# meffmadd/intro-tc-vae

Measured on AMD Instinct MI355X. Metric: images/sec (64x64x3, z=128, bs=64) intro-TC step, higher is better.
Workload: dtype f32 in/out/accumulate, conv products on split-fp16 MFMA (two scaled fp16 planes, 3 products, fp32-class); 1 GPU; c2: IntroTCSovler.train_step, conv arch, 64x64x3, z_dim=128, channels (64, 128, 256, 512), batch 64/GPU, Adam lr 2e-4, clip 100, N=10000; global_batch=64, parallelism=single, sync_bn=False

## Files before the change

### include/itcv_hip.h

```cpp
#ifndef ITCV_HIP_H
#define ITCV_HIP_H

#include <stddef.h>
#include <stdint.h>

#ifdef __cplusplus
extern "C" {
#endif

#define ITCV_ABI_VERSION 4

int itcv_abi_version(void);
const char* itcv_last_error(void);
int itcv_set_option(const char* name, int value);
int itcv_get_option(const char* name);

int itcv_profile_begin(void);
int itcv_profile_end(void);
int itcv_profile_get(int i, int* code, double* flop, float* ms);
int itcv_profile_clear(void);

size_t itcv_conv2d_packed_weight_elems(int Co, int Ci, int KS, int for_dgrad);
int itcv_conv2d_pack_weight(const float* w, float* wp, int Co, int Ci, int KS, int for_dgrad,
                            void* stream);
size_t itcv_conv2d_fwd_workspace(int B, int Ci, int H, int W, int Co, int KS);
int itcv_conv2d_fwd(const float* x, const float* wp, const float* bias, float* y, int B, int Ci,
                    int H, int W, int Co, int KS, int up2, void* ws, size_t ws_bytes, void* stream);
int itcv_conv2d_bf16s_supported(int Ci, int Co, int KS);
size_t itcv_conv2d_packed_weight_bytes_bf16s(int Co, int Ci, int KS, int for_dgrad, int ns);
int itcv_conv2d_pack_weight_bf16s(const float* w, void* wp, int Co, int Ci, int KS, int for_dgrad, int ns,
                                  void* stream);
size_t itcv_pack_desc_bytes(void);
int itcv_conv2d_pack_desc_bf16s(void* host_desc, const float* w, void* wp, int Co, int Ci, int KS, int for_dgrad,
                                int ns, int block0);
int itcv_conv2d_pack_weights_bf16s(const void* dev_table, int n, int total_blocks, int ns, void* stream);
size_t itcv_conv2d_fwd_bf16s_workspace(int B, int Ci, int H, int W, int Co, int KS);
int itcv_conv2d_fwd_bf16s(const float* x, const void* wp, const float* bias, float* y, int B, int Ci, int H,
                          int W, int Co, int KS, int up2, int ns, void* ws, size_t ws_bytes, void* stream);
#define ITCV_PLANES_F16X2 4
size_t itcv_planes_bytes(int B, int C, int HW, int ns);
int itcv_split_planes(const float* x, void* planes, int B, int C, int HW, int ns, void* stream);
int itcv_absmax(const float* x, size_t n, float* parts, void* stream);
int itcv_split_planes_scaled(const float* x, void* planes, int B, int C, int HW, int ns, const float* amax, void* stream);
size_t itcv_conv2d_fwd_bf16p_workspace(int B, int Ci, int H, int W, int Co, int KS, int ns);
int itcv_conv2d_fwd_bf16p(const void* xplanes, const void* wp, const float* bias, float* y, int B, int Ci, int H,
                          int W, int Co, int KS, int up2, int ns, void* ws, size_t ws_bytes, void* stream);
int itcv_conv2d_fwd_bf16p_stat_tiles(int B, int Ci, int H, int W, int Co, int KS, int ns);
int itcv_conv2d_fwd_bf16p_st(const void* xplanes, const void* wp, const float* bias, float* y, int B, int Ci, int H,
                             int W, int Co, int KS, int up2, int ns, float* tile_stats, void* ws, size_t ws_bytes,
                             void* stream);
int itcv_conv2d_wgrad_bf16p_supported(int B, int Ci, int H, int W, int Co, int KS);
size_t itcv_conv2d_wgrad_bf16p_workspace(int B, int Ci, int H, int W, int Co, int KS);
int itcv_conv2d_wgrad_bf16p(const void* xplanes, const void* dyplanes, float* dw, int B, int Ci, int H, int W,
                            int Co, int KS, int up2, int ns , int accumulate, void* ws, size_t ws_bytes,
                            void* stream);
int itcv_conv2d_wgrad_bf16p_slabs(int B, int Ci, int H, int W, int Co, int KS);
size_t itcv_wgrad_reduce_desc_bytes(void);
int itcv_wgrad_reduce_desc(void* host_desc, const float* const* slabs, const int* splits, int nsrc, float* dw, int Co,
                           int Ci, int accumulate, int block0);
int itcv_wgrad_reduce_many(const void* dev_table, int n, int total_blocks, void* stream);
int itcv_wgrad_reduce_max_descs(void);
size_t itcv_linear_workspace(int B, int K, int N);
int itcv_linear_fwd(const float* x, const float* w, const float* bias, float* y, int B, int K, int N, void* ws,
                    size_t ws_bytes, void* stream);
int itcv_linear_dgrad(const float* dy, const float* w, float* dx, int B, int K, int N, void* ws, size_t ws_bytes,
                      void* stream);
int itcv_linear_wgrad(const float* dy, const float* x, float* dw, int B, int K, int N, int accumulate, void* ws,
                      size_t ws_bytes, void* stream);
int itcv_conv2d_wgrad5_bf16p_supported(int Cs, int Cb, int H, int W);
size_t itcv_conv2d_wgrad5_bf16p_workspace(int B, int H);
int itcv_conv2d_wgrad5_bf16p(const float* small, const void* big_planes, float* dw, int B, int Cs, int H, int W,
                             int stem, int ns , const float* small_amax ,
                             int accumulate, void* ws, size_t ws_bytes, void* stream);
int itcv_conv2d_small_cout_supported(int Co, int KS);
int itcv_conv2d_small_cout_bf16p_supported(int C, int Co, int KS);
int itcv_conv2d_small_cout_fwd_bf16p(const void* xplanes, const float* w, const float* bias, float* y, int B, int C,
                                     int H, int W, int Co, int KS, int for_dgrad, int ns , void* stream);
int itcv_conv2d_small_cout_fwd(const float* x, const float* w, const float* bias, float* y, int B, int C,
                               int H, int W, int Co, int KS, int for_dgrad, void* stream);
int itcv_conv2d_small_cin_supported(int C, int KS);
int itcv_conv2d_small_cin_fwd(const float* x, const float* w, const float* bias, float* y, int B, int C, int H,
                              int W, int Co, int KS, int for_dgrad, void* stream);

int itcv_conv2d_small_cin_bf16x3_supported(int C, int Co, int KS, int W);
int itcv_conv2d_small_cin_fwd_bf16x3(const float* x, const float* w, const float* bias, float* y, int B, int C, int H,
                                     int W, int Co, int KS, int for_dgrad, int ns ,
                                     const float* x_amax , void* stream);
int itcv_conv2d_wgrad_bf16s_supported(int Ci, int H, int W, int Co, int KS);
int itcv_conv2d_wgrad_bf16s(const float* x, const float* dy, float* dw, int B, int Ci, int H, int W, int Co,
                            int KS, int ns, int accumulate, void* ws, size_t ws_bytes, void* stream);
size_t itcv_conv2d_wgrad_workspace(int B, int Ci, int H, int W, int Co, int KS);
int itcv_conv2d_wgrad(const float* x, const float* dy, float* dw, int B, int Ci, int H, int W,
                      int Co, int KS, int up2, int accumulate, void* ws, size_t ws_bytes, void* stream);
int itcv_conv2d_fwd_variant(int B, int Ci, int H, int W, int Co, int KS, int up2);
int itcv_conv2d_wgrad_variant(int B, int Ci, int H, int W, int Co, int KS, int up2);
size_t itcv_bias_grad_workspace(int B, int C, int HW);
int itcv_bias_grad(const float* dy, float* db, int B, int C, int HW, int accumulate, void* ws,
                   size_t ws_bytes, void* stream);

size_t itcv_bn_workspace(int B, int C, int HW);
int itcv_bn_moments(const float* x, double* sums, int B, int C, int HW, void* ws, size_t ws_bytes,
                    void* stream);
int itcv_bn_train_stats(const float* x, int B, int C, int HW, float eps, float momentum, float* running_mean,
                        float* running_var, int64_t* num_batches_tracked, float* mean, float* rstd, void* ws,
                        size_t ws_bytes, void* stream);
int itcv_bn_finalize(const double* sums, double count, float eps, float momentum, float* running_mean,
                     float* running_var, int64_t* num_batches_tracked, float* mean, float* rstd, int C,
                     void* stream);
int itcv_bn_eval_stats(const float* running_mean, const float* running_var, float eps, float* mean,
                       float* rstd, int C, void* stream);
int itcv_bn_act_fwd(const float* x, const float* mean, const float* rstd, const float* gamma,
                    const float* beta, const float* skip, float* y, int B, int C, int H, int W,
                    float slope, int pool, void* planes, int ns, size_t plane_stride, void* stream);
int itcv_bn_act_planes_supported(int C, int H, int W, int pool);
int itcv_bn_act_bwd_reduce(const float* x, const float* dy, const float* mean, const float* rstd,
                           const float* gamma, const float* beta, const float* skip, double* dsums,
                           float* dgamma, float* dbeta, int accumulate, int B, int C, int H, int W,
                           float slope, int pool, int up2, void* ws, size_t ws_bytes, void* stream);
int itcv_bn_act_bwd_apply(const float* x, const float* dy, const float* mean, const float* rstd,
                          const float* gamma, const float* beta, const float* skip, const double* dsums,
                          const double* local_dsums, double count, float* dx, float* dskip,
                          float* dgamma, float* dbeta, int accumulate, int B, int C, int H, int W,
                          float slope, int pool, int up2, void* dx_planes, int ns, size_t plane_stride, void* stream);

int itcv_bn_train_fwd(const float* x, const float* gamma, const float* beta, const float* skip, float* y, void* planes,
                      int ns, int B, int C, int H, int W, float slope, int pool, float eps, float momentum,
                      float* running_mean, float* running_var, int64_t* num_batches_tracked, float* mean, float* rstd,
                      void* ws, size_t ws_bytes, size_t plane_stride, const float* tile_stats, int tiles, int tile_pitch,
                      int groups, void* stream);
int itcv_bn_train_bwd(const float* x, const float* dy, const float* mean, const float* rstd, const float* gamma,
                      const float* beta, const float* skip, double* dsums, float* dx, float* dskip, void* dx_planes,
                      int ns, float* dgamma, float* dbeta, int accumulate, int B, int C, int H, int W, float slope,
                      int pool, int up2, void* ws, size_t ws_bytes, size_t plane_stride, int groups, void* stream);

#define ITCV_BN_PATH_ONE_BLOCK 0
#define ITCV_BN_PATH_SLICED_FOLD 1
#define ITCV_BN_PATH_SLICED_COMBINE 2
#define ITCV_BN_PATH_FALLBACK 3
#define ITCV_BN_PATH_PER_GROUP 4
#define ITCV_BN_PATH_TILE_STATS 5
int itcv_bn_plan_query(int bwd, int B, int C, int H, int W, int pool, int up2, int groups, int planes, int ns,
                       size_t ws_bytes, int tile_stats, int* path, int* splits);

int itcv_lrelu_fwd(const float* x, float* y, size_t n, float slope, void* stream);
int itcv_lrelu_bwd(const float* x, const float* dy, float* dx, size_t n, float slope, void* stream);
int itcv_sigmoid_fwd(const float* x, float* y, size_t n, void* stream);
int itcv_sigmoid_bwd(const float* y, const float* dy, float* dx, size_t n, void* stream);
int itcv_avgpool2_fwd(const float* x, float* y, int BC, int H, int W, void* stream);
int itcv_avgpool2_bwd(const float* dy, float* dx, int BC, int H, int W, void* stream);
int itcv_upsample2_fwd(const float* x, float* y, int BC, int H, int W, void* stream);
int itcv_upsample2_bwd(const float* dy, float* dx, int BC, int H, int W, void* stream);
int itcv_add(const float* a, const float* b, float* out, size_t n, void* stream);

int itcv_reparam_fwd(const float* mu, const float* logvar, const float* eps, float* z, size_t n,
                     void* stream);
int itcv_reparam_bwd(const float* dz, const float* logvar, const float* eps, float* dmu, float* dlogvar,
                     size_t n, void* stream);
int itcv_kl_rows_fwd(const float* logvar, const float* mu, float* kl, int B, int D, void* stream);
int itcv_kl_rows_bwd(const float* g, const float* logvar, const float* mu, float* dlogvar, float* dmu,
                     int B, int D, void* stream);

#define ITCV_TC_VAR_FROM_ROW 0x1
#define ITCV_TC_EPS_DENSITY 0x2
#define ITCV_TC_WEIGHTED 0x4
#define ITCV_TC_LIVE (ITCV_TC_VAR_FROM_ROW | ITCV_TC_EPS_DENSITY)
size_t itcv_tc_fwd_workspace(int Bl, int Bt, int D);
int itcv_tc_fwd(const float* z, const float* mu_all, const float* logvar, float* prodm, float* logqz,
                float* lse, float* sjoint, int Bl, int Bt, int row_offset, int D, int64_t dataset_size, int flags,
                void* ws, size_t ws_bytes, void* stream);
size_t itcv_tc_bwd_workspace(int Bl, int Bt);
int itcv_tc_bwd(const float* g, const float* z, const float* mu_all, const float* logvar,
                const float* logqz, const float* lse, const float* sjoint, float* dz, float* dmu_all,
                float* dlogvar, int Bl, int Bt, int row_offset, int D, int64_t dataset_size, int flags, void* ws,
                size_t ws_bytes, void* stream);
int itcv_tc_kl_fwd(const float* z, const float* mu_all, const float* logvar, float* out, float* rows, float* prodm,
                   float* logqz, float* lse, float* sjoint, int Bl, int Bt, int row_offset, int D, int64_t dataset_size,
                   float coef_tc, float coef_kl, int reduction, void* ws, size_t ws_bytes, void* stream);
int itcv_tc_kl_bwd(const float* g, const float* z, const float* mu_all, const float* logvar, const float* logqz,
                   const float* lse, const float* sjoint, float* dz, float* dmu_all, float* dlogvar, int Bl, int Bt,
                   int row_offset, int D, int64_t dataset_size, float coef_tc, float coef_kl, int reduction, void* ws,
                   size_t ws_bytes, void* stream);
size_t itcv_tc_full_fwd_workspace(int Bl, int Bt, int D);
int itcv_tc_full_fwd(const float* z, const float* mu_all, const float* logvar_all, int ld, float* out, float* rows,
                     float* comps, float* prodm, float* logqz, float* lse, float* sjoint, float* ivar, int Bl, int Bt,
                     int row_offset, int D, int64_t dataset_size, float alpha, float beta, float gamma, int reduction,
                     void* ws, size_t ws_bytes, void* stream);
size_t itcv_tc_full_bwd_workspace(int Bl, int Bt);
int itcv_tc_full_bwd(const float* g, const float* z, const float* mu_all, const float* logvar_all, int ld,
                     const float* logqz, const float* lse, const float* sjoint, const float* ivar, float* dz, float* dmu_all,
                     float* dlogvar_all, int Bl, int Bt, int row_offset, int D, int64_t dataset_size, float alpha,
                     float beta, float gamma, int reduction, void* ws, size_t ws_bytes, void* stream);
int itcv_kl_loss_fwd(const float* logvar, const float* mu, float* out, int B, int D, int reduction, float scale, void* stream);
int itcv_kl_loss_bwd(const float* g, const float* logvar, const float* mu, float* dlogvar, float* dmu, int B, int D,
                     int reduction, float scale, void* stream);
int itcv_diag_logdensity_rows(const float* z, const float* mu, const float* logvar, float* logq_cx,
                              float* logpz, int B, int D, void* stream);
int itcv_gauss_logdensity_fwd(const float* x, const float* mu, const float* logvar, float* out, const int64_t* dims,
                              const int64_t* sx, const int64_t* sm, const int64_t* sl, int eps_density, void* stream);
int itcv_gauss_logdensity_bwd(const float* g, const float* x, const float* mu, const float* logvar, float* dx,
                              float* dlogvar, const int64_t* dims, const int64_t* sx, const int64_t* sm,
                              const int64_t* sl, int eps_density, void* stream);
int itcv_sampling_fwd(const float* lp, float* prodm, float* logqz, float* lse, float* sjoint, int B, int D,
                      int64_t dataset_size, int weighted, void* stream);
int itcv_sampling_bwd(const float* g_prodm, const float* g_logqz, const float* lp, const float* lse,
                      const float* sjoint, const float* logqz, float* dlp, int B, int D, int64_t dataset_size,
                      int weighted, void* stream);
int itcv_on_off_diag(const float* x, float* diag, float* off, int m, int n, void* stream);

#define ITCV_LOSS_MSE 0
#define ITCV_LOSS_L1 1
#define ITCV_LOSS_BCE 2
int itcv_recon_rows_fwd(const float* x, const float* recon, float* rows, int B, size_t P, int loss_type,
                        void* ws, size_t ws_bytes, void* stream);
size_t itcv_recon_workspace(int B, size_t P);
int itcv_recon_rows_bwd(const float* x, const float* recon, const float* g, float* drecon, int B, size_t P,
                        int loss_type, void* stream);

int itcv_recon_loss_fwd(const float* x, const float* recon, float* out, int B, size_t P, int loss_type, int reduction,
                        float scale, void* ws, size_t ws_bytes, void* stream);
int itcv_recon_loss_bwd(const float* x, const float* recon, const float* g, float* drecon, int B, size_t P,
                        int loss_type, int reduction, float scale, void* stream);
int itcv_exp_elbo_fwd(const float* a, const float* b, float* out, float* w, int B, float c, void* stream);
int itcv_exp_elbo_bwd(const float* g, const float* w, float* da, float* db, int B, void* stream);
int itcv_lincomb_fwd(const float* const* terms, const float* weights, int n, float* out, void* stream);
int itcv_lincomb_bwd(const float* g, const float* weights, int n, float* grads, void* stream);

size_t itcv_sumsq_workspace(size_t n);
int itcv_sumsq(const float* x, size_t n, double* out, void* ws, size_t ws_bytes, void* stream);
int itcv_clip_coef(const double* sumsq, int nparts, double clip, float* norm_out, float* coef_out,
                   void* stream);
int itcv_scale_by_dev(float* x, size_t n, const float* coef_dev, void* stream);
int itcv_adam_step(float* p, const float* g, float* m, float* v, size_t n, float lr, float beta1,
                   float beta2, float eps, int step, void* stream);
int itcv_adam_step_dev(float* p, const float* g, float* m, float* v, size_t n, float lr, float beta1,
                       float beta2, float eps, int* step_dev, void* stream);
#define ITCV_OPT_MAXIMIZE 0x1
#define ITCV_OPT_NESTEROV 0x2
#define ITCV_OPT_AMSGRAD 0x4
#define ITCV_OPT_DECOUPLED_WD 0x8
#define ITCV_OPT_CENTERED 0x10
int itcv_adamx_step_dev(float* p, const float* g, float* exp_avg, float* exp_avg_sq, float* max_exp_avg_sq,
                        const unsigned char* live, size_t n, double lr, double beta1, double beta2, double eps,
                        double weight_decay, int flags, int* step_dev, void* stream);
int itcv_sgd_step_dev(float* p, const float* g, float* momentum_buffer, const unsigned char* live, size_t n, double lr,
                      double momentum, double dampening, double weight_decay, int flags, int* step_dev, void* stream);
int itcv_adagrad_step_dev(float* p, const float* g, float* sum, const unsigned char* live, size_t n, double lr,
                          double lr_decay, double weight_decay, double eps, int flags, int* step_dev, void* stream);
int itcv_rmsprop_step_dev(float* p, const float* g, float* square_avg, float* momentum_buffer, float* grad_avg,
                          const unsigned char* live, size_t n, double lr, double alpha, double eps,
                          double weight_decay, double momentum, int flags, int* step_dev, void* stream);
int itcv_fill(float* x, size_t n, float value, void* stream);
int itcv_hflip(const float* x, float* y, const unsigned char* flip, int B, int rows_per_image, int W, void* stream);

#ifdef __cplusplus
}
#endif
#endif
```

### intro-tc-vae_amd/csrc/norm_act.hip

```cpp
#include <stdlib.h>

#include <type_traits>

#include "common.h"

namespace itcv {

constexpr int kRedThreads = 256;

__device__ __forceinline__ uint32_t fdiv(uint32_t a, uint32_t d, int sh) { return sh >= 0 ? (a >> sh) : (a / d); }

struct BnGrp {
  size_t xs;
  size_t os;
  size_t dys;
  size_t ps;
  int cs;
  int G;
};

struct BnFinal {
  double count;
  float eps, momentum;
  float* running_mean;
  float* running_var;
  int64_t* nbt;
  float* mean;
  float* rstd;
};

__device__ __forceinline__ void bn_finalize(double s1, double s2, double count, float eps, float momentum,
                                            float* running_mean, float* running_var, int c, float& mean_c, float& rstd_c) {
  const double m = s1 / count;
  double var = s2 / count - m * m;
  if (var < 0.0) var = 0.0;
  mean_c = (float)m;
  rstd_c = (float)(1.0 / sqrt(var + (double)eps));
  if (running_mean) running_mean[c] = (1.f - momentum) * running_mean[c] + momentum * (float)m;
  if (running_var) {
    const double unbiased = count > 1.0 ? var * count / (count - 1.0) : var;
    running_var[c] = (1.f - momentum) * running_var[c] + momentum * (float)unbiased;
  }
}

template <bool FUSED>
__global__ __launch_bounds__(kRedThreads) void bn_moments_partial(const float* __restrict__ x,
                                                                  double* __restrict__ part, int B, int C, int HW,
                                                                  int splits, int hw_shift, BnFinal f, BnGrp grp) {
  __shared__ double scratch[kRedThreads / 64];
  const uint32_t c = blockIdx.x, s = blockIdx.y, hw_n = HW, total = (uint32_t)B * hw_n;
  const uint32_t chunk = ((total + splits - 1) / splits + 3) & ~3u;
  const uint32_t beg = s * chunk, end = min(beg + chunk, total);
  const int ngroups = (FUSED && grp.G > 1) ? grp.G : 1;
  if (!FUSED) {
    x += (size_t)blockIdx.z * grp.xs;
    part += (size_t)blockIdx.z * splits * 2 * C;
  }
 for (int gi = 0; gi < ngroups; ++gi, x += grp.xs, f.mean += grp.cs, f.rstd += grp.cs) {
  double s1 = 0.0, s2 = 0.0;
  if ((HW & 3) == 0) {
#pragma unroll 4
    for (uint32_t i = beg + threadIdx.x * 4; i < end; i += kRedThreads * 4) {
      const uint32_t b = fdiv(i, hw_n, hw_shift), hw = i - b * hw_n;
      const float4 v = *reinterpret_cast<const float4*>(x + ((size_t)b * C + c) * hw_n + hw);
      s1 += ((double)v.x + (double)v.y) + ((double)v.z + (double)v.w);
      s2 += ((double)v.x * v.x + (double)v.y * v.y) + ((double)v.z * v.z + (double)v.w * v.w);
    }
  } else {
    for (uint32_t i = beg + threadIdx.x; i < end; i += kRedThreads) {
      const uint32_t b = fdiv(i, hw_n, hw_shift), hw = i - b * hw_n;
      const float v = x[((size_t)b * C + c) * hw_n + hw];
      s1 += (double)v;
      s2 += (double)v * v;
    }
  }
  s1 = block_sum(s1, scratch);
  s2 = block_sum(s2, scratch);
  if (threadIdx.x == 0) {
    if (FUSED) {
      bn_finalize(s1, s2, f.count, f.eps, f.momentum, f.running_mean, f.running_var, c, f.mean[c], f.rstd[c]);
      if (c == 0 && f.nbt) f.nbt[0] += 1;
    } else {
      part[((size_t)s * 2 + 0) * C + c] = s1;
      part[((size_t)s * 2 + 1) * C + c] = s2;
    }
  }
 }
}

__global__ void combine_partials(const double* __restrict__ part, double* __restrict__ sums, int C2, int splits) {
  const int i = blockIdx.x * blockDim.x + threadIdx.x;
  if (i >= C2) return;
  sums[i] = fold_strided(0.0, part + i, (size_t)C2, splits);
}

__global__ void bn_finalize_kernel(const double* __restrict__ sums, double count, float eps, float momentum,
                                   float* running_mean, float* running_var, int64_t* nbt, float* mean, float* rstd,
                                   int C) {
  const int c = blockIdx.x * blockDim.x + threadIdx.x;
  if (c == 0 && nbt) nbt[0] += 1;
  if (c >= C) return;
  bn_finalize(sums[c], sums[C + c], count, eps, momentum, running_mean, running_var, c, mean[c], rstd[c]);
}

__global__ __launch_bounds__(256) void bn_tile_stats_finalize_kernel(const float* __restrict__ ts, int tiles, int pitch,
                                                                    double count, float eps, float momentum,
                                                                    float* running_mean, float* running_var, int64_t* nbt,
                                                                    float* mean, float* rstd, int C) {
  __shared__ double scratch[4];
  const int c = blockIdx.x;
  const float* p1 = ts + (size_t)c * pitch;
  const float* p2 = ts + ((size_t)C + c) * pitch;
  double s1 = 0.0, s2 = 0.0;
  for (int t = threadIdx.x; t < tiles; t += 256) s1 += (double)p1[t], s2 += (double)p2[t];
  s1 = block_sum(s1, scratch);
  s2 = block_sum(s2, scratch);
  if (threadIdx.x == 0) {
    bn_finalize(s1, s2, count, eps, momentum, running_mean, running_var, c, mean[c], rstd[c]);
    if (c == 0 && nbt) nbt[0] += 1;
  }
}

__global__ void bn_combine_finalize_groups_kernel(const double* __restrict__ part, int splits, int G, double count, float eps,
                                                  float momentum, float* running_mean, float* running_var, int64_t* nbt,
                                                  float* mean, float* rstd, int C) {
  const int c = blockIdx.x * blockDim.x + threadIdx.x;
  if (c == 0 && nbt) nbt[0] += G;
  if (c >= C) return;
  for (int g = 0; g < G; ++g) {
    const double* pg = part + (size_t)g * splits * 2 * C;
    const double s1 = fold_strided(0.0, pg + c, (size_t)2 * C, splits);
    const double s2 = fold_strided(0.0, pg + C + c, (size_t)2 * C, splits);
    bn_finalize(s1, s2, count, eps, momentum, running_mean, running_var, c, mean[(size_t)g * C + c], rstd[(size_t)g * C + c]);
  }
}
__global__ void bn_combine_param_groups_kernel(const double* __restrict__ part, double* __restrict__ dsums, int C, int splits,
                                               int G, float* dgamma, float* dbeta, int accumulate) {
  const int c = blockIdx.x * blockDim.x + threadIdx.x;
  if (c >= C) return;
  float db = (accumulate && dbeta) ? dbeta[c] : 0.f, dg = (accumulate && dgamma) ? dgamma[c] : 0.f;
  for (int g = 0; g < G; ++g) {
    const double* pg = part + (size_t)g * splits * 2 * C;
    const double s1 = fold_strided(0.0, pg + c, (size_t)2 * C, splits);
    const double s2 = fold_strided(0.0, pg + C + c, (size_t)2 * C, splits);
    dsums[(size_t)g * 2 * C + c] = s1;
    dsums[(size_t)g * 2 * C + C + c] = s2;
    db += (float)s1, dg += (float)s2;
  }
  if (dbeta) dbeta[c] = db;
  if (dgamma) dgamma[c] = dg;
}

__global__ void bn_eval_stats_kernel(const float* rm, const float* rv, float eps, float* mean, float* rstd, int C) {
  const int c = blockIdx.x * blockDim.x + threadIdx.x;
  if (c >= C) return;
  mean[c] = rm[c];
  rstd[c] = 1.f / sqrtf(rv[c] + eps);
}

__device__ __forceinline__ float lrelu(float v, float slope) { return v > 0.f ? v : v * slope; }

template <int POOL>
__global__ void bn_act_fwd_kernel(const float* __restrict__ x, const float* __restrict__ mean,
                                  const float* __restrict__ rstd, const float* __restrict__ gamma,
                                  const float* __restrict__ beta, const float* __restrict__ skip,
                                  float* __restrict__ y, int C, int H, int W, size_t nout, float slope,
                                  int hw_shift, int c_mask) {
  const int HW = H * W;
  if (POOL == 0) {
    for (size_t i = ((size_t)blockIdx.x * blockDim.x + threadIdx.x) * 4; i < nout;
         i += (size_t)gridDim.x * blockDim.x * 4) {
      const uint32_t pl = fdiv((uint32_t)i, HW, hw_shift);
      const int c = c_mask >= 0 ? (int)(pl & (uint32_t)c_mask) : (int)(pl % (uint32_t)C);
      const float sc = gamma[c] * rstd[c], sh = beta[c] - mean[c] * sc;
      float4 v = *reinterpret_cast<const float4*>(x + i);
      v.x = v.x * sc + sh, v.y = v.y * sc + sh, v.z = v.z * sc + sh, v.w = v.w * sc + sh;
      if (skip) {
        const float4 k = *reinterpret_cast<const float4*>(skip + i);
        v.x += k.x, v.y += k.y, v.z += k.z, v.w += k.w;
      }
      v.x = lrelu(v.x, slope), v.y = lrelu(v.y, slope), v.z = lrelu(v.z, slope), v.w = lrelu(v.w, slope);
      *reinterpret_cast<float4*>(y + i) = v;
    }
  } else {
    const int Ho = H / 2, Wo = W / 2, HWo = Ho * Wo;
    for (size_t i = (size_t)blockIdx.x * blockDim.x + threadIdx.x; i < nout; i += (size_t)gridDim.x * blockDim.x) {
      const uint32_t bc = hw_shift >= 2 ? ((uint32_t)i >> (hw_shift - 2)) : (uint32_t)i / (uint32_t)HWo;
      const int r = (int)((uint32_t)i - bc * HWo), ho = r / Wo, wo = r - ho * Wo;
      const int c = c_mask >= 0 ? (int)(bc & (uint32_t)c_mask) : (int)(bc % (uint32_t)C);
      const float sc = gamma[c] * rstd[c], sh = beta[c] - mean[c] * sc;
      const size_t src = (size_t)bc * HW + (size_t)(2 * ho) * W + 2 * wo;
      const float2 a = *reinterpret_cast<const float2*>(x + src);
      const float2 b = *reinterpret_cast<const float2*>(x + src + W);
      float v0 = a.x * sc + sh, v1 = a.y * sc + sh, v2 = b.x * sc + sh, v3 = b.y * sc + sh;
      if (skip) {
        const float2 ka = *reinterpret_cast<const float2*>(skip + src);
        const float2 kb = *reinterpret_cast<const float2*>(skip + src + W);
        v0 += ka.x, v1 += ka.y, v2 += kb.x, v3 += kb.y;
      }
      y[i] = 0.25f * (lrelu(v0, slope) + lrelu(v1, slope) + lrelu(v2, slope) + lrelu(v3, slope));
    }
  }
}

constexpr int kStatCh = 64;
struct BnStatsIn {
  const double* part;
  int splits;
  double count;
  float eps, momentum;
  float* running_mean;
  float* running_var;
  int64_t* nbt;
  float* mean_out;
  float* rstd_out;
};

template <int PX, int NS>
__device__ __forceinline__ void store_planes_wave(u32x4* __restrict__ planes, size_t plane_stride, uint32_t per_plane,
                                                  uint32_t HWo, uint32_t cidx0, const u32x4 (&ch)[PX][NS],
                                                  u32x4* __restrict__ strip) {
  const uint32_t lane = threadIdx.x & 63;
#pragma unroll
  for (int p = 0; p < NS; ++p) {
#pragma unroll
    for (int s = 0; s < PX; ++s) strip[lane * PX + s] = ch[s][p];
#pragma unroll
    for (int k = 0; k < PX; ++k) {
      const uint32_t n = k * 64 + lane, idx2 = cidx0 + n / PX, s2 = n % PX;
      const uint32_t bc8 = idx2 / per_plane, pp = idx2 - bc8 * per_plane;
      planes[(size_t)p * plane_stride + (size_t)bc8 * HWo + (size_t)pp * PX + s2] = strip[n];
    }
  }
}

template <int POOL, int NS, bool STATS, bool F16 = false>
__global__ __launch_bounds__(256) void bn_act_fwd_planes_kernel(
    const float* __restrict__ x, const float* __restrict__ mean, const float* __restrict__ rstd,
    const float* __restrict__ gamma, const float* __restrict__ beta, const float* __restrict__ skip,
    float* __restrict__ y, u32x4* __restrict__ planes, int B, int C, int H, int W, float slope, BnStatsIn st,
    size_t plane_stride, BnGrp grp) {
  if constexpr (F16) {
    if (blockIdx.x == 0 && blockIdx.z == 0 && threadIdx.x == 0) {
      ScaleRec* rec = reinterpret_cast<ScaleRec*>(planes + (size_t)NS * plane_stride);
      rec->scale = 1.f, rec->inv = 1.f, rec->pad[0] = rec->pad[1] = 0.f;
    }
  }
  {
    const size_t g = blockIdx.z;
    x += g * grp.xs, planes += g * grp.ps, mean += g * grp.cs, rstd += g * grp.cs;
    if (skip) skip += g * grp.xs;
    if (y) y += g * grp.os;
  }
  __shared__ float s_mean[STATS ? kStatCh : 1], s_rstd[STATS ? kStatCh : 1];
  constexpr int PX = POOL ? 2 : 4;
  __shared__ u32x4 strips[4][64 * PX];
  const int HW = H * W, C8 = C >> 3;
  const int Ho = POOL ? H / 2 : H, Wo = POOL ? W / 2 : W, HWo = Ho * Wo;
  const uint32_t per_plane = (uint32_t)HWo / PX, total = (uint32_t)B * C8 * per_plane;
  for (uint32_t base = blockIdx.x * blockDim.x; base < total; base += gridDim.x * blockDim.x) {
    const uint32_t idx = base + threadIdx.x;
    const uint32_t g0 = base / per_plane;
    if (STATS) {
      __syncthreads();
      const uint32_t last = min(base + blockDim.x, total) - 1, ng = last / per_plane - g0 + 1;
      if (threadIdx.x < ng * 8) {
        const uint32_t gz = blockIdx.z, G = grp.G > 1 ? grp.G : 1;
        const uint32_t g = g0 + threadIdx.x / 8, c = (g % C8) * 8 + (threadIdx.x & 7);
        const double* part = st.part + (size_t)gz * st.splits * 2 * C;
        const double s1 = fold_strided(0.0, part + c, (size_t)2 * C, st.splits);
        const double s2 = fold_strided(0.0, part + C + c, (size_t)2 * C, st.splits);
        float mf, rf;
        bn_finalize(s1, s2, st.count, st.eps, 0.f, nullptr, nullptr, 0, mf, rf);
        s_mean[threadIdx.x] = mf, s_rstd[threadIdx.x] = rf;
        if (g < (uint32_t)C8 && g * per_plane >= base) {
          st.mean_out[(size_t)gz * C + c] = mf, st.rstd_out[(size_t)gz * C + c] = rf;
          if (gz == 0) {
            double t1 = s1, t2 = s2;
            for (uint32_t gg = 0; gg < G; ++gg) {
              if (gg) {
                const double* pg = st.part + (size_t)gg * st.splits * 2 * C;
                t1 = fold_strided(0.0, pg + c, (size_t)2 * C, st.splits);
                t2 = fold_strided(0.0, pg + C + c, (size_t)2 * C, st.splits);
              }
              float um, ur;
              bn_finalize(t1, t2, st.count, st.eps, st.momentum, st.running_mean, st.running_var, c, um, ur);
            }
            if (c == 0 && st.nbt) st.nbt[0] += G;
          }
        }
      }
      __syncthreads();
    }
    if (idx >= total) continue;
    const uint32_t bc8 = idx / per_plane, pp = idx - bc8 * per_plane;
    const uint32_t b = bc8 / C8, c8 = bc8 - b * C8;
    float o[8][PX];
    float4 xin[POOL ? 1 : 8];
    float p_ga[8], p_be[8], p_mu[8], p_rs[8];
#pragma unroll
    for (int j = 0; j < 8; ++j) {
      const int c = c8 * 8 + j;
      if (POOL == 0) xin[POOL ? 0 : j] = *reinterpret_cast<const float4*>(x + ((size_t)b * C + c) * HW + (size_t)pp * 4);
      p_ga[j] = gamma[c], p_be[j] = beta[c];
      p_mu[j] = STATS ? s_mean[(bc8 - g0) * 8 + j] : mean[c], p_rs[j] = STATS ? s_rstd[(bc8 - g0) * 8 + j] : rstd[c];
    }
#pragma unroll
    for (int j = 0; j < 8; ++j) {
      const int c = c8 * 8 + j;
      const float mu = p_mu[j], rs = p_rs[j];
      const float sc = p_ga[j] * rs, sh = p_be[j] - mu * sc;
      const size_t bc = (size_t)b * C + c;
      if (POOL == 0) {
        const size_t i = bc * HW + (size_t)pp * 4;
        float4 v = xin[POOL ? 0 : j];
        v.x = v.x * sc + sh, v.y = v.y * sc + sh, v.z = v.z * sc + sh, v.w = v.w * sc + sh;
        if (skip) {
          const float4 k = *reinterpret_cast<const float4*>(skip + i);
          v.x += k.x, v.y += k.y, v.z += k.z, v.w += k.w;
        }
        v.x = lrelu(v.x, slope), v.y = lrelu(v.y, slope), v.z = lrelu(v.z, slope), v.w = lrelu(v.w, slope);
        if (y) *reinterpret_cast<float4*>(y + i) = v;
        o[j][0] = v.x, o[j][1] = v.y, o[j][POOL ? 0 : 2] = v.z, o[j][POOL ? 1 : 3] = v.w;
      } else {
        const uint32_t ho = (pp * 2) / Wo, wo = pp * 2 - ho * Wo;
        const size_t src = bc * HW + (size_t)(2 * ho) * W + 2 * wo;
        const float4 a = *reinterpret_cast<const float4*>(x + src);
        const float4 bb = *reinterpret_cast<const float4*>(x + src + W);
        float v0 = a.x * sc + sh, v1 = a.y * sc + sh, v2 = bb.x * sc + sh, v3 = bb.y * sc + sh;
        float w0 = a.z * sc + sh, w1 = a.w * sc + sh, w2 = bb.z * sc + sh, w3 = bb.w * sc + sh;
        if (skip) {
          const float4 ka = *reinterpret_cast<const float4*>(skip + src);
          const float4 kb = *reinterpret_cast<const float4*>(skip + src + W);
          v0 += ka.x, v1 += ka.y, v2 += kb.x, v3 += kb.y;
          w0 += ka.z, w1 += ka.w, w2 += kb.z, w3 += kb.w;
        }
        const float r0 = 0.25f * (lrelu(v0, slope) + lrelu(v1, slope) + lrelu(v2, slope) + lrelu(v3, slope));
        const float r1 = 0.25f * (lrelu(w0, slope) + lrelu(w1, slope) + lrelu(w2, slope) + lrelu(w3, slope));
        if (y) *reinterpret_cast<float2*>(y + bc * HWo + (size_t)pp * 2) = make_float2(r0, r1);
        o[j][0] = r0, o[j][1] = r1;
      }
    }
    u32x4 chk[PX][NS];
#pragma unroll
    for (int px = 0; px < PX; ++px) {
      float v8[8];
#pragma unroll
      for (int j = 0; j < 8; ++j) v8[j] = o[j][px];
      split8<NS, F16>(v8, chk[px]);
    }
    const uint32_t cidx0 = base + (threadIdx.x & ~63u);
    if (cidx0 + 64 <= total) {
      store_planes_wave<PX, NS>(planes, plane_stride, per_plane, (uint32_t)HWo, cidx0, chk, strips[threadIdx.x >> 6]);
    } else {
#pragma unroll
      for (int px = 0; px < PX; ++px)
#pragma unroll
        for (int p = 0; p < NS; ++p) planes[(size_t)p * plane_stride + (size_t)bc8 * HWo + (size_t)pp * PX + px] = chk[px][p];
    }
  }
}

template <int MODE>
__device__ __forceinline__ float upstream(const float* __restrict__ dy, size_t bc, int h, int w, int H, int W) {
  if (MODE == 0) return dy[bc * H * W + (size_t)h * W + w];
  if (MODE == 1) return 0.25f * dy[bc * (H / 2) * (W / 2) + (size_t)(h >> 1) * (W / 2) + (w >> 1)];
  const size_t base = bc * (size_t)(4 * H * W) + (size_t)(2 * h) * (2 * W) + 2 * w;
  const float2 a = *reinterpret_cast<const float2*>(dy + base);
  const float2 b = *reinterpret_cast<const float2*>(dy + base + 2 * W);
  return (a.x + a.y) + (b.x + b.y);
}

template <int MODE>
__global__ __launch_bounds__(kRedThreads) void bn_bwd_partial(const float* __restrict__ x,
                                                              const float* __restrict__ dy,
                                                              const float* __restrict__ mean,
                                                              const float* __restrict__ rstd,
                                                              const float* __restrict__ gamma,
                                                              const float* __restrict__ beta,
                                                              const float* __restrict__ skip,
                                                              double* __restrict__ part, int B, int C, int H, int W,
                                                              float slope, int splits) {
  __shared__ double scratch[kRedThreads / 64];
  const int c = blockIdx.x, s = blockIdx.y, HW = H * W;
  const size_t total = (size_t)B * HW;
  const size_t chunk = (total + splits - 1) / splits;
  const size_t beg = (size_t)s * chunk, end = beg + chunk < total ? beg + chunk : total;
  const float mu = mean[c], rs = rstd[c], ga = gamma[c], be = beta[c];
  double s1 = 0.0, s2 = 0.0;
  for (size_t i = beg + threadIdx.x; i < end; i += kRedThreads) {
    const size_t b = i / HW;
    const int hw = (int)(i - b * HW), h = hw / W, w = hw - h * W;
    const size_t bc = b * C + c;
    const float xh = (x[bc * HW + hw] - mu) * rs;
    float u = xh * ga + be;
    if (skip) u += skip[bc * HW + hw];
    float g = upstream<MODE>(dy, bc, h, w, H, W);
    if (!(u > 0.f)) g *= slope;
    s1 += (double)g;
    s2 += (double)g * (double)xh;
  }
  s1 = block_sum(s1, scratch);
  s2 = block_sum(s2, scratch);
  if (threadIdx.x == 0) {
    part[((size_t)s * 2 + 0) * C + c] = s1;
    part[((size_t)s * 2 + 1) * C + c] = s2;
  }
}

template <int MODE>
__global__ void bn_bwd_apply_kernel(const float* __restrict__ x, const float* __restrict__ dy,
                                    const float* __restrict__ mean, const float* __restrict__ rstd,
                                    const float* __restrict__ gamma, const float* __restrict__ beta,
                                    const float* __restrict__ skip, const double* __restrict__ dsums, double count,
                                    float* __restrict__ dx, float* __restrict__ dskip, int C, int H, int W,
                                    size_t n, float slope) {
  const int HW = H * W;
  for (size_t i = (size_t)blockIdx.x * blockDim.x + threadIdx.x; i < n; i += (size_t)gridDim.x * blockDim.x) {
    const size_t bc = i / HW;
    const int hw = (int)(i - bc * HW), h = hw / W, w = hw - h * W;
    const int c = (int)(bc % C);
    const float mu = mean[c], rs = rstd[c], ga = gamma[c];
    const float xh = (x[i] - mu) * rs;
    float u = xh * ga + beta[c];
    if (skip) u += skip[i];
    float g = upstream<MODE>(dy, bc, h, w, H, W);
    if (!(u > 0.f)) g *= slope;
    const float m1 = (float)(dsums[c] / count), m2 = (float)(dsums[C + c] / count);
    dx[i] = ga * rs * (g - m1 - xh * m2);
    if (dskip) dskip[i] = g;
  }
}



template <int MODE>
__device__ __forceinline__ float4 upstream4(const float* __restrict__ dy, uint32_t bc, uint32_t h, uint32_t w,
                                            uint32_t H, uint32_t W) {
  if (MODE == 0) return *reinterpret_cast<const float4*>(dy + (size_t)bc * H * W + h * W + w);
  if (MODE == 1) {
    const float2 d = *reinterpret_cast<const float2*>(dy + (size_t)bc * (H / 2) * (W / 2) + (h >> 1) * (W / 2) + (w >> 1));
    return make_float4(0.25f * d.x, 0.25f * d.x, 0.25f * d.y, 0.25f * d.y);
  }
  const float* p = dy + (size_t)bc * (4 * H * W) + (size_t)(2 * h) * (2 * W) + 2 * w;
  const float4 a0 = *reinterpret_cast<const float4*>(p), a1 = *reinterpret_cast<const float4*>(p + 4);
  const float4 b0 = *reinterpret_cast<const float4*>(p + 2 * W), b1 = *reinterpret_cast<const float4*>(p + 2 * W + 4);
  return make_float4((a0.x + a0.y) + (b0.x + b0.y), (a0.z + a0.w) + (b0.z + b0.w), (a1.x + a1.y) + (b1.x + b1.y),
                     (a1.z + a1.w) + (b1.z + b1.w));
}

struct BnBwdFinal {
  double* dsums;
  float* dgamma;
  float* dbeta;
  int accumulate;
};

template <int MODE, bool FUSED, bool MX = false>
__global__ __launch_bounds__(kRedThreads) void bn_bwd_partial_v4(
    const float* __restrict__ x, const float* __restrict__ dy, const float* __restrict__ mean,
    const float* __restrict__ rstd, const float* __restrict__ gamma, const float* __restrict__ beta,
    const float* __restrict__ skip, double* __restrict__ part, int B, int C, int H, int W, float slope, int splits,
    int w_shift, int hw_shift, BnBwdFinal f, BnGrp grp, float* __restrict__ mx = nullptr, int nmx = 0) {
  __shared__ double scratch[kRedThreads / 64];
  __shared__ float mscratch[MX ? 2 * (kRedThreads / 64) : 1];
  const uint32_t gz = FUSED ? 0u : blockIdx.z;
  const uint32_t c = blockIdx.x, s = blockIdx.y, HW = H * W, total = (uint32_t)B * HW;
  const uint32_t chunk = ((total + splits - 1) / splits + 3) & ~3u;
  const uint32_t beg = s * chunk, end = min(beg + chunk, total);
  const float ga = gamma[c], be = beta[c];
  const int ngroups = (FUSED && grp.G > 1) ? grp.G : 1;
  if (!FUSED) {
    const size_t g = blockIdx.z;
    x += g * grp.xs, dy += g * grp.dys, mean += g * grp.cs, rstd += g * grp.cs, part += g * splits * 2 * C;
    if (skip) skip += g * grp.xs;
  }
  float acc_db = 0.f, acc_dg = 0.f;
  if (FUSED && threadIdx.x == 0 && f.accumulate) {
    if (f.dbeta) acc_db = f.dbeta[c];
    if (f.dgamma) acc_dg = f.dgamma[c];
  }
 for (int gi = 0; gi < ngroups; ++gi, x += grp.xs, dy += grp.dys, mean += grp.cs, rstd += grp.cs, f.dsums += 2 * grp.cs) {
  if (skip && gi) skip += grp.xs;
  const float mu = mean[c], rs = rstd[c];
  double s1 = 0.0, s2 = 0.0;
  float gmax = 0.f, xmax = 0.f;
  constexpr int U = 4;
  for (uint32_t i0 = beg + threadIdx.x * 4; i0 < end; i0 += kRedThreads * 4 * U) {
    float4 xv4[U], g4[U], k4[U];
    bool ok[U];
#pragma unroll
    for (int u = 0; u < U; ++u) {
      const uint32_t iu = i0 + (uint32_t)u * kRedThreads * 4;
      ok[u] = iu < end;
      const uint32_t i = ok[u] ? iu : i0;
      const uint32_t b = fdiv(i, HW, hw_shift), hw = i - b * HW;
      const uint32_t h = fdiv(hw, W, w_shift), w = hw - h * W;
      const uint32_t bc = b * C + c;
      xv4[u] = *reinterpret_cast<const float4*>(x + (size_t)bc * HW + hw);
      g4[u] = upstream4<MODE>(dy, bc, h, w, H, W);
    }
    if (skip) {
#pragma unroll
      for (int u = 0; u < U; ++u) {
        const uint32_t iu = i0 + (uint32_t)u * kRedThreads * 4, i = iu < end ? iu : i0;
        const uint32_t b = fdiv(i, HW, hw_shift), hw = i - b * HW;
        k4[u] = *reinterpret_cast<const float4*>(skip + (size_t)(b * C + c) * HW + hw);
      }
    } else {
#pragma unroll
      for (int u = 0; u < U; ++u) k4[u] = make_float4(0.f, 0.f, 0.f, 0.f);
    }
#pragma unroll
    for (int u = 0; u < U; ++u) {
      const float4 xv = xv4[u];
      float4 g = g4[u];
      const float xh0 = (xv.x - mu) * rs, xh1 = (xv.y - mu) * rs, xh2 = (xv.z - mu) * rs, xh3 = (xv.w - mu) * rs;
      float u0 = xh0 * ga + be, u1 = xh1 * ga + be, u2 = xh2 * ga + be, u3 = xh3 * ga + be;
      if (skip) u0 += k4[u].x, u1 += k4[u].y, u2 += k4[u].z, u3 += k4[u].w;
      if (!(u0 > 0.f)) g.x *= slope;
      if (!(u1 > 0.f)) g.y *= slope;
      if (!(u2 > 0.f)) g.z *= slope;
      if (!(u3 > 0.f)) g.w *= slope;
      const double a1 = ((double)g.x + (double)g.y) + ((double)g.z + (double)g.w);
      const double a2 = ((double)g.x * xh0 + (double)g.y * xh1) + ((double)g.z * xh2 + (double)g.w * xh3);
      s1 += ok[u] ? a1 : 0.0;
      s2 += ok[u] ? a2 : 0.0;
      if constexpr (MX) {
        const float gm = fmaxf(fmaxf(fabsf(g.x), fabsf(g.y)), fmaxf(fabsf(g.z), fabsf(g.w)));
        const float xm = fmaxf(fmaxf(fabsf(xh0), fabsf(xh1)), fmaxf(fabsf(xh2), fabsf(xh3)));
        gmax = fmaxf(gmax, ok[u] ? gm : 0.f);
        xmax = fmaxf(xmax, ok[u] ? xm : 0.f);
      }
    }
  }
  s1 = block_sum(s1, scratch);
  s2 = block_sum(s2, scratch);
  if constexpr (MX) {
    gmax = wave_max(gmax), xmax = wave_max(xmax);
    if ((threadIdx.x & 63) == 0) mscratch[threadIdx.x >> 6] = gmax, mscratch[kRedThreads / 64 + (threadIdx.x >> 6)] = xmax;
    __syncthreads();
    if (threadIdx.x == 0) {
      float gm = 0.f, xm = 0.f;
      for (int k = 0; k < kRedThreads / 64; ++k) gm = fmaxf(gm, mscratch[k]), xm = fmaxf(xm, mscratch[kRedThreads / 64 + k]);
      const size_t idx = ((size_t)(FUSED ? (uint32_t)gi : gz) * splits + s) * C + c;
      mx[idx] = fabsf(ga * rs) * gm, mx[(size_t)nmx + idx] = xm;
    }
    __syncthreads();
  }
  if (threadIdx.x == 0) {
    if (FUSED) {
      f.dsums[c] = s1;
      f.dsums[C + c] = s2;
      acc_db += (float)s1, acc_dg += (float)s2;
    } else {
      part[((size_t)s * 2 + 0) * C + c] = s1;
      part[((size_t)s * 2 + 1) * C + c] = s2;
    }
  }
 }
  if (FUSED && threadIdx.x == 0) {
    if (f.dbeta) f.dbeta[c] = acc_db;
    if (f.dgamma) f.dgamma[c] = acc_dg;
  }
}

template <int MODE>
__global__ void bn_bwd_apply_v4(const float* __restrict__ x, const float* __restrict__ dy,
                                const float* __restrict__ mean, const float* __restrict__ rstd,
                                const float* __restrict__ gamma, const float* __restrict__ beta,
                                const float* __restrict__ skip, const double* __restrict__ dsums, double count,
                                float* __restrict__ dx, float* __restrict__ dskip, int C, int H, int W, uint32_t n4,
                                float slope, int w_shift, int hw_shift, int c_mask) {
  const uint32_t HW = H * W;
  for (uint32_t j = blockIdx.x * blockDim.x + threadIdx.x; j < n4; j += gridDim.x * blockDim.x) {
    const uint32_t i = j * 4;
    const uint32_t bc = fdiv(i, HW, hw_shift), hw = i - bc * HW;
    const uint32_t h = fdiv(hw, W, w_shift), w = hw - h * W;
    const uint32_t c = c_mask >= 0 ? (bc & (uint32_t)c_mask) : (bc % (uint32_t)C);
    const float mu = mean[c], rs = rstd[c], ga = gamma[c], be = beta[c];
    const float m1 = (float)(dsums[c] / count), m2 = (float)(dsums[C + c] / count), gr = ga * rs;
    const float4 xv = *reinterpret_cast<const float4*>(x + i);
    float4 g = upstream4<MODE>(dy, bc, h, w, H, W);
    const float xh0 = (xv.x - mu) * rs, xh1 = (xv.y - mu) * rs, xh2 = (xv.z - mu) * rs, xh3 = (xv.w - mu) * rs;
    float u0 = xh0 * ga + be, u1 = xh1 * ga + be, u2 = xh2 * ga + be, u3 = xh3 * ga + be;
    if (skip) {
      const float4 k = *reinterpret_cast<const float4*>(skip + i);
      u0 += k.x, u1 += k.y, u2 += k.z, u3 += k.w;
    }
// ... 42 lines not shown
      for (int k = 0; k < 4; ++k) {
        u = fmaxf(fmaxf(u, fmaxf(tu[k].x, tu[k].y)), fmaxf(tu[k].z, tu[k].w));
        v = fmaxf(fmaxf(v, fmaxf(tv[k].x, tv[k].y)), fmaxf(tv[k].z, tv[k].w));
      }
    }
    u = wave_max(u), v = wave_max(v);
    if ((threadIdx.x & 63) == 0) s_uv[threadIdx.x >> 6] = u, s_uv[4 + (threadIdx.x >> 6)] = v;
    __syncthreads();
    u = fmaxf(fmaxf(s_uv[0], s_uv[1]), fmaxf(s_uv[2], s_uv[3]));
    v = fmaxf(fmaxf(s_uv[4], s_uv[5]), fmaxf(s_uv[6], s_uv[7]));
    pscale = scale_for_bound(u * (2.f + v));
    if (blockIdx.x == 0 && blockIdx.z == 0 && threadIdx.x == 0) {
      ScaleRec* rec = reinterpret_cast<ScaleRec*>(planes + (size_t)NS * plane_stride);
      rec->scale = pscale, rec->inv = 1.f / pscale, rec->pad[0] = rec->pad[1] = 0.f;
    }
  }
  const uint32_t zg = gridDim.z - 1 - blockIdx.z;
  {
    const size_t g = zg;
    x += g * grp.xs, dy += g * grp.dys, planes += g * grp.ps, mean += g * grp.cs, rstd += g * grp.cs;
    if (dsums) dsums += g * 2 * grp.cs;
    if (skip) skip += g * grp.xs;
    if (dx) dx += g * grp.xs;
    if (dskip) dskip += g * grp.xs;
  }
  __shared__ float s_m1[SUMS ? kStatCh : 1], s_m2[SUMS ? kStatCh : 1];
  __shared__ u32x4 strips[4][64 * 4];
  const uint32_t HW = H * W, C8 = C >> 3, per_plane = HW / 4, total = (uint32_t)B * C8 * per_plane;
  const uint32_t sweep = gridDim.x * blockDim.x, rbase = (gridDim.x - 1 - blockIdx.x) * blockDim.x;
  for (int it = (int)((total + sweep - 1) / sweep) - 1; it >= 0; --it) {
    const uint32_t base = (uint32_t)it * sweep + rbase;
    if (base >= total) continue;
    const uint32_t idx = base + threadIdx.x;
    const uint32_t g0 = base / per_plane;
    if (SUMS) {
      __syncthreads();
      const uint32_t last = min(base + blockDim.x, total) - 1, ng = last / per_plane - g0 + 1;
      if (threadIdx.x < ng * 8) {
        const uint32_t gz = zg, G = grp.G > 1 ? grp.G : 1;
        const uint32_t g = g0 + threadIdx.x / 8, c = (g % C8) * 8 + (threadIdx.x & 7);
        const double* part = sm.part + (size_t)gz * sm.splits * 2 * C;
        const double s1 = fold_strided(0.0, part + c, (size_t)2 * C, sm.splits);
        const double s2 = fold_strided(0.0, part + C + c, (size_t)2 * C, sm.splits);
        s_m1[threadIdx.x] = (float)(s1 / count), s_m2[threadIdx.x] = (float)(s2 / count);
        if (g < C8 && g * per_plane >= base) {
          sm.dsums_out[(size_t)gz * 2 * C + c] = s1, sm.dsums_out[(size_t)gz * 2 * C + C + c] = s2;
          if (gz == 0) {
            float db = (sm.accumulate && sm.dbeta) ? sm.dbeta[c] : 0.f, dg = (sm.accumulate && sm.dgamma) ? sm.dgamma[c] : 0.f;
            db += (float)s1, dg += (float)s2;
            for (uint32_t gg = 1; gg < G; ++gg) {
              const double* pg = sm.part + (size_t)gg * sm.splits * 2 * C;
              db += (float)fold_strided(0.0, pg + c, (size_t)2 * C, sm.splits);
              dg += (float)fold_strided(0.0, pg + C + c, (size_t)2 * C, sm.splits);
            }
            if (sm.dbeta) sm.dbeta[c] = db;
            if (sm.dgamma) sm.dgamma[c] = dg;
          }
        }
      }
      __syncthreads();
    }
    if (idx >= total) continue;
    const uint32_t bc8 = idx / per_plane, p4 = idx - bc8 * per_plane;
    const uint32_t b = bc8 / C8, c8 = bc8 - b * C8;
    const uint32_t hw = p4 * 4, h = fdiv(hw, W, w_shift), w = hw - h * W;
    float o[8][4];
#pragma unroll
    for (int j0 = 0; j0 < 8; j0 += 4) {
      float4 xv4[4], g4[4], k4[4];
      float pm[4][4];
      double ds4[4][2];
#pragma unroll
      for (int jj = 0; jj < 4; ++jj) {
        const uint32_t c = c8 * 8 + j0 + jj, bc = b * C + c;
        xv4[jj] = *reinterpret_cast<const float4*>(x + bc * HW + hw);
        g4[jj] = upstream4<MODE>(dy, bc, h, w, H, W);
        pm[jj][0] = mean[c], pm[jj][1] = rstd[c], pm[jj][2] = gamma[c], pm[jj][3] = beta[c];
        if (!SUMS) ds4[jj][0] = dsums[c], ds4[jj][1] = dsums[C + c];
      }
      if (skip) {
#pragma unroll
        for (int jj = 0; jj < 4; ++jj) k4[jj] = *reinterpret_cast<const float4*>(skip + (b * C + c8 * 8 + j0 + jj) * HW + hw);
      } else {
#pragma unroll
        for (int jj = 0; jj < 4; ++jj) k4[jj] = make_float4(0.f, 0.f, 0.f, 0.f);
      }
#pragma unroll
      for (int jj = 0; jj < 4; ++jj) {
        const int j = j0 + jj;
        const uint32_t c = c8 * 8 + j, bc = b * C + c;
        const uint32_t i = bc * HW + hw;
        const float mu = pm[jj][0], rs = pm[jj][1], ga = pm[jj][2], be = pm[jj][3];
        const float m1 = SUMS ? s_m1[(bc8 - g0) * 8 + j] : (float)(ds4[jj][0] / count);
        const float m2 = SUMS ? s_m2[(bc8 - g0) * 8 + j] : (float)(ds4[jj][1] / count), gr = ga * rs;
        const float4 xv = xv4[jj];
        float4 g = g4[jj];
        const float xh0 = (xv.x - mu) * rs, xh1 = (xv.y - mu) * rs, xh2 = (xv.z - mu) * rs, xh3 = (xv.w - mu) * rs;
        float u0 = xh0 * ga + be, u1 = xh1 * ga + be, u2 = xh2 * ga + be, u3 = xh3 * ga + be;
        if (skip) {
          const float4 k = k4[jj];
          u0 += k.x, u1 += k.y, u2 += k.z, u3 += k.w;
        }
        if (!(u0 > 0.f)) g.x *= slope;
        if (!(u1 > 0.f)) g.y *= slope;
        if (!(u2 > 0.f)) g.z *= slope;
        if (!(u3 > 0.f)) g.w *= slope;
        const float4 d = make_float4(gr * (g.x - m1 - xh0 * m2), gr * (g.y - m1 - xh1 * m2), gr * (g.z - m1 - xh2 * m2),
                                     gr * (g.w - m1 - xh3 * m2));
        if (dx) *reinterpret_cast<float4*>(dx + i) = d;
        if (dskip) *reinterpret_cast<float4*>(dskip + i) = g;
        o[j][0] = d.x, o[j][1] = d.y, o[j][2] = d.z, o[j][3] = d.w;
      }
    }
    u32x4 chk[4][NS];
#pragma unroll
    for (int px = 0; px < 4; ++px) {
      float v8[8];
#pragma unroll
      for (int j = 0; j < 8; ++j) v8[j] = o[j][px];
      split8<NS, F16>(v8, chk[px], pscale);
    }
    const uint32_t cidx0 = base + (threadIdx.x & ~63u);
    if (cidx0 + 64 <= total) {
      store_planes_wave<4, NS>(planes, plane_stride, per_plane, HW, cidx0, chk, strips[threadIdx.x >> 6]);
    } else {
#pragma unroll
      for (int px = 0; px < 4; ++px)
#pragma unroll
        for (int p = 0; p < NS; ++p) planes[(size_t)p * plane_stride + (size_t)bc8 * HW + hw + px] = chk[px][p];
    }
  }
}

__global__ void bn_param_grad_kernel(const double* __restrict__ local, float* dgamma, float* dbeta, int C,
                                     int accumulate) {
  const int c = blockIdx.x * blockDim.x + threadIdx.x;
  if (c >= C) return;
  if (dbeta) dbeta[c] = (accumulate ? dbeta[c] : 0.f) + (float)local[c];
  if (dgamma) dgamma[c] = (accumulate ? dgamma[c] : 0.f) + (float)local[C + c];
}

__global__ void lrelu_fwd_kernel(const float* __restrict__ x, float* __restrict__ y, size_t n, float slope) {
  for (size_t i = (size_t)blockIdx.x * blockDim.x + threadIdx.x; i < n; i += (size_t)gridDim.x * blockDim.x)
    y[i] = lrelu(x[i], slope);
}
__global__ void lrelu_bwd_kernel(const float* __restrict__ x, const float* __restrict__ dy, float* __restrict__ dx,
                                 size_t n, float slope) {
  for (size_t i = (size_t)blockIdx.x * blockDim.x + threadIdx.x; i < n; i += (size_t)gridDim.x * blockDim.x)
    dx[i] = x[i] > 0.f ? dy[i] : dy[i] * slope;
}
__global__ void sigmoid_fwd_kernel(const float* __restrict__ x, float* __restrict__ y, size_t n) {
  for (size_t i = (size_t)blockIdx.x * blockDim.x + threadIdx.x; i < n; i += (size_t)gridDim.x * blockDim.x)
    y[i] = 1.f / (1.f + expf(-x[i]));
}
__global__ void sigmoid_bwd_kernel(const float* __restrict__ y, const float* __restrict__ dy,
                                   float* __restrict__ dx, size_t n) {
  for (size_t i = (size_t)blockIdx.x * blockDim.x + threadIdx.x; i < n; i += (size_t)gridDim.x * blockDim.x) {
    const float s = y[i];
    dx[i] = dy[i] * (1.f - s) * s;
  }
}
__global__ void add_kernel(const float* __restrict__ a, const float* __restrict__ b, float* __restrict__ o,
                           size_t n) {
  for (size_t i = (size_t)blockIdx.x * blockDim.x + threadIdx.x; i < n; i += (size_t)gridDim.x * blockDim.x)
    o[i] = a[i] + b[i];
}
__global__ void avgpool2_fwd_kernel(const float* __restrict__ x, float* __restrict__ y, int H, int W, size_t nout) {
  const int Ho = H / 2, Wo = W / 2;
  for (size_t i = (size_t)blockIdx.x * blockDim.x + threadIdx.x; i < nout; i += (size_t)gridDim.x * blockDim.x) {
    const size_t bc = i / ((size_t)Ho * Wo);
    const int r = (int)(i - bc * Ho * Wo), ho = r / Wo, wo = r - ho * Wo;
    const size_t src = bc * H * W + (size_t)(2 * ho) * W + 2 * wo;
    const float2 a = *reinterpret_cast<const float2*>(x + src);
    const float2 b = *reinterpret_cast<const float2*>(x + src + W);
    y[i] = 0.25f * ((a.x + a.y) + (b.x + b.y));
  }
}
__global__ void avgpool2_bwd_kernel(const float* __restrict__ dy, float* __restrict__ dx, int H, int W, size_t n) {
  for (size_t i = (size_t)blockIdx.x * blockDim.x + threadIdx.x; i < n; i += (size_t)gridDim.x * blockDim.x) {
    const size_t bc = i / ((size_t)H * W);
    const int r = (int)(i - bc * H * W), h = r / W, w = r - h * W;
    dx[i] = 0.25f * dy[bc * (H / 2) * (W / 2) + (size_t)(h >> 1) * (W / 2) + (w >> 1)];
  }
}
__global__ void upsample2_fwd_kernel(const float* __restrict__ x, float* __restrict__ y, int H, int W, size_t n) {
  const int Ho = 2 * H, Wo = 2 * W;
  for (size_t i = (size_t)blockIdx.x * blockDim.x + threadIdx.x; i < n; i += (size_t)gridDim.x * blockDim.x) {
    const size_t bc = i / ((size_t)Ho * Wo);
    const int r = (int)(i - bc * Ho * Wo), h = r / Wo, w = r - h * Wo;
    y[i] = x[bc * H * W + (size_t)(h >> 1) * W + (w >> 1)];
  }
}
__global__ void upsample2_bwd_kernel(const float* __restrict__ dy, float* __restrict__ dx, int H, int W, size_t n) {
  for (size_t i = (size_t)blockIdx.x * blockDim.x + threadIdx.x; i < n; i += (size_t)gridDim.x * blockDim.x) {
    const size_t bc = i / ((size_t)H * W);
    const int r = (int)(i - bc * H * W), h = r / W, w = r - h * W;
    dx[i] = upstream<2>(dy, bc, h, w, H, W);
  }
}

static inline int ilog2_exact(int v) {
  if (v <= 0 || (v & (v - 1))) return -1;
  int sh = 0;
  while ((1 << sh) < v) ++sh;
  return sh;
}

static inline int grid_for(size_t n, int per_thread = 1) {
  size_t b = cdivz(cdivz(n, per_thread), 256);
  if (b > 256 * 8) b = 256 * 8;
  return b < 1 ? 1 : (int)b;
}

static inline bool bn_fmt_ok(int ns) { return ns == 2 || ns == 3 || ns == ITCV_PLANES_F16X2; }
static inline int bn_splits(int B, int C, int HW) {
  const size_t total = (size_t)B * HW;
  constexpr int target = 1024;
  int s = cdiv(target, C);
  const size_t maxs = cdivz(total, 1024);
  if ((size_t)s > maxs) s = (int)maxs;
  if (s < 1) s = 1;
  if (C >= 256 && total <= 65536) s = 1;
  return s;
}

enum class BnPath {
  OneBlock,
  SlicedFold,
  SlicedCombine,
  Fallback,
  PerGroup,
  TileStats,
};
struct BnPlan {
  BnPath path;
  int G, splits, mode;
  bool vec, f16;
  int per_plane, nmx;
  BnGrp grp;
  size_t pstride;
  size_t part_doubles;
  size_t ws_need;
  dim3 rgrid, agrid;
};

static inline size_t bn_ws_bytes(int G, int splits, int C, bool maxima) {
  return (size_t)G * splits * 2 * C * (sizeof(double) + (maxima ? sizeof(float) : 0));
}

static BnPlan bn_plan(bool bwd, int B, int C, int H, int W, int pool, int up2, int groups, bool planes, int ns,
                      size_t plane_stride, size_t ws_bytes, bool tile_stats) {
  BnPlan p{};
  const bool opool = !bwd && pool;
  const int HW = H * W, HWo = opool ? HW / 4 : HW;
  const size_t n = (size_t)B * C * HW;
  p.G = groups > 1 ? groups : 1;
  p.splits = bn_splits(B, C, HW);
  p.mode = pool ? 1 : (up2 ? 2 : 0);
  p.vec = W % 4 == 0 && n < (1ull << 31);
  p.f16 = ns == ITCV_PLANES_F16X2 && (planes || (bwd && groups > 1));
  p.per_plane = HWo / (opool ? 2 : 4);
  p.nmx = p.G * p.splits * C;
  p.grp = BnGrp{n, (size_t)B * C * HWo, pool ? n / 4 : (up2 ? n * 4 : n), (size_t)B * (C / 8) * HWo, C, p.G};
  p.pstride = plane_stride ? plane_stride : p.grp.ps;
  p.part_doubles = (size_t)p.G * p.splits * 2 * C;
  p.ws_need = bn_ws_bytes(p.G, p.splits, C, bwd && p.f16);
  const bool planes_ok = planes && bn_fmt_ok(ns) && itcv_bn_act_planes_supported(C, H, W, opool) && n < (1ull << 31);
  if (tile_stats) p.path = groups > 1 ? BnPath::PerGroup : BnPath::TileStats;
  else if (!planes_ok) p.path = groups > 1 ? BnPath::PerGroup : BnPath::Fallback;
  else if (p.splits == 1) p.path = BnPath::OneBlock;
  else if (groups > 1 && ws_bytes < p.ws_need) p.path = BnPath::PerGroup;
  else p.path = p.per_plane >= 64 ? BnPath::SlicedFold : BnPath::SlicedCombine;
  if (groups > 1 && p.path == BnPath::OneBlock && !(bwd && p.f16)) p.ws_need = 0;
  p.rgrid = dim3(C, p.splits, p.splits == 1 ? 1 : p.G);
  if (planes_ok) p.agrid = dim3(grid_for((size_t)B * (C / 8) * p.per_plane), 1, p.G);
  else p.agrid = dim3(bwd ? grid_for(n, p.vec ? 4 : 1) : grid_for((size_t)B * C * HWo, pool ? 1 : 4));
  return p;
}

template <int N, typename F>
static inline void bn_pick(int v, F&& f) {
  if constexpr (N > 1) {
    if (v == N - 1) return f(std::integral_constant<int, N - 1>{});
    return bn_pick<N - 1>(v, f);
  } else {
    f(std::integral_constant<int, 0>{});
  }
}
static inline int bn_fmt(int ns) { return ns == ITCV_PLANES_F16X2 ? 2 : (ns == 2 ? 0 : 1); }

static int bn_stats_launch(const BnPlan& p, const float* x, int B, int C, int HW, const BnFinal& f, void* ws, size_t ws_bytes,
                           hipStream_t st, const char* who) {
  ITCV_REQUIRE(!p.ws_need || (ws && ws_bytes >= p.ws_need), who);
  double* part = static_cast<double*>(ws);
  if (p.splits == 1)
    hipLaunchKernelGGL(bn_moments_partial<true>, p.rgrid, dim3(kRedThreads), 0, st, x, part, B, C, HW, 1, ilog2_exact(HW), f,
                       p.grp);
  else
    hipLaunchKernelGGL(bn_moments_partial<false>, p.rgrid, dim3(kRedThreads), 0, st, x, part, B, C, HW, p.splits,
                       ilog2_exact(HW), BnFinal{}, p.grp);
  ITCV_CHECK_LAUNCH(who);
  if (p.splits > 1 && p.path != BnPath::SlicedFold) {
    hipLaunchKernelGGL(bn_combine_finalize_groups_kernel, dim3(cdiv(C, 256)), dim3(256), 0, st, part, p.splits, p.G, f.count,
                       f.eps, f.momentum, f.running_mean, f.running_var, f.nbt, f.mean, f.rstd, C);
    ITCV_CHECK_LAUNCH(who);
  }
  return 0;
}

static int bn_fwd_apply_launch(const BnPlan& p, const float* x, const float* mean, const float* rstd, const float* gamma,
                               const float* beta, const float* skip, float* y, void* planes, int ns, int B, int C, int H, int W,
                               float slope, int pool, const BnStatsIn& fold, hipStream_t st) {
  ITCV_REQUIRE((size_t)B * C * H * W < (1ull << 31), "itcv_bn_act_fwd(tensor < 2^31 elements)");
  if (planes) {
    ITCV_REQUIRE(bn_fmt_ok(ns) && itcv_bn_act_planes_supported(C, H, W, pool), "itcv_bn_act_fwd(planes)");
    bn_pick<2>(pool ? 1 : 0, [&](auto pool_c) {
      bn_pick<3>(bn_fmt(ns), [&](auto fmt_c) {
        bn_pick<2>(fold.part ? 1 : 0, [&](auto stats_c) {
          constexpr int POOL = decltype(pool_c)::value, FMT = decltype(fmt_c)::value;
          constexpr bool STATS = decltype(stats_c)::value != 0;
          launch_timed((bn_act_fwd_planes_kernel<POOL, FMT == 1 ? 3 : 2, STATS, FMT == 2>), p.agrid, dim3(256), 0, st, x, mean,
                       rstd, gamma, beta, skip, y, static_cast<u32x4*>(planes), B, C, H, W, slope, fold, p.pstride, p.grp);
        });
      });
    });
    ITCV_CHECK_LAUNCH("itcv_bn_act_fwd(planes)");
    return 0;
  }
  if (pool) ITCV_REQUIRE(H % 2 == 0 && W % 2 == 0, "itcv_bn_act_fwd(pool)");
  else ITCV_REQUIRE((H * W) % 4 == 0, "itcv_bn_act_fwd(H*W % 4)");
  const size_t nout = pool ? (size_t)B * C * (H / 2) * (W / 2) : (size_t)B * C * H * W;
  bn_pick<2>(pool ? 1 : 0, [&](auto pool_c) {
    hipLaunchKernelGGL(bn_act_fwd_kernel<decltype(pool_c)::value>, p.agrid, dim3(256), 0, st, x, mean, rstd, gamma, beta, skip,
                       y, C, H, W, nout, slope, ilog2_exact(H * W), ilog2_exact(C) >= 0 ? C - 1 : -1);
  });
  ITCV_CHECK_LAUNCH("itcv_bn_act_fwd");
  return 0;
}

static int bn_bwd_reduce_launch(const BnPlan& p, const float* x, const float* dy, const float* mean, const float* rstd,
                                const float* gamma, const float* beta, const float* skip, double* dsums, float* dgamma,
                                float* dbeta, int accumulate, int B, int C, int H, int W, float slope, void* ws, size_t ws_bytes,
                                hipStream_t st, const char* who) {
  if (p.mode == 1) ITCV_REQUIRE(H % 2 == 0 && W % 2 == 0, who);
  ITCV_REQUIRE(!p.ws_need || (ws && ws_bytes >= p.ws_need), who);
  ITCV_REQUIRE(!p.f16 || p.vec, "itcv_bn_train_bwd(fp16 planes need W % 4 == 0)");
  double* part = static_cast<double*>(ws);
  float* mx = p.f16 ? reinterpret_cast<float*>(part + p.part_doubles) : nullptr;
  const bool fused = p.vec && p.splits == 1;
  const BnBwdFinal bf = fused ? BnBwdFinal{dsums, dgamma, dbeta, accumulate} : BnBwdFinal{};
  bn_pick<3>(p.mode, [&](auto mode_c) {
    constexpr int MODE = decltype(mode_c)::value;
    if (!p.vec) {
      hipLaunchKernelGGL(bn_bwd_partial<MODE>, p.rgrid, dim3(kRedThreads), 0, st, x, dy, mean, rstd, gamma, beta, skip, part,
                         B, C, H, W, slope, p.splits);
      return;
    }
    bn_pick<2>(fused ? 1 : 0, [&](auto fused_c) {
      bn_pick<2>(p.f16 ? 1 : 0, [&](auto mx_c) {
        hipLaunchKernelGGL((bn_bwd_partial_v4<MODE, decltype(fused_c)::value != 0, decltype(mx_c)::value != 0>), p.rgrid,
                           dim3(kRedThreads), 0, st, x, dy, mean, rstd, gamma, beta, skip, part, B, C, H, W, slope, p.splits,
                           ilog2_exact(W), ilog2_exact(H * W), bf, p.grp, mx, p.nmx);
      });
    });
  });
  ITCV_CHECK_LAUNCH(who);
  if (!fused && p.path != BnPath::SlicedFold) {
    hipLaunchKernelGGL(bn_combine_param_groups_kernel, dim3(cdiv(C, 256)), dim3(256), 0, st, part, dsums, C, p.splits, p.G,
                       dgamma, dbeta, accumulate);
    ITCV_CHECK_LAUNCH(who);
  }
  return 0;
}

static int bn_bwd_apply_launch(const BnPlan& p, const float* x, const float* dy, const float* mean, const float* rstd,
                               const float* gamma, const float* beta, const float* skip, const double* dsums, double count,
                               float* dx, float* dskip, void* dx_planes, int ns, int B, int C, int H, int W, float slope,
                               const BnBwdSumsIn& fold, const float* mx, hipStream_t st) {
  ITCV_REQUIRE(x && dy && mean && rstd && gamma && beta && dsums && (dx || dx_planes) && B > 0 && C > 0 && count > 0,
               "itcv_bn_act_bwd_apply");
  const int wsh = ilog2_exact(W);
  if (dx_planes) {
    ITCV_REQUIRE(bn_fmt_ok(ns) && p.vec && itcv_bn_act_planes_supported(C, H, W, 0), "itcv_bn_act_bwd_apply(planes)");
    if (ns == ITCV_PLANES_F16X2 && !mx)
      return fail("%s: fp16 gradient planes take their scale from the maxima of the reduce pass: use itcv_bn_train_bwd",
                  "itcv_bn_act_bwd_apply");
    bn_pick<3>(p.mode, [&](auto mode_c) {
      bn_pick<3>(bn_fmt(ns), [&](auto fmt_c) {
        bn_pick<2>(fold.part ? 1 : 0, [&](auto sums_c) {
          constexpr int MODE = decltype(mode_c)::value, FMT = decltype(fmt_c)::value;
          constexpr bool SUMS = decltype(sums_c)::value != 0;
          launch_timed((bn_bwd_apply_planes<MODE, FMT == 1 ? 3 : 2, SUMS, FMT == 2>), p.agrid, dim3(256), 0, st, x, dy, mean,
                       rstd, gamma, beta, skip, SUMS ? static_cast<const double*>(nullptr) : dsums, count, dx, dskip,
                       static_cast<u32x4*>(dx_planes), B, C, H, W, slope, wsh, fold, p.pstride, p.grp, mx, p.nmx);
        });
      });
    });
    ITCV_CHECK_LAUNCH("itcv_bn_act_bwd_apply(planes)");
    return 0;
  }
  const size_t n = (size_t)B * C * H * W;
  bn_pick<3>(p.mode, [&](auto mode_c) {
    constexpr int MODE = decltype(mode_c)::value;
    if (p.vec)
      hipLaunchKernelGGL(bn_bwd_apply_v4<MODE>, p.agrid, dim3(256), 0, st, x, dy, mean, rstd, gamma, beta, skip, dsums, count,
                         dx, dskip, C, H, W, (uint32_t)(n / 4), slope, wsh, ilog2_exact(H * W),
                         ilog2_exact(C) >= 0 ? C - 1 : -1);
    else
      hipLaunchKernelGGL(bn_bwd_apply_kernel<MODE>, p.agrid, dim3(256), 0, st, x, dy, mean, rstd, gamma, beta, skip, dsums,
                         count, dx, dskip, C, H, W, n, slope);
  });
  ITCV_CHECK_LAUNCH("itcv_bn_act_bwd_apply");
  return 0;
}

}

using namespace itcv;

extern "C" {

size_t itcv_bn_workspace(int B, int C, int HW) {
  if (B <= 0 || C <= 0 || HW <= 0) return 0;
  return bn_ws_bytes(1, bn_splits(B, C, HW), C, true);
}

int itcv_bn_moments(const float* x, double* sums, int B, int C, int HW, void* ws, size_t ws_bytes, void* stream) {
  ITCV_REQUIRE(x && sums && B > 0 && C > 0 && HW > 0, "itcv_bn_moments");
  const int splits = bn_splits(B, C, HW);
  ITCV_REQUIRE(ws && ws_bytes >= bn_ws_bytes(1, splits, C, false), "itcv_bn_moments(workspace)");
  double* part = static_cast<double*>(ws);
  hipLaunchKernelGGL(bn_moments_partial<false>, dim3(C, splits), dim3(kRedThreads), 0, S(stream), x, part, B, C, HW,
                     splits, ilog2_exact(HW), BnFinal{}, BnGrp{});
  ITCV_CHECK_LAUNCH("itcv_bn_moments");
  hipLaunchKernelGGL(combine_partials, dim3(cdiv(2 * C, 256)), dim3(256), 0, S(stream), part, sums, 2 * C, splits);
  ITCV_CHECK_LAUNCH("itcv_bn_moments(combine)");
  return 0;
}

int itcv_bn_train_stats(const float* x, int B, int C, int HW, float eps, float momentum, float* running_mean,
                        float* running_var, int64_t* num_batches_tracked, float* mean, float* rstd, void* ws,
                        size_t ws_bytes, void* stream) {
  ITCV_REQUIRE(x && mean && rstd && B > 0 && C > 0 && HW > 0, "itcv_bn_train_stats");
  const BnPlan p = bn_plan(false, B, C, HW, 1, 0, 0, 1, false, 0, 0, ws ? ws_bytes : 0, false);
  const BnFinal f{(double)B * HW, eps, momentum, running_mean, running_var, num_batches_tracked, mean, rstd};
  return bn_stats_launch(p, x, B, C, HW, f, ws, ws_bytes, S(stream), "itcv_bn_train_stats");
}

int itcv_bn_finalize(const double* sums, double count, float eps, float momentum, float* running_mean,
                     float* running_var, int64_t* num_batches_tracked, float* mean, float* rstd, int C,
                     void* stream) {
  ITCV_REQUIRE(sums && mean && rstd && C > 0 && count > 0, "itcv_bn_finalize");
  hipLaunchKernelGGL(bn_finalize_kernel, dim3(cdiv(C, 256)), dim3(256), 0, S(stream), sums, count, eps, momentum,
                     running_mean, running_var, num_batches_tracked, mean, rstd, C);
  ITCV_CHECK_LAUNCH("itcv_bn_finalize");
  return 0;
}

int itcv_bn_eval_stats(const float* running_mean, const float* running_var, float eps, float* mean, float* rstd,
                       int C, void* stream) {
  ITCV_REQUIRE(running_mean && running_var && mean && rstd && C > 0, "itcv_bn_eval_stats");
  hipLaunchKernelGGL(bn_eval_stats_kernel, dim3(cdiv(C, 256)), dim3(256), 0, S(stream), running_mean, running_var,
                     eps, mean, rstd, C);
  ITCV_CHECK_LAUNCH("itcv_bn_eval_stats");
  return 0;
}

int itcv_bn_act_planes_supported(int C, int H, int W, int pool) {
  return C > 0 && (C & 7) == 0 && H > 0 && W > 0 && W % 4 == 0 && (!pool || H % 2 == 0);
}

int itcv_bn_act_fwd(const float* x, const float* mean, const float* rstd, const float* gamma, const float* beta,
                    const float* skip, float* y, int B, int C, int H, int W, float slope, int pool, void* planes,
                    int ns, size_t plane_stride, void* stream) {
  ITCV_REQUIRE(x && mean && rstd && gamma && beta && (y || planes) && B > 0 && C > 0 && H > 0 && W > 0, "itcv_bn_act_fwd");
  const BnPlan p = bn_plan(false, B, C, H, W, pool, 0, 1, planes != nullptr, ns, plane_stride, 0, false);
  return bn_fwd_apply_launch(p, x, mean, rstd, gamma, beta, skip, y, planes, ns, B, C, H, W, slope, pool, BnStatsIn{},
                             S(stream));
}

int itcv_bn_act_bwd_reduce(const float* x, const float* dy, const float* mean, const float* rstd, const float* gamma,
                           const float* beta, const float* skip, double* dsums, float* dgamma, float* dbeta,
                           int accumulate, int B, int C, int H, int W, float slope, int pool, int up2, void* ws,
                           size_t ws_bytes, void* stream) {
  ITCV_REQUIRE(x && dy && mean && rstd && gamma && beta && dsums && B > 0 && C > 0, "itcv_bn_act_bwd_reduce");
  ITCV_REQUIRE(!(pool && up2), "itcv_bn_act_bwd_reduce(pool and up2 are exclusive)");
  const BnPlan p = bn_plan(true, B, C, H, W, pool, up2, 1, false, 0, 0, ws ? ws_bytes : 0, false);
  return bn_bwd_reduce_launch(p, x, dy, mean, rstd, gamma, beta, skip, dsums, dgamma, dbeta, accumulate, B, C, H, W, slope, ws,
                              ws_bytes, S(stream), "itcv_bn_act_bwd_reduce");
}

int itcv_bn_act_bwd_apply(const float* x, const float* dy, const float* mean, const float* rstd, const float* gamma,
                          const float* beta, const float* skip, const double* dsums, const double* local_dsums,
                          double count, float* dx, float* dskip, float* dgamma, float* dbeta, int accumulate, int B,
                          int C, int H, int W, float slope, int pool, int up2, void* dx_planes, int ns,
                          size_t plane_stride, void* stream) {
  ITCV_REQUIRE(!(pool && up2), "itcv_bn_act_bwd_apply(pool and up2 are exclusive)");
  const BnPlan p = bn_plan(true, B, C, H, W, pool, up2, 1, dx_planes != nullptr, ns, plane_stride, 0, false);
  if (int e = bn_bwd_apply_launch(p, x, dy, mean, rstd, gamma, beta, skip, dsums, count, dx, dskip, dx_planes, ns, B, C, H, W,
                                  slope, BnBwdSumsIn{}, nullptr, S(stream)))
    return e;
  if (dgamma || dbeta) {
    hipLaunchKernelGGL(bn_param_grad_kernel, dim3(cdiv(C, 256)), dim3(256), 0, S(stream), local_dsums ? local_dsums : dsums,
                       dgamma, dbeta, C, accumulate);
    ITCV_CHECK_LAUNCH("itcv_bn_act_bwd_apply(param grads)");
  }
  return 0;
}

int itcv_bn_train_fwd(const float* x, const float* gamma, const float* beta, const float* skip, float* y, void* planes,
                      int ns, int B, int C, int H, int W, float slope, int pool, float eps, float momentum,
                      float* running_mean, float* running_var, int64_t* num_batches_tracked, float* mean, float* rstd,
                      void* ws, size_t ws_bytes, size_t plane_stride, const float* tile_stats, int tiles, int tile_pitch,
                      int groups, void* stream) {
  ITCV_REQUIRE(x && gamma && beta && mean && rstd && (y || planes) && B > 0 && C > 0 && H > 0 && W > 0, "itcv_bn_train_fwd");
  const double px_out = (double)(groups > 1 ? groups : 1) * B * C * (pool ? H * W / 4 : H * W);
  ProfScope bn_prof(S(stream), 13, ilog2_exact(W) >= 0 ? ilog2_exact(W) : 0, C / 8, pool ? 1 : 0, planes ? ns : 0,
                    (double)(groups > 1 ? groups : 1) * B * C * H * W * 4.0 * (skip ? 2 : 1) + px_out * ((planes ? 4.0 : 0.0) + (y ? 4.0 : 0.0)));
  if (groups > 1) ITCV_REQUIRE(!planes || plane_stride, "itcv_bn_train_fwd(groups need the plane stride of the whole tensor)");
  const BnPlan p = bn_plan(false, B, C, H, W, pool, 0, groups, planes != nullptr, ns, plane_stride, ws ? ws_bytes : 0,
                           tile_stats != nullptr);
  if (p.path == BnPath::PerGroup && planes && ns == ITCV_PLANES_F16X2)
    return fail("%s: fp16 planes need the merged group path (no tile statistics, a workspace of itcv_bn_workspace * groups)",
                "itcv_bn_train_fwd");
  if (p.path == BnPath::PerGroup) {
    const BnGrp& s = p.grp;
    for (int g = 0; g < groups; ++g)
      if (int e = itcv_bn_train_fwd(x + g * s.xs, gamma, beta, skip ? skip + g * s.xs : nullptr, y ? y + g * s.os : nullptr,
                                    planes ? static_cast<u32x4*>(planes) + g * s.ps : nullptr, ns, B, C, H, W, slope, pool,
                                    eps, momentum, running_mean, running_var, num_batches_tracked, mean + (size_t)g * C,
                                    rstd + (size_t)g * C, ws, ws_bytes, plane_stride,
                                    tile_stats ? tile_stats + (size_t)g * tiles : nullptr, tiles, tile_pitch, 1, stream))
        return e;
    return 0;
  }
  const BnFinal f{(double)B * H * W, eps, momentum, running_mean, running_var, num_batches_tracked, mean, rstd};
  if (p.path == BnPath::TileStats) {
    ITCV_REQUIRE(tiles > 0 && tile_pitch >= tiles, "itcv_bn_train_fwd(tile statistics)");
    hipLaunchKernelGGL(bn_tile_stats_finalize_kernel, dim3(C), dim3(256), 0, S(stream), tile_stats, tiles, tile_pitch, f.count,
                       eps, momentum, running_mean, running_var, num_batches_tracked, mean, rstd, C);
    ITCV_CHECK_LAUNCH("itcv_bn_train_fwd(tile statistics)");
  } else if (int e = bn_stats_launch(p, x, B, C, H * W, f, ws, ws_bytes, S(stream), "itcv_bn_train_fwd(statistics)")) {
    return e;
  }
  const BnStatsIn fold = p.path == BnPath::SlicedFold
                             ? BnStatsIn{static_cast<const double*>(ws), p.splits, f.count, eps, momentum, running_mean,
                                         running_var, num_batches_tracked, mean, rstd}
                             : BnStatsIn{};
  return bn_fwd_apply_launch(p, x, mean, rstd, gamma, beta, skip, y, planes, ns, B, C, H, W, slope, pool, fold, S(stream));
}

int itcv_bn_train_bwd(const float* x, const float* dy, const float* mean, const float* rstd, const float* gamma,
                      const float* beta, const float* skip, double* dsums, float* dx, float* dskip, void* dx_planes,
                      int ns, float* dgamma, float* dbeta, int accumulate, int B, int C, int H, int W, float slope,
                      int pool, int up2, void* ws, size_t ws_bytes, size_t plane_stride, int groups, void* stream) {
  ITCV_REQUIRE(x && dy && mean && rstd && gamma && beta && dsums && (dx || dx_planes) && B > 0 && C > 0,
               "itcv_bn_train_bwd");
  ITCV_REQUIRE(!(pool && up2), "itcv_bn_train_bwd(pool and up2 are exclusive)");
  const double bn_el = (double)(groups > 1 ? groups : 1) * B * C * H * W;
  ProfScope bn_prof(S(stream), 14, ilog2_exact(W) >= 0 ? ilog2_exact(W) : 0, C / 8, pool ? 1 : (up2 ? 2 : 0), dx_planes ? ns : 0,
                    bn_el * 4.0 * (1.0 + (pool ? 0.25 : (up2 ? 4.0 : 1.0)) + (skip ? 1.0 : 0.0)) +
                        bn_el * ((dx_planes ? 4.0 : 0.0) + (dx ? 4.0 : 0.0) + (dskip ? 4.0 : 0.0)));
  if (groups > 1) ITCV_REQUIRE(!dx_planes || plane_stride, "itcv_bn_train_bwd(groups need the plane stride of the whole tensor)");
  const BnPlan p = bn_plan(true, B, C, H, W, pool, up2, groups, dx_planes != nullptr, ns, plane_stride, ws ? ws_bytes : 0,
                           false);
  const size_t ws_need = p.ws_need;
  if (p.f16 && groups > 1 && (p.path == BnPath::PerGroup || !(ws && ws_bytes >= ws_need)))
    return fail("%s: fp16 gradient planes need the merged group path (W %% 4 == 0, planes, a workspace of itcv_bn_workspace * groups)",
                "itcv_bn_train_bwd");
  if (p.path == BnPath::PerGroup) {
    const BnGrp& s = p.grp;
    for (int g = 0; g < groups; ++g)
      if (int e = itcv_bn_train_bwd(x + g * s.xs, dy + g * s.dys, mean + (size_t)g * C, rstd + (size_t)g * C, gamma, beta,
                                    skip ? skip + g * s.xs : nullptr, dsums + (size_t)g * 2 * C, dx ? dx + g * s.xs : nullptr,
                                    dskip ? dskip + g * s.xs : nullptr,
                                    dx_planes ? static_cast<u32x4*>(dx_planes) + g * s.ps : nullptr, ns, dgamma, dbeta,
                                    (accumulate || g > 0) ? 1 : 0, B, C, H, W, slope, pool, up2, ws, ws_bytes, plane_stride,
                                    1, stream))
        return e;
    return 0;
  }
  if (p.f16) ITCV_REQUIRE(ws && ws_bytes >= ws_need, "itcv_bn_train_bwd(workspace, fp16 planes)");
  if (int e = bn_bwd_reduce_launch(p, x, dy, mean, rstd, gamma, beta, skip, dsums, dgamma, dbeta, accumulate, B, C, H, W, slope,
                                   ws, ws_bytes, S(stream), "itcv_bn_train_bwd(sums)"))
    return e;
  const BnBwdSumsIn fold = p.path == BnPath::SlicedFold
                               ? BnBwdSumsIn{static_cast<const double*>(ws), p.splits, dsums, dgamma, dbeta, accumulate}
                               : BnBwdSumsIn{};
  const float* mx = p.f16 ? reinterpret_cast<const float*>(static_cast<const double*>(ws) + p.part_doubles) : nullptr;
  return bn_bwd_apply_launch(p, x, dy, mean, rstd, gamma, beta, skip, dsums, (double)B * H * W, dx, dskip, dx_planes, ns, B, C,
                             H, W, slope, fold, mx, S(stream));
}

static_assert((int)BnPath::OneBlock == ITCV_BN_PATH_ONE_BLOCK && (int)BnPath::SlicedFold == ITCV_BN_PATH_SLICED_FOLD &&
                  (int)BnPath::SlicedCombine == ITCV_BN_PATH_SLICED_COMBINE && (int)BnPath::Fallback == ITCV_BN_PATH_FALLBACK &&
                  (int)BnPath::PerGroup == ITCV_BN_PATH_PER_GROUP && (int)BnPath::TileStats == ITCV_BN_PATH_TILE_STATS,
              "ITCV_BN_PATH_* follow BnPath");

int itcv_bn_plan_query(int bwd, int B, int C, int H, int W, int pool, int up2, int groups, int planes, int ns,
                       size_t ws_bytes, int tile_stats, int* path, int* splits) {
  ITCV_REQUIRE(B > 0 && C > 0 && H > 0 && W > 0, "itcv_bn_plan_query");
  const BnPlan p = bn_plan(bwd != 0, B, C, H, W, pool, up2, groups, planes != 0, ns, 0, ws_bytes, tile_stats != 0);
  if (path) *path = (int)p.path;
  if (splits) *splits = p.splits;
  return 0;
}

#define ITCV_POINTWISE(NAME, KERNEL, N, ...)                                                        \
  do {                                                                                              \
    if ((N) == 0) return 0;                                                                         \
    hipLaunchKernelGGL(KERNEL, dim3(grid_for(N)), dim3(256), 0, S(stream), __VA_ARGS__);            \
    ITCV_CHECK_LAUNCH(NAME);                                                                        \
    return 0;                                                                                       \
  } while (0)

int itcv_lrelu_fwd(const float* x, float* y, size_t n, float slope, void* stream) {
  ITCV_REQUIRE(x && y, "itcv_lrelu_fwd");
  ITCV_POINTWISE("itcv_lrelu_fwd", lrelu_fwd_kernel, n, x, y, n, slope);
}
int itcv_lrelu_bwd(const float* x, const float* dy, float* dx, size_t n, float slope, void* stream) {
  ITCV_REQUIRE(x && dy && dx, "itcv_lrelu_bwd");
  ITCV_POINTWISE("itcv_lrelu_bwd", lrelu_bwd_kernel, n, x, dy, dx, n, slope);
}
int itcv_sigmoid_fwd(const float* x, float* y, size_t n, void* stream) {
  ITCV_REQUIRE(x && y, "itcv_sigmoid_fwd");
  ITCV_POINTWISE("itcv_sigmoid_fwd", sigmoid_fwd_kernel, n, x, y, n);
}
int itcv_sigmoid_bwd(const float* y, const float* dy, float* dx, size_t n, void* stream) {
  ITCV_REQUIRE(y && dy && dx, "itcv_sigmoid_bwd");
  ITCV_POINTWISE("itcv_sigmoid_bwd", sigmoid_bwd_kernel, n, y, dy, dx, n);
}
int itcv_add(const float* a, const float* b, float* out, size_t n, void* stream) {
  ITCV_REQUIRE(a && b && out, "itcv_add");
  ITCV_POINTWISE("itcv_add", add_kernel, n, a, b, out, n);
}
int itcv_avgpool2_fwd(const float* x, float* y, int BC, int H, int W, void* stream) {
  ITCV_REQUIRE(x && y && BC > 0 && H > 0 && W > 0 && H % 2 == 0 && W % 2 == 0, "itcv_avgpool2_fwd");
  const size_t n = (size_t)BC * (H / 2) * (W / 2);
  ITCV_POINTWISE("itcv_avgpool2_fwd", avgpool2_fwd_kernel, n, x, y, H, W, n);
}
int itcv_avgpool2_bwd(const float* dy, float* dx, int BC, int H, int W, void* stream) {
  ITCV_REQUIRE(dy && dx && BC > 0 && H > 0 && W > 0 && H % 2 == 0 && W % 2 == 0, "itcv_avgpool2_bwd");
  const size_t n = (size_t)BC * H * W;
  ITCV_POINTWISE("itcv_avgpool2_bwd", avgpool2_bwd_kernel, n, dy, dx, H, W, n);
}
int itcv_upsample2_fwd(const float* x, float* y, int BC, int H, int W, void* stream) {
  ITCV_REQUIRE(x && y && BC > 0 && H > 0 && W > 0, "itcv_upsample2_fwd");
  const size_t n = (size_t)BC * H * W * 4;
  ITCV_POINTWISE("itcv_upsample2_fwd", upsample2_fwd_kernel, n, x, y, H, W, n);
}
int itcv_upsample2_bwd(const float* dy, float* dx, int BC, int H, int W, void* stream) {
  ITCV_REQUIRE(dy && dx && BC > 0 && H > 0 && W > 0, "itcv_upsample2_bwd");
  const size_t n = (size_t)BC * H * W;
  ITCV_POINTWISE("itcv_upsample2_bwd", upsample2_bwd_kernel, n, dy, dx, H, W, n);
}

}
```

### intro-tc-vae_amd/hipvae/abi.py

```python
import ctypes
import os
import subprocess

import torch

_HERE = os.path.dirname(os.path.abspath(__file__))
PKG_ROOT = os.path.dirname(_HERE)
LIB_PATH = os.environ.get("ITCV_LIB") or os.path.join(PKG_ROOT, "lib", "libitcv_hip.so")
CSRC = os.path.join(PKG_ROOT, "csrc")
ABI_VERSION = 4

p, i32, i64, sz, f32, f64 = (ctypes.c_void_p, ctypes.c_int, ctypes.c_int64, ctypes.c_size_t,
                             ctypes.c_float, ctypes.c_double)

SIGNATURES = {
    "itcv_abi_version": (i32, []),
    "itcv_last_error": (ctypes.c_char_p, []),
    "itcv_set_option": (i32, [ctypes.c_char_p, i32]),
    "itcv_get_option": (i32, [ctypes.c_char_p]),
    "itcv_profile_begin": (i32, []),
    "itcv_profile_end": (i32, []),
    "itcv_profile_get": (i32, [i32, p, p, p]),
    "itcv_profile_clear": (i32, []),
    "itcv_conv2d_packed_weight_elems": (sz, [i32, i32, i32, i32]),
    "itcv_conv2d_pack_weight": (i32, [p, p, i32, i32, i32, i32, p]),
    "itcv_conv2d_fwd_workspace": (sz, [i32] * 6),
    "itcv_conv2d_fwd": (i32, [p, p, p, p, i32, i32, i32, i32, i32, i32, i32, p, sz, p]),
    "itcv_conv2d_bf16s_supported": (i32, [i32, i32, i32]),
    "itcv_conv2d_packed_weight_bytes_bf16s": (sz, [i32] * 5),
    "itcv_conv2d_pack_weight_bf16s": (i32, [p, p, i32, i32, i32, i32, i32, p]),
    "itcv_pack_desc_bytes": (sz, []),
    "itcv_conv2d_pack_desc_bf16s": (i32, [p, p, p, i32, i32, i32, i32, i32, i32]),
    "itcv_conv2d_pack_weights_bf16s": (i32, [p, i32, i32, i32, p]),
    "itcv_conv2d_fwd_bf16s_workspace": (sz, [i32] * 6),
    "itcv_conv2d_fwd_bf16s": (i32, [p, p, p, p] + [i32] * 8 + [p, sz, p]),
    "itcv_planes_bytes": (sz, [i32] * 4),
    "itcv_split_planes": (i32, [p, p, i32, i32, i32, i32, p]),
    "itcv_absmax": (i32, [p, sz, p, p]),
    "itcv_split_planes_scaled": (i32, [p, p, i32, i32, i32, i32, p, p]),
    "itcv_conv2d_fwd_bf16p_workspace": (sz, [i32] * 7),
    "itcv_conv2d_fwd_bf16p": (i32, [p, p, p, p] + [i32] * 8 + [p, sz, p]),
    "itcv_conv2d_fwd_bf16p_stat_tiles": (i32, [i32] * 7),
    "itcv_conv2d_fwd_bf16p_st": (i32, [p, p, p, p] + [i32] * 8 + [p, p, sz, p]),
    "itcv_conv2d_wgrad_bf16p_supported": (i32, [i32] * 6),
    "itcv_conv2d_wgrad_bf16p_workspace": (sz, [i32] * 6),
    "itcv_conv2d_wgrad_bf16p": (i32, [p, p, p] + [i32] * 9 + [p, sz, p]),
    "itcv_conv2d_wgrad_bf16p_slabs": (i32, [i32] * 6),
    "itcv_wgrad_reduce_desc_bytes": (sz, []),
    "itcv_wgrad_reduce_desc": (i32, [p, p, p, i32, p, i32, i32, i32, i32]),
    "itcv_wgrad_reduce_many": (i32, [p, i32, i32, p]),
    "itcv_wgrad_reduce_max_descs": (i32, []),
    "itcv_linear_workspace": (sz, [i32] * 3),
    "itcv_linear_fwd": (i32, [p, p, p, p, i32, i32, i32, p, sz, p]),
    "itcv_linear_dgrad": (i32, [p, p, p, i32, i32, i32, p, sz, p]),
    "itcv_linear_wgrad": (i32, [p, p, p, i32, i32, i32, i32, p, sz, p]),
    "itcv_conv2d_wgrad5_bf16p_supported": (i32, [i32] * 4),
    "itcv_conv2d_wgrad5_bf16p_workspace": (sz, [i32, i32]),
    "itcv_conv2d_wgrad5_bf16p": (i32, [p, p, p] + [i32] * 6 + [p, i32, p, sz, p]),
    "itcv_conv2d_small_cout_supported": (i32, [i32, i32]),
    "itcv_conv2d_small_cout_bf16p_supported": (i32, [i32, i32, i32]),
    "itcv_conv2d_small_cout_fwd_bf16p": (i32, [p, p, p, p] + [i32] * 8 + [p]),
    "itcv_conv2d_small_cout_fwd": (i32, [p, p, p, p] + [i32] * 7 + [p]),
    "itcv_conv2d_small_cin_supported": (i32, [i32, i32]),
    "itcv_conv2d_small_cin_fwd": (i32, [p, p, p, p] + [i32] * 7 + [p]),
    "itcv_conv2d_small_cin_bf16x3_supported": (i32, [i32, i32, i32, i32]),
    "itcv_conv2d_small_cin_fwd_bf16x3": (i32, [p, p, p, p] + [i32] * 8 + [p, p]),
    "itcv_conv2d_wgrad_bf16s_supported": (i32, [i32] * 5),
    "itcv_conv2d_wgrad_bf16s": (i32, [p, p, p] + [i32] * 8 + [p, sz, p]),
    "itcv_conv2d_wgrad_workspace": (sz, [i32] * 6),
    "itcv_conv2d_wgrad": (i32, [p, p, p, i32, i32, i32, i32, i32, i32, i32, i32, p, sz, p]),
    "itcv_conv2d_fwd_variant": (i32, [i32] * 7),
    "itcv_conv2d_wgrad_variant": (i32, [i32] * 7),
    "itcv_bias_grad_workspace": (sz, [i32, i32, i32]),
    "itcv_bias_grad": (i32, [p, p, i32, i32, i32, i32, p, sz, p]),
    "itcv_bn_workspace": (sz, [i32, i32, i32]),
    "itcv_bn_moments": (i32, [p, p, i32, i32, i32, p, sz, p]),
    "itcv_bn_train_stats": (i32, [p, i32, i32, i32, f32, f32, p, p, p, p, p, p, sz, p]),
    "itcv_bn_finalize": (i32, [p, f64, f32, f32, p, p, p, p, p, i32, p]),
    "itcv_bn_eval_stats": (i32, [p, p, f32, p, p, i32, p]),
    "itcv_bn_act_planes_supported": (i32, [i32] * 4),
    "itcv_bn_act_fwd": (i32, [p, p, p, p, p, p, p, i32, i32, i32, i32, f32, i32, p, i32, sz, p]),
    "itcv_bn_act_bwd_reduce": (i32, [p, p, p, p, p, p, p, p, p, p, i32, i32, i32, i32, i32, f32, i32, i32, p, sz,
                                     p]),
    "itcv_bn_act_bwd_apply": (i32, [p, p, p, p, p, p, p, p, p, f64, p, p, p, p, i32, i32, i32, i32, i32, f32,
                                    i32, i32, p, i32, sz, p]),
    "itcv_bn_train_fwd": (i32, [p, p, p, p, p, p, i32, i32, i32, i32, i32, f32, i32, f32, f32, p, p, p, p, p, p, sz, sz, p, i32, i32,
                                i32, p]),
    "itcv_bn_train_bwd": (i32, [p, p, p, p, p, p, p, p, p, p, p, i32, p, p, i32, i32, i32, i32, i32, f32, i32, i32, p,
                                sz, sz, i32, p]),
    "itcv_bn_plan_query": (i32, [i32] * 10 + [sz, i32, p, p]),
    "itcv_lrelu_fwd": (i32, [p, p, sz, f32, p]),
    "itcv_lrelu_bwd": (i32, [p, p, p, sz, f32, p]),
    "itcv_sigmoid_fwd": (i32, [p, p, sz, p]),
    "itcv_sigmoid_bwd": (i32, [p, p, p, sz, p]),
    "itcv_avgpool2_fwd": (i32, [p, p, i32, i32, i32, p]),
    "itcv_avgpool2_bwd": (i32, [p, p, i32, i32, i32, p]),
    "itcv_upsample2_fwd": (i32, [p, p, i32, i32, i32, p]),
    "itcv_upsample2_bwd": (i32, [p, p, i32, i32, i32, p]),
    "itcv_add": (i32, [p, p, p, sz, p]),
    "itcv_reparam_fwd": (i32, [p, p, p, p, sz, p]),
    "itcv_reparam_bwd": (i32, [p, p, p, p, p, sz, p]),
    "itcv_kl_rows_fwd": (i32, [p, p, p, i32, i32, p]),
    "itcv_kl_rows_bwd": (i32, [p, p, p, p, p, i32, i32, p]),
    "itcv_tc_fwd_workspace": (sz, [i32, i32, i32]),
    "itcv_tc_fwd": (i32, [p, p, p, p, p, p, p, i32, i32, i32, i32, i64, i32, p, sz, p]),
    "itcv_tc_bwd_workspace": (sz, [i32, i32]),
    "itcv_tc_bwd": (i32, [p, p, p, p, p, p, p, p, p, p, i32, i32, i32, i32, i64, i32, p, sz, p]),
    "itcv_tc_kl_fwd": (i32, [p] * 9 + [i32, i32, i32, i32, i64, f32, f32, i32, p, sz, p]),
    "itcv_tc_kl_bwd": (i32, [p] * 10 + [i32, i32, i32, i32, i64, f32, f32, i32, p, sz, p]),
    "itcv_tc_full_fwd_workspace": (sz, [i32, i32, i32]),
    "itcv_tc_full_fwd": (i32, [p, p, p, i32] + [p] * 8 + [i32, i32, i32, i32, i64, f32, f32, f32, i32, p, sz, p]),
    "itcv_tc_full_bwd_workspace": (sz, [i32, i32]),
    "itcv_tc_full_bwd": (i32, [p, p, p, p, i32] + [p] * 7 + [i32, i32, i32, i32, i64, f32, f32, f32, i32, p, sz, p]),
    "itcv_kl_loss_fwd": (i32, [p, p, p, i32, i32, i32, f32, p]),
    "itcv_kl_loss_bwd": (i32, [p, p, p, p, p, i32, i32, i32, f32, p]),
    "itcv_diag_logdensity_rows": (i32, [p, p, p, p, p, i32, i32, p]),
    "itcv_gauss_logdensity_fwd": (i32, [p, p, p, p, p, p, p, p, i32, p]),
    "itcv_gauss_logdensity_bwd": (i32, [p, p, p, p, p, p, p, p, p, p, i32, p]),
    "itcv_sampling_fwd": (i32, [p, p, p, p, p, i32, i32, i64, i32, p]),
    "itcv_sampling_bwd": (i32, [p, p, p, p, p, p, p, i32, i32, i64, i32, p]),
    "itcv_on_off_diag": (i32, [p, p, p, i32, i32, p]),
    "itcv_recon_workspace": (sz, [i32, sz]),
    "itcv_recon_rows_fwd": (i32, [p, p, p, i32, sz, i32, p, sz, p]),
    "itcv_recon_rows_bwd": (i32, [p, p, p, p, i32, sz, i32, p]),
    "itcv_recon_loss_fwd": (i32, [p, p, p, i32, sz, i32, i32, f32, p, sz, p]),
    "itcv_recon_loss_bwd": (i32, [p, p, p, p, i32, sz, i32, i32, f32, p]),
    "itcv_exp_elbo_fwd": (i32, [p, p, p, p, i32, f32, p]),
    "itcv_exp_elbo_bwd": (i32, [p, p, p, p, i32, p]),
    "itcv_lincomb_fwd": (i32, [p, p, i32, p, p]),
    "itcv_lincomb_bwd": (i32, [p, p, i32, p, p]),
    "itcv_sumsq_workspace": (sz, [sz]),
    "itcv_sumsq": (i32, [p, sz, p, p, sz, p]),
    "itcv_clip_coef": (i32, [p, i32, f64, p, p, p]),
    "itcv_scale_by_dev": (i32, [p, sz, p, p]),
    "itcv_adam_step": (i32, [p, p, p, p, sz, f32, f32, f32, f32, i32, p]),
    "itcv_adam_step_dev": (i32, [p, p, p, p, sz, f32, f32, f32, f32, p, p]),
    "itcv_adamx_step_dev": (i32, [p] * 6 + [sz] + [f64] * 5 + [i32, p, p]),
    "itcv_sgd_step_dev": (i32, [p] * 4 + [sz] + [f64] * 4 + [i32, p, p]),
    "itcv_adagrad_step_dev": (i32, [p] * 4 + [sz] + [f64] * 4 + [i32, p, p]),
    "itcv_rmsprop_step_dev": (i32, [p] * 6 + [sz] + [f64] * 5 + [i32, p, p]),
    "itcv_fill": (i32, [p, sz, f32, p]),
    "itcv_hflip": (i32, [p, p, p, i32, i32, i32, p]),
}

TC_VAR_FROM_ROW, TC_EPS_DENSITY, TC_WEIGHTED = 1, 2, 4
TC_LIVE = TC_VAR_FROM_ROW | TC_EPS_DENSITY
BN_PATHS = ("OneBlock", "SlicedFold", "SlicedCombine", "Fallback", "PerGroup", "TileStats")
LOSS_TYPES = {"mse": 0, "l1": 1, "bce": 2}
OPT_MAXIMIZE, OPT_NESTEROV, OPT_AMSGRAD, OPT_DECOUPLED_WD, OPT_CENTERED = 0x1, 0x2, 0x4, 0x8, 0x10


class HipExtensionError(RuntimeError):
    pass


def build(verbose=False):
    out = subprocess.run(["make", "-C", CSRC, "-j4"], capture_output=True, text=True)
    if verbose or out.returncode:
        print(out.stdout[-4000:], out.stderr[-4000:])
    if out.returncode:
        raise HipExtensionError("building libitcv_hip.so failed (see output above)")
    return LIB_PATH


def _load():
    if not os.path.exists(LIB_PATH):
        raise HipExtensionError(
            f"{LIB_PATH} is missing: build it with `make -C {CSRC}` (or __graft_entry__.build()). "
            "There is no CPU fallback for the HIP hot path.")
    lib = ctypes.CDLL(LIB_PATH)
    for name, (res, args) in SIGNATURES.items():
        try:
            fn = getattr(lib, name)
        except AttributeError as e:
            raise HipExtensionError(f"{LIB_PATH} does not export {name}") from e
        fn.restype, fn.argtypes = res, args
    if lib.itcv_abi_version() != ABI_VERSION:
        raise HipExtensionError(f"ABI version mismatch: library {lib.itcv_abi_version()} != binding {ABI_VERSION}")
    return lib


class _Lib:

    _PURE = ("_supported", "_workspace", "_bytes", "_elems", "_variant", "_stat_tiles", "_slabs", "_max_descs")

    def __init__(self, cdll):
        object.__setattr__(self, "_cdll", cdll)

    def __getattr__(self, name):
        fn = getattr(self._cdll, name)
        if name.endswith(self._PURE):
            memo = {}

            def cached(*args, _fn=fn, _memo=memo):
                r = _memo.get(args)
                if r is None:
                    r = _memo[args] = _fn(*args)
                return r

            fn = cached
        object.__setattr__(self, name, fn)
        return fn


lib = _Lib(_load())


def last_error():
    return lib.itcv_last_error().decode()


def check(rc, exc=RuntimeError):
    if rc:
        raise exc(last_error())


def stream():
    return torch._C._cuda_getCurrentRawStream(torch.cuda.current_device())


def ptr(t):
    if t is None:
        return None
    if not t.is_cuda:
        raise HipExtensionError("HIP kernels need device tensors (got a CPU tensor); there is no CPU path")
    if not t.is_contiguous():
        raise HipExtensionError("HIP kernels need contiguous tensors")
    return t.data_ptr()


def call(name, *args):
    check(getattr(lib, name)(*args))


def bn_plan_query(bwd, B, C, H, W, pool=0, up2=0, groups=1, planes=True, ns=2, ws_bytes=None, tile_stats=False):
    if ws_bytes is None:
        ws_bytes = lib.itcv_bn_workspace(B, C, H * W) * max(int(groups), 1)
    path, splits = ctypes.c_int(-1), ctypes.c_int(-1)
    call("itcv_bn_plan_query", int(bool(bwd)), B, C, H, W, int(pool), int(up2), int(groups), int(bool(planes)), int(ns),
         ws_bytes, int(bool(tile_stats)), ctypes.byref(path), ctypes.byref(splits))
    return BN_PATHS[path.value], splits.value
```

### intro-tc-vae_amd/hipvae/functional.py

```python
import contextlib
import weakref

import torch
import torch.distributed as dist
from torch.autograd import Function
from torch.autograd.function import once_differentiable

from . import abi
from .abi import call, lib, ptr, stream

F32 = torch.float32


def set_option(name, value):
    call("itcv_set_option", name.encode(), int(value))


def get_option(name):
    return lib.itcv_get_option(name.encode())


@contextlib.contextmanager
def option_scope(name, value):
    prev = get_option(name)
    set_option(name, value)
    try:
        yield
    finally:
        set_option(name, prev)


def _ws(nbytes, device):
    return torch.empty(max(int(nbytes), 16), dtype=torch.uint8, device=device)


def _f32c(t):
    if t.dtype != F32:
        raise abi.HipExtensionError(f"HIP path is fp32 only (got {t.dtype})")
    return t if t.is_contiguous() else t.contiguous()


_DIRECT = [False]


@contextlib.contextmanager
def direct_grad_accumulation():
    prev, _DIRECT[0] = _DIRECT[0], True
    try:
        yield
    finally:
        _DIRECT[0] = prev


def _grad_target(param):
    g = param.grad if _DIRECT[0] else None
    return g if (g is not None and g.is_contiguous() and g.dtype == F32) else None



_WEIGHT_EPOCH = [0]
_PACK_CACHE = {}


_PARAM_EPOCH = {}


def bump_weight_epoch(params=None):
    if params is None:
        _WEIGHT_EPOCH[0] += 1
        return
    for p in params:
        _PARAM_EPOCH[id(p)] = _PARAM_EPOCH.get(id(p), 0) + 1


_NS = {"fp32": 0, "bf16x3": 2, "bf16x6": 3, "f16x3": 4}
F16X2 = 4
import os as _os

_CONV_MATH = [_os.environ.get("ITCV_CONV_MATH", "fp32")]
assert _CONV_MATH[0] in _NS, "ITCV_CONV_MATH must be one of fp32 / bf16x3 / bf16x6 / f16x3"


def _two(ns):
    return ns in (2, F16X2)


_SMALL_PLANES = [True]
_POISON = [False]
_PLANES = [True]


def set_conv_math(mode):
    assert mode in _NS, mode
    _CONV_MATH[0] = mode


def conv_math():
    return _CONV_MATH[0]


@contextlib.contextmanager
def conv_math_scope(mode):
    if mode is None:
        yield
        return
    assert mode in _NS, mode
    prev, _CONV_MATH[0] = _CONV_MATH[0], mode
    try:
        yield
    finally:
        _CONV_MATH[0] = prev


def _pack_key(weight):
    return (weight.data_ptr(), weight._version, _WEIGHT_EPOCH[0], _PARAM_EPOCH.get(id(weight), 0))


def _pack_entry(weight, key):
    ent = _PACK_CACHE.get(id(weight))
    if ent is None:
        ent = _PACK_CACHE[id(weight)] = [key, {}]
        weakref.finalize(weight, _PACK_CACHE.pop, id(weight), None)
        weakref.finalize(weight, _PARAM_EPOCH.pop, id(weight), None)
    elif ent[0] != key:
        ent[0], ent[1] = key, {}
    return ent


def packed_weight(weight, w4, for_dgrad, ns=0):
    ent = _pack_entry(weight, _pack_key(weight))
    wp = ent[1].get((for_dgrad, ns))
    if wp is None:
        grp = _PACK_GROUPS.get(id(weight)) if ns and _PACK_BATCH[0] else None
        if grp is not None:
            wp = grp.pack(weight, w4, for_dgrad, ns)
        else:
            wp = ent[1][(for_dgrad, ns)] = pack_weight(w4, for_dgrad) if ns == 0 else pack_weight_bf16s(w4, for_dgrad, ns)
    return wp


_PACK_BATCH = [True]
_PACK_GROUPS = {}


class _PackGroup:

    def __init__(self):
        self.members = {}
        self.tables = {}

    def pack(self, weight, w4, for_dgrad, ns):
        k = (for_dgrad, ns)
        mem = self.members.setdefault(k, {})
        rec = mem.get(id(weight))
        if rec is None or rec[2] != w4.data_ptr() or rec[1] != tuple(w4.shape[:3]):
            wp = pack_weight_bf16s(w4, for_dgrad, ns)
            mem[id(weight)] = [weakref.ref(weight), tuple(w4.shape[:3]), w4.data_ptr(), wp]
            self.tables.pop(k, None)
            _pack_entry(weight, _pack_key(weight))[1][k] = wp
            return wp
        stale = [i for i, r in mem.items()
                 if r[0]() is None or r[0]().data_ptr() != r[2] or tuple(r[0]().shape[:3]) != r[1]]
        if stale:
            for i in stale:
                del mem[i]
            self.tables.pop(k, None)
        tab = self.tables.get(k)
        if tab is None:
            tab = self.tables[k] = self._build(mem, for_dgrad, ns, weight.device)
        call("itcv_conv2d_pack_weights_bf16s", ptr(tab[0]), tab[1], tab[2], ns, stream())
        for r in mem.values():
            m = r[0]()
            _pack_entry(m, _pack_key(m))[1][k] = r[3]
        return rec[3]

    @staticmethod
    def _build(mem, for_dgrad, ns, device):
        import ctypes

        nb = lib.itcv_pack_desc_bytes()
        host = (ctypes.c_uint8 * (nb * len(mem)))()
        blocks = 0
        for i, r in enumerate(mem.values()):
            co, ci, ks = r[1]
            got = lib.itcv_conv2d_pack_desc_bf16s(ctypes.byref(host, i * nb), r[2], ptr(r[3]), co, ci, ks, int(for_dgrad), ns,
                                                  blocks)
            if got <= 0:
                raise abi.HipExtensionError("itcv_conv2d_pack_desc_bf16s: " + abi.last_error())
            blocks += got
        dev_table = torch.frombuffer(bytearray(host), dtype=torch.uint8).to(device)
        return dev_table, len(mem), blocks


def register_pack_group(params):
    grp = _PackGroup()
    for p in params:
        if p.dim() == 4:
            _PACK_GROUPS[id(p)] = grp
            weakref.finalize(p, _PACK_GROUPS.pop, id(p), None)
    return grp


def pack_weight_bf16s(w4, for_dgrad, ns):
    co, ci, ks = w4.shape[0], w4.shape[1], w4.shape[2]
    nbytes = lib.itcv_conv2d_packed_weight_bytes_bf16s(co, ci, ks, int(for_dgrad), ns)
    wp = torch.empty(nbytes // 4, dtype=torch.int32, device=w4.device)
    call("itcv_conv2d_pack_weight_bf16s", ptr(w4), ptr(wp), co, ci, ks, int(for_dgrad), ns, stream())
    return wp


_SCIN_MFMA = [True]


def conv_apply(x, weight, w4, for_dgrad, bias, B, Ci, H, W, Co, KS, up2):
    if not up2 and lib.itcv_conv2d_small_cout_supported(Co, KS):
        y = torch.empty((B, Co, H, W), dtype=F32, device=x.device)

        call("itcv_conv2d_small_cout_fwd", ptr(x), ptr(w4), ptr(bias), ptr(y), B, Ci, H, W, Co, KS, int(for_dgrad),
             stream())
        return y
    if not up2 and lib.itcv_conv2d_small_cin_supported(Ci, KS):
        y = torch.empty((B, Co, H, W), dtype=F32, device=x.device)
        fmt = _NS[_CONV_MATH[0]]
        if _SCIN_MFMA[0] and _two(fmt) and lib.itcv_conv2d_small_cin_bf16x3_supported(Ci, Co, KS, W):
            amax = absmax_parts(x) if (fmt == F16X2 and for_dgrad) else None
            call("itcv_conv2d_small_cin_fwd_bf16x3", ptr(x), ptr(w4), ptr(bias), ptr(y), B, Ci, H, W, Co, KS,
                 int(for_dgrad), fmt, ptr(amax), stream())
            return y

        call("itcv_conv2d_small_cin_fwd", ptr(x), ptr(w4), ptr(bias), ptr(y), B, Ci, H, W, Co, KS, int(for_dgrad),
             stream())
        return y
    ns = _NS[_CONV_MATH[0]]
    if ns in (2, 3) and lib.itcv_conv2d_bf16s_supported(Ci, Co, KS):
        wp = packed_weight(weight, w4, for_dgrad, ns)
        y = torch.empty((B, Co, H, W), dtype=F32, device=x.device)
        nws = lib.itcv_conv2d_fwd_bf16s_workspace(B, Ci, H, W, Co, KS)
        ws = _ws(nws, x.device) if nws else None

        call("itcv_conv2d_fwd_bf16s", ptr(x), ptr(wp), ptr(bias), ptr(y), B, Ci, H, W, Co, KS, int(up2), ns, ptr(ws), nws,
             stream())
        return y
    return conv_fwd_raw(x, packed_weight(weight, w4, for_dgrad), bias, B, Ci, H, W, Co, KS, up2)


def absmax_parts(x):
    parts = torch.empty(256, dtype=F32, device=x.device)
    call("itcv_absmax", ptr(x), x.numel(), ptr(parts), stream())
    return parts


def split_planes(x, ns, gradient=False):
    B, C, H, W = x.shape
    nbytes = lib.itcv_planes_bytes(B, C, H * W, ns)
    if not nbytes:
        raise abi.HipExtensionError(f"split_planes: unsupported shape {tuple(x.shape)} / ns={ns}")
    xp = torch.empty(nbytes // 4, dtype=torch.int32, device=x.device)
    if ns == F16X2 and gradient:
        call("itcv_split_planes_scaled", ptr(x), ptr(xp), B, C, H * W, ns, ptr(absmax_parts(x)), stream())
    else:
        call("itcv_split_planes", ptr(x), ptr(xp), B, C, H * W, ns, stream())
    return xp


_FUSE_STATS = [False]


def conv_apply_planes(xp, weight, w4, for_dgrad, bias, B, Ci, H, W, Co, KS, up2, ns, want_stats=False):
    if not up2 and _two(ns) and lib.itcv_conv2d_small_cout_bf16p_supported(Ci, Co, KS):
        y = torch.empty((B, Co, H, W), dtype=F32, device=xp.device)
        call("itcv_conv2d_small_cout_fwd_bf16p", ptr(xp), ptr(w4), ptr(bias), ptr(y), B, Ci, H, W, Co, KS, int(for_dgrad),
             ns, stream())
        return y
    wp = packed_weight(weight, w4, for_dgrad, ns)
    y = torch.empty((B, Co, H, W), dtype=F32, device=xp.device)
    nws = lib.itcv_conv2d_fwd_bf16p_workspace(B, Ci, H, W, Co, KS, ns)
    ws = _ws(nws, xp.device) if nws else None
    T = lib.itcv_conv2d_fwd_bf16p_stat_tiles(B, Ci, H, W, Co, KS, ns) if (want_stats and _FUSE_STATS[0]) else 0
    stats = torch.empty((2, Co, T), dtype=F32, device=xp.device) if T else None
    call("itcv_conv2d_fwd_bf16p_st", ptr(xp), ptr(wp), ptr(bias), ptr(y), B, Ci, H, W, Co, KS, int(up2), ns, ptr(stats),
         ptr(ws), nws, stream())
    if stats is not None:
        y._itcv_tile_stats = (stats, T, 256, y._version, y.data_ptr())
    return y


def _tile_stats_of(x, B, G, HW):
    tag = getattr(x, "_itcv_tile_stats", None)
    if tag is None or tag[3] != x._version or tag[4] != x.data_ptr():
        return None
    stats, T, px = tag[0], tag[1], tag[2]
    if T * px != B * HW or (B // G * HW) % px:
        return None
    return stats, T // G, T


_DEFER = {"on": False, "pending": [], "pool": {}, "tables": {}}


@contextlib.contextmanager
def deferred_wgrad_reduces():
    prev, _DEFER["on"] = _DEFER["on"], True
    try:
        yield
    finally:
        _DEFER["on"] = prev
        if not prev:
            flush_wgrad_reduces()


def flush_wgrad_reduces():
    pend = _DEFER["pending"]
    if not pend:
        return
    import ctypes
    groups = {}
    for ws, dw, co, ci, slabs in pend:
        groups.setdefault(dw.data_ptr(), [dw, co, ci, []])[3].append((ws, slabs))
    key = tuple((k, tuple((w.data_ptr(), n) for w, n in g[3])) for k, g in groups.items())
    tab = _DEFER["tables"].get(key)
    if tab is None:
        nb = lib.itcv_wgrad_reduce_desc_bytes()
        descs, blocks = [], 0
        for dw, co, ci, srcs in groups.values():
            for c0 in range(0, len(srcs), 4):
                part = srcs[c0:c0 + 4]
                descs.append((dw, co, ci, part, 1))
        host = (ctypes.c_uint8 * (nb * len(descs)))()
        for i, (dw, co, ci, part, acc) in enumerate(descs):
            sl = (ctypes.c_void_p * len(part))(*[w.data_ptr() for w, _ in part])
            sp = (ctypes.c_int * len(part))(*[n for _, n in part])
            got = lib.itcv_wgrad_reduce_desc(ctypes.byref(host, i * nb), sl, sp, len(part), dw.data_ptr(), co, ci, acc, blocks)
            if got <= 0:
                raise abi.HipExtensionError("itcv_wgrad_reduce_desc: " + abi.last_error())
            blocks += got
        if len(descs) != len(groups):
            raise abi.HipExtensionError("deferred weight-gradient reduce: more than four passes over one weight")
        if len(_DEFER["tables"]) > 64:
            _DEFER["tables"].clear()
        tab = _DEFER["tables"][key] = (torch.frombuffer(bytearray(host), dtype=torch.uint8).to(pend[0][1].device), len(descs), blocks)
    call("itcv_wgrad_reduce_many", ptr(tab[0]), tab[1], tab[2], stream())
    pend.clear()


def _defer_slab_buffer(nbytes, device):
    k = (len(_DEFER["pending"]), int(nbytes), str(device))
    buf = _DEFER["pool"].get(k)
    if buf is None:
        buf = _DEFER["pool"][k] = torch.empty(max(int(nbytes), 16), dtype=torch.uint8, device=device)
    return buf


def conv_wgrad_planes(xp, dyp, B, Ci, H, W, Co, KS, up2, out=None, accumulate=False, ns=2):
    dw = out if out is not None else torch.empty((Co, Ci, KS, KS), dtype=F32, device=xp.device)
    nws = lib.itcv_conv2d_wgrad_bf16p_workspace(B, Ci, H, W, Co, KS)
    if _DEFER["on"] and out is not None and accumulate:
        same = sum(1 for p in _DEFER["pending"] if p[1].data_ptr() == dw.data_ptr())
        if same >= 4 or (same == 0 and len({p[1].data_ptr() for p in _DEFER["pending"]}) >= lib.itcv_wgrad_reduce_max_descs()):
            flush_wgrad_reduces()
        ws = _defer_slab_buffer(nws, xp.device)
        call("itcv_conv2d_wgrad_bf16p", ptr(xp), ptr(dyp), ptr(dw), B, Ci, H, W, Co, KS, int(up2), int(ns), 2, ptr(ws), nws,
             stream())
        _DEFER["pending"].append((ws, dw, Co, Ci, lib.itcv_conv2d_wgrad_bf16p_slabs(B, Ci, H, W, Co, KS)))
        return dw
    ws = _ws(nws, xp.device)

    call("itcv_conv2d_wgrad_bf16p", ptr(xp), ptr(dyp), ptr(dw), B, Ci, H, W, Co, KS, int(up2), int(ns), int(accumulate),
         ptr(ws), nws, stream())
    return dw


def pack_weight(w4, for_dgrad):
    co, ci, ks = w4.shape[0], w4.shape[1], w4.shape[2]
    wp = torch.empty(lib.itcv_conv2d_packed_weight_elems(co, ci, ks, for_dgrad), dtype=F32, device=w4.device)
    call("itcv_conv2d_pack_weight", ptr(w4), ptr(wp), co, ci, ks, int(for_dgrad), stream())
    return wp


class LaunchProfile:
    KINDS = {0: "conv_fwd_kernel", 1: "conv_fwd_bf16s_kernel", 2: "conv_wgrad_kernel", 3: "conv_wgrad_bf16s_kernel",
             4: "conv_small_cout_kernel", 5: "conv_small_cin_kernel", 6: "conv_fwd_bf16p_kernel",
             7: "conv_wgrad_bf16p_kernel", 8: "conv_fwd_bf16p2_kernel", 9: "conv_fwd_bf16p3_kernel",
             10: "conv_small_cout_planes_kernel", 11: "conv_small_cin_mfma_kernel", 12: "conv_wgrad5_planes_kernel",
             13: "bn_act_fwd_planes_kernel", 14: "bn_bwd_apply_planes"}
    HBM_KINDS = (13, 14)

    @classmethod
    def begin(cls):
        call("itcv_profile_begin")

    @classmethod
    def end(cls):
        import ctypes
        n = lib.itcv_profile_end()
        code, flop, ms = ctypes.c_int(), ctypes.c_double(), ctypes.c_float()
        out = []
        for i in range(n):
            call("itcv_profile_get", i, ctypes.byref(code), ctypes.byref(flop), ctypes.byref(ms))
            c = code.value
            kind, ks, bm, up2, ns = c & 15, (c >> 4) & 15, (c >> 8) & 255, (c >> 16) & 1, (c >> 20) & 15
            if kind in (0, 2):
                label = f"{cls.KINDS[kind]}<KS={ks},BM={bm},up2={up2}>"
            elif kind in (7, 8, 9):
                label = f"{cls.KINDS[kind]}<LOG2W={ks},BM={bm},up2={up2},NS={ns}>"
            elif kind in (1, 3, 6):
                label = f"{cls.KINDS[kind]}<KS={ks},BM={bm},up2={up2},NS={ns}>"
            elif kind in cls.HBM_KINDS:
                label = f"{cls.KINDS[kind]}<C={8 * bm},W={1 << ks},mode={(c >> 16) & 15},NS={ns}>"
            elif kind in (10, 11, 12):
                label = f"{cls.KINDS[kind]}<KS={ks},C={bm},stem={up2},NS={ns}>"
            else:
                label = f"{cls.KINDS[kind]}<KS={ks},C={bm}>"
            out.append((label, flop.value, ms.value * 1e-3))
        call("itcv_profile_clear")
        return out


def conv_fwd_raw(x, wp, bias, B, Ci, H, W, Co, KS, up2):
    y = torch.empty((B, Co, H, W), dtype=F32, device=x.device)
    nws = lib.itcv_conv2d_fwd_workspace(B, Ci, H, W, Co, KS)
    ws = _ws(nws, x.device) if nws else None

    call("itcv_conv2d_fwd", ptr(x), ptr(wp), ptr(bias), ptr(y), B, Ci, H, W, Co, KS, int(up2), ptr(ws), nws, stream())
    return y


def conv_wgrad_raw(x, dy, B, Ci, H, W, Co, KS, up2, out=None, accumulate=False):
    dw = out if out is not None else torch.empty((Co, Ci, KS, KS), dtype=F32, device=x.device)
    nws = lib.itcv_conv2d_wgrad_workspace(B, Ci, H, W, Co, KS)
    ws = _ws(nws, x.device)
    ns = _NS[_CONV_MATH[0]]
    if ns in (2, 3) and lib.itcv_conv2d_wgrad_bf16s_supported(Ci, H, W, Co, KS):
        if up2:
            xu = torch.empty((B, Ci, H, W), dtype=F32, device=x.device)
            call("itcv_upsample2_fwd", ptr(x), ptr(xu), B * Ci, H // 2, W // 2, stream())
            x = xu

        call("itcv_conv2d_wgrad_bf16s", ptr(x), ptr(dy), ptr(dw), B, Ci, H, W, Co, KS, ns, int(accumulate), ptr(ws), nws,
             stream())
        return dw

    call("itcv_conv2d_wgrad", ptr(x), ptr(dy), ptr(dw), B, Ci, H, W, Co, KS, int(up2), int(accumulate), ptr(ws), nws,
         stream())
    return dw


def bias_grad_raw(dy, B, C, HW, target=None):
    db = target if target is not None else torch.empty((C,), dtype=F32, device=dy.device)
    nws = lib.itcv_bias_grad_workspace(B, C, HW)
    ws = _ws(nws, dy.device)
    call("itcv_bias_grad", ptr(dy), ptr(db), B, C, HW, int(target is not None), ptr(ws), nws, stream())
    return None if target is not None else db


PLANES_STATS = [0, 0]


def _tag_planes(t, planes, ns, fp32_valid=True):
    t._itcv_planes = (planes, ns, t._version, t.data_ptr(), fp32_valid)


def _require_fp32(t, what):
    tag = getattr(t, "_itcv_planes", None)
    if tag is not None and not tag[4]:
        raise abi.HipExtensionError(f"{what}: this tensor was produced as planes only (fp32 values not written)")
    return t


def _tagged_planes(t, ns):
    tag = getattr(t, "_itcv_planes", None)
    if tag is None or tag[1] != ns or tag[2] != t._version or tag[3] != t.data_ptr():
        return None
    return tag[0]


def planes_of(t, ns, gradient=False):
    p = _tagged_planes(t, ns)
    PLANES_STATS[0 if p is not None else 1] += 1
    return p if p is not None else split_planes(t, ns, gradient)


def conv_input_planes_ns(conv, up2=False):
    if conv is None:
        return 0
    return _planes_ns(conv.in_channels, conv.out_channels, conv.kernel_size[0], up2)


def conv_grad_planes_ns(conv, needs_input_grad=True):
    if conv is None:
        return 0
    ks = conv.kernel_size[0]
    ns = _planes_ns(conv.out_channels, conv.in_channels, ks, False) if needs_input_grad else 0
    if not ns and _two(_NS[_CONV_MATH[0]]) and _PLANES[0] and (ks == 3 or (ks == 5 and _SMALL_PLANES[0]
                                                                           and conv.in_channels <= 3
                                                                           and conv.out_channels == 64)):
        ns = _NS[_CONV_MATH[0]]
    return ns


def conv_input_mode(conv, B, H, W, up2=False):
    ns = conv_input_planes_ns(conv, up2)
    if not ns:
        return 0, True
    ks = conv.kernel_size[0]
    wg_ok = (_wgrad_planes_ok(B, conv.in_channels, H, W, conv.out_channels, ks)
             or _wgrad5_mode(conv.in_channels, H, W, conv.out_channels, ks, up2) == "predict")
    return ns, not (_two(ns) and wg_ok)


def conv_grad_mode(conv, B, H, W, needs_input_grad=True):
    ns = conv_grad_planes_ns(conv, needs_input_grad)
    if not ns:
        return 0, True
    ks = conv.kernel_size[0]
    dgrad_ok = (not needs_input_grad) or _planes_ns(conv.out_channels, conv.in_channels, ks, False) == ns
    wgrad_ok = _two(ns) and _wgrad_planes_ok(B, conv.in_channels, H, W, conv.out_channels, ks)
    return ns, not (dgrad_ok and wgrad_ok and conv.bias is None)


def _planes_ns(Ci, Co, KS, up2):
    ns = _NS[_CONV_MATH[0]]
    if not ns or not _PLANES[0]:
        return 0
    if not up2 and _two(ns) and _SMALL_PLANES[0] and lib.itcv_conv2d_small_cout_bf16p_supported(Ci, Co, KS):
        return ns
    if not up2 and (lib.itcv_conv2d_small_cout_supported(Co, KS) or lib.itcv_conv2d_small_cin_supported(Ci, KS)):
        return 0
    return ns if lib.itcv_conv2d_bf16s_supported(Ci, Co, KS) else 0


def _wgrad5_mode(Ci, H, W, Co, KS, up2):
    if up2 or KS != 5 or not _two(_NS[_CONV_MATH[0]]) or not (_PLANES[0] and _SMALL_PLANES[0]):
        return None
    if Ci <= 3 and lib.itcv_conv2d_wgrad5_bf16p_supported(Ci, Co, H, W):
        return "stem"
    if Co <= 3 and lib.itcv_conv2d_wgrad5_bf16p_supported(Co, Ci, H, W):
        return "predict"
    return None


def conv_wgrad5_planes(small, big_planes, B, Cs, H, W, stem, out=None, accumulate=False, ns=2):
    dw = out if out is not None else torch.empty((64, Cs, 5, 5) if stem else (Cs, 64, 5, 5), dtype=F32, device=small.device)
    nws = lib.itcv_conv2d_wgrad5_bf16p_workspace(B, H)
    ws = _ws(nws, small.device)

    amax = absmax_parts(small) if (ns == F16X2 and not stem) else None
    call("itcv_conv2d_wgrad5_bf16p", ptr(small), ptr(big_planes), ptr(dw), B, Cs, H, W, int(stem), int(ns), ptr(amax),
         int(accumulate), ptr(ws), nws, stream())
    return dw


def _wgrad_planes_ok(B, Ci, H, W, Co, KS):
    return bool(_two(_NS[_CONV_MATH[0]]) and _PLANES[0] and lib.itcv_conv2d_wgrad_bf16p_supported(B, Ci, H, W, Co, KS))


class Conv2dFn(Function):

    @staticmethod
    def forward(ctx, x, weight, bias, up2):
        x, weight = _f32c(x), _f32c(weight)
        B, Ci, Hs, Ws = x.shape
        Co, KS = weight.shape[0], weight.shape[2]
        H, W = (Hs * 2, Ws * 2) if up2 else (Hs, Ws)
        b = None if bias is None else _f32c(bias)
        ns = _planes_ns(Ci, Co, KS, up2)
        xp = None
        if ns:
            xp = planes_of(x, ns)
            y = conv_apply_planes(xp, weight, weight, 0, b, B, Ci, H, W, Co, KS, up2, ns, want_stats=True)
        else:
            y = conv_apply(_require_fp32(x, "Conv2dFn.forward"), weight, weight, 0, b, B, Ci, H, W, Co, KS, up2)
        wg_planes = _wgrad_planes_ok(B, Ci, H, W, Co, KS)
        keep_xp = xp if (_two(ns) and (wg_planes or _wgrad5_mode(Ci, H, W, Co, KS, up2) == "predict")) else None
        ctx.save_for_backward(None if keep_xp is not None else _require_fp32(x, "Conv2dFn.forward (saved input)"),
                              weight, bias, keep_xp)
        ctx.cfg = (B, Ci, H, W, Co, KS, up2, bias is not None, (Hs, Ws))
        return y

    @staticmethod
    @once_differentiable
    def backward(ctx, dy):
        x, weight, bias, xp = ctx.saved_tensors
        B, Ci, H, W, Co, KS, up2, has_bias, (Hs, Ws) = ctx.cfg
        dy = _f32c(dy)
        dx = dw = db = None
        ns_d = _planes_ns(Co, Ci, KS, False) if ctx.needs_input_grad[0] else 0
        wg_planes = ctx.needs_input_grad[1] and _wgrad_planes_ok(B, Ci, H, W, Co, KS)
        dyp = None
        fmt2 = F16X2 if _NS[_CONV_MATH[0]] == F16X2 else 2
        if ns_d or wg_planes:
            dyp = planes_of(dy, ns_d if ns_d else fmt2, gradient=True)
        if ctx.needs_input_grad[0]:
            if ns_d:
                dx = conv_apply_planes(dyp, weight, weight, 1, None, B, Co, H, W, Ci, KS, False, ns_d)
            else:
                dx = conv_apply(_require_fp32(dy, "Conv2dFn.backward"), weight, weight, 1, None, B, Co, H, W, Ci, KS, False)
            if up2:
                lo = torch.empty((B, Ci, H // 2, W // 2), dtype=F32, device=dy.device)
                call("itcv_upsample2_bwd", ptr(dx), ptr(lo), B * Ci, H // 2, W // 2, stream())
                dx = lo
        wg5 = _wgrad5_mode(Ci, H, W, Co, KS, up2) if ctx.needs_input_grad[1] else None
        if wg5 == "predict" and xp is None and x is None:
            wg5 = None
        if wg5 is not None:
            tgt = _grad_target(weight)
            if wg5 == "stem":
                small, big = _require_fp32(x, "Conv2dFn.backward (5x5 weight gradient)"), (dyp if dyp is not None else planes_of(dy, fmt2, gradient=True))
            else:
                small, big = _require_fp32(dy, "Conv2dFn.backward (5x5 weight gradient)"), (xp if xp is not None else split_planes(x, fmt2))
            cs = Ci if wg5 == "stem" else Co
            if tgt is not None:
                conv_wgrad5_planes(small, big, B, cs, H, W, wg5 == "stem", out=tgt, accumulate=True, ns=fmt2)
            else:
                dw = conv_wgrad5_planes(small, big, B, cs, H, W, wg5 == "stem", ns=fmt2)
        elif ctx.needs_input_grad[1]:
            tgt = _grad_target(weight)
            if wg_planes and (ns_d in (0, fmt2)):
                if xp is None:
                    xp = split_planes(x, fmt2)
                if tgt is not None:
                    conv_wgrad_planes(xp, dyp, B, Ci, H, W, Co, KS, up2, out=tgt, accumulate=True, ns=fmt2)
                else:
                    dw = conv_wgrad_planes(xp, dyp, B, Ci, H, W, Co, KS, up2, ns=fmt2)
            else:
                if x is None:
                    raise abi.HipExtensionError("Conv2dFn.backward: conv math mode changed between forward and backward")
                _require_fp32(dy, "Conv2dFn.backward (weight gradient)")
                if tgt is not None:
                    conv_wgrad_raw(x, dy, B, Ci, H, W, Co, KS, up2, out=tgt, accumulate=True)
                else:
                    dw = conv_wgrad_raw(x, dy, B, Ci, H, W, Co, KS, up2)
        if has_bias and ctx.needs_input_grad[2]:
            db = bias_grad_raw(_require_fp32(dy, "Conv2dFn.backward (bias gradient)"), B, Co, H * W, _grad_target(bias))
        return dx, dw, db, None


class LinearFn(Function):

    @staticmethod
    def forward(ctx, x, weight, bias):
        x, weight = _f32c(x), _f32c(weight)
        B, K = x.shape
        N = weight.shape[0]
        y = torch.empty((B, N), dtype=F32, device=x.device)
        nws = lib.itcv_linear_workspace(B, K, N)
        ws = _ws(nws, x.device) if nws else None
        call("itcv_linear_fwd", ptr(x), ptr(weight), ptr(None if bias is None else _f32c(bias)), ptr(y), B, K, N, ptr(ws),
             nws, stream())
        ctx.save_for_backward(x, weight, bias)
        ctx.cfg = (B, K, N, bias is not None)
        return y

    @staticmethod
    @once_differentiable
    def backward(ctx, dy):
        x, weight, bias = ctx.saved_tensors
        B, K, N, has_bias = ctx.cfg
        dy = _f32c(dy)
        dx = dw = db = None
        nws = lib.itcv_linear_workspace(B, K, N)
        if ctx.needs_input_grad[0]:
            dx = torch.empty((B, K), dtype=F32, device=dy.device)
            ws = _ws(nws, dy.device) if nws else None
            call("itcv_linear_dgrad", ptr(dy), ptr(weight), ptr(dx), B, K, N, ptr(ws), nws, stream())
        if ctx.needs_input_grad[1]:
            tgt = _grad_target(weight)
            dw = None if tgt is not None else torch.empty((N, K), dtype=F32, device=dy.device)
            ws = _ws(nws, dy.device) if nws else None
            call("itcv_linear_wgrad", ptr(dy), ptr(x), ptr(tgt if tgt is not None else dw), B, K, N,
                 int(tgt is not None), ptr(ws), nws, stream())
        if has_bias and ctx.needs_input_grad[2]:
            db = bias_grad_raw(dy, B, N, 1, _grad_target(bias))
        return dx, dw, db


def _world(group):
    return dist.get_world_size(group) if (group is not None and dist.is_initialized()) else 1


class BnActFn(Function):

    @staticmethod
    def forward(ctx, x, gamma, beta, skip, running_mean, running_var, nbt, eps, momentum, slope, pool, training,
                group, out_planes=0, grad_planes=0, out_fp32=True, grad_fp32=True, bn_groups=1):
        x, gamma, beta = _f32c(x), _f32c(gamma), _f32c(beta)
        skip = None if skip is None else _f32c(skip)
        B, C, H, W = x.shape
        G = int(bn_groups) if training else 1
        if G < 1 or B % G:
            raise abi.HipExtensionError(f"BatchNorm groups: batch {B} is not {G} equal passes")
        Bg = B // G
        dev = x.device
        mean = torch.empty((G, C), dtype=F32, device=dev)
        rstd = torch.empty((G, C), dtype=F32, device=dev)
        world = _world(group) if training else 1
        oshape = (B, C, H // 2, W // 2) if pool else (B, C, H, W)
        y = torch.empty(oshape, dtype=F32, device=dev)
        yp, pstride = None, 0
        if F16X2 in (out_planes, grad_planes) and not (training and world == 1):
            out_planes = 0 if out_planes == F16X2 else out_planes
            grad_planes = 0 if grad_planes == F16X2 else grad_planes
            out_fp32 = grad_fp32 = True
        if out_planes and lib.itcv_bn_act_planes_supported(C, H, W, int(pool)):
            yp = torch.empty(lib.itcv_planes_bytes(B, C, oshape[2] * oshape[3], out_planes) // 4, dtype=torch.int32,
                             device=dev)
            pstride = B * (C // 8) * oshape[2] * oshape[3]
        write_y = out_fp32 or yp is None or _POISON[0]
        nws = lib.itcv_bn_workspace(Bg, C, H * W) * G
        ts = _tile_stats_of(x, B, G, H * W) if (training and world == 1) else None
        if training and world == 1:
            ws = _ws(nws, dev)
            call("itcv_bn_train_fwd", ptr(x), ptr(gamma), ptr(beta), ptr(skip), ptr(y) if write_y else None, ptr(yp),
                 int(out_planes), Bg, C, H, W, float(slope), int(pool), float(eps), float(momentum), ptr(running_mean),
                 ptr(running_var), ptr(nbt), ptr(mean), ptr(rstd), ptr(ws), nws, pstride,
                 None if ts is None else ts[0].data_ptr(), ts[1] if ts else 0, ts[2] if ts else 0, G, stream())
        for g in (range(G) if not (training and world == 1) else ()):
            r = slice(g * Bg, (g + 1) * Bg)
            xg, yg = x[r], (y[r] if write_y else None)
            sg = None if skip is None else skip[r]
            ypg = None if yp is None else yp[g * Bg * (C // 8) * oshape[2] * oshape[3] * 4:]
            if training:
                ws = _ws(nws, dev)
                sums = torch.empty((2 * C,), dtype=torch.float64, device=dev)
                call("itcv_bn_moments", ptr(xg), ptr(sums), Bg, C, H * W, ptr(ws), nws, stream())
                dist.all_reduce(sums, group=group)
                call("itcv_bn_finalize", ptr(sums), float(Bg * H * W * world), float(eps), float(momentum),
                     ptr(running_mean), ptr(running_var), ptr(nbt), ptr(mean[g]), ptr(rstd[g]), C, stream())
            else:
                call("itcv_bn_eval_stats", ptr(running_mean), ptr(running_var), float(eps), ptr(mean[g]), ptr(rstd[g]), C,
                     stream())
            call("itcv_bn_act_fwd", ptr(xg), ptr(mean[g]), ptr(rstd[g]), ptr(gamma), ptr(beta), ptr(sg), ptr(yg), Bg, C, H, W,
                 float(slope), int(pool), ptr(ypg), int(out_planes), pstride, stream())
        if yp is not None:
            if _POISON[0] and not out_fp32:
                y.fill_(float("nan"))
            _tag_planes(y, yp, out_planes, bool(out_fp32))
        ctx.save_for_backward(x, gamma, beta, mean, rstd, skip)
        ctx.params = (gamma, beta)
        if not lib.itcv_bn_act_planes_supported(C, H, W, 0):
            grad_planes = 0
        ctx.cfg = (B, C, H, W, float(slope), int(pool), bool(training), group, world, int(grad_planes),
                   bool(grad_fp32) or not grad_planes, G)
        ctx.mark_non_differentiable(*[t for t in (running_mean, running_var, nbt) if t is not None])
        return y

    @staticmethod
    @once_differentiable
    def backward(ctx, dy):
        x, gamma, beta, mean, rstd, skip = ctx.saved_tensors
        B, C, H, W, slope, pool, training, group, world, grad_planes, grad_fp32, G = ctx.cfg
        if not training:
            raise abi.HipExtensionError("BatchNorm backward in eval mode is not part of the training hot path")
        dy = _f32c(dy)
        dev = x.device
        Bg = B // G
        nws = lib.itcv_bn_workspace(Bg, C, H * W) * G
        tg = _grad_target(gamma) if ctx.needs_input_grad[1] else None
        tb = _grad_target(beta) if ctx.needs_input_grad[2] else None
        direct = tg is not None and tb is not None
        dgamma = dbeta = None
        if direct:
            pg, pb = tg, tb
        else:
            dgamma = torch.empty_like(gamma) if ctx.needs_input_grad[1] else None
            dbeta = torch.empty_like(beta) if ctx.needs_input_grad[2] else None
            pg, pb = dgamma, dbeta
        dx = torch.empty_like(x)
        dskip = torch.empty_like(x) if (skip is not None and ctx.needs_input_grad[3]) else None
        dxp, pstride = None, 0
        if grad_planes:
            dxp = torch.empty(lib.itcv_planes_bytes(B, C, H * W, grad_planes) // 4, dtype=torch.int32, device=dev)
            pstride = B * (C // 8) * H * W
        write_dx = grad_fp32 or dxp is None or _POISON[0]
        if world == 1:
            ws = _ws(nws, dev)
            local = torch.empty((G, 2 * C), dtype=torch.float64, device=dev)
            call("itcv_bn_train_bwd", ptr(x), ptr(dy), ptr(mean), ptr(rstd), ptr(gamma), ptr(beta), ptr(skip), ptr(local),
                 ptr(dx) if write_dx else None, ptr(dskip), ptr(dxp), grad_planes, ptr(pg), ptr(pb), 1 if direct else 0, Bg,
                 C, H, W, slope, pool, 0, ptr(ws), nws, pstride, G, stream())
        for g in (range(G) if world != 1 else ()):
            r = slice(g * Bg, (g + 1) * Bg)
            acc = 1 if (direct or g > 0) else 0
            xg, dyg = x[r], dy[r]
            sg = None if skip is None else skip[r]
            dxg = dx[r] if write_dx else None
            dsg = None if dskip is None else dskip[r]
            dxpg = None if dxp is None else dxp[g * Bg * (C // 8) * H * W * 4:]
            ws = _ws(nws, dev)
            local = torch.empty((2 * C,), dtype=torch.float64, device=dev)
            call("itcv_bn_act_bwd_reduce", ptr(xg), ptr(dyg), ptr(mean[g]), ptr(rstd[g]), ptr(gamma), ptr(beta), ptr(sg),
                 ptr(local), ptr(pg), ptr(pb), acc, Bg, C, H, W, slope, pool, 0, ptr(ws), nws, stream())
            total = local.clone()
            dist.all_reduce(total, group=group)
            call("itcv_bn_act_bwd_apply", ptr(xg), ptr(dyg), ptr(mean[g]), ptr(rstd[g]), ptr(gamma), ptr(beta), ptr(sg),
                 ptr(total), None, float(Bg * H * W * world), ptr(dxg), ptr(dsg), None, None, 0, Bg, C, H, W, slope,
                 pool, 0, ptr(dxpg), grad_planes, pstride, stream())
        if dxp is not None:
            if _POISON[0] and not grad_fp32:
                dx.fill_(float("nan"))
            _tag_planes(dx, dxp, grad_planes, bool(grad_fp32))
        return (dx, dgamma, dbeta, dskip) + (None,) * 14


class LeakyReluFn(Function):
    @staticmethod
    def forward(ctx, x, slope):
        x = _f32c(x)
        y = torch.empty_like(x)
        call("itcv_lrelu_fwd", ptr(x), ptr(y), x.numel(), float(slope), stream())
        ctx.save_for_backward(x)
        ctx.slope = float(slope)
        return y

    @staticmethod
    @once_differentiable
    def backward(ctx, dy):
        (x,) = ctx.saved_tensors
        dy = _f32c(dy)
        dx = torch.empty_like(x)
        call("itcv_lrelu_bwd", ptr(x), ptr(dy), ptr(dx), x.numel(), ctx.slope, stream())
        return dx, None


class SigmoidFn(Function):
    @staticmethod
    def forward(ctx, x):
        x = _f32c(x)
        y = torch.empty_like(x)
        call("itcv_sigmoid_fwd", ptr(x), ptr(y), x.numel(), stream())
        ctx.save_for_backward(y)
        return y

    @staticmethod
    @once_differentiable
    def backward(ctx, dy):
        (y,) = ctx.saved_tensors
        dy = _f32c(dy)
        dx = torch.empty_like(y)
        call("itcv_sigmoid_bwd", ptr(y), ptr(dy), ptr(dx), y.numel(), stream())
        return dx


class AvgPool2Fn(Function):
    @staticmethod
    def forward(ctx, x):
        x = _f32c(x)
        B, C, H, W = x.shape
        y = torch.empty((B, C, H // 2, W // 2), dtype=F32, device=x.device)
        call("itcv_avgpool2_fwd", ptr(x), ptr(y), B * C, H, W, stream())
        ctx.shape = (B, C, H, W)
        return y

    @staticmethod
    @once_differentiable
    def backward(ctx, dy):
        B, C, H, W = ctx.shape
        dy = _f32c(dy)
        dx = torch.empty((B, C, H, W), dtype=F32, device=dy.device)
        call("itcv_avgpool2_bwd", ptr(dy), ptr(dx), B * C, H, W, stream())
        return dx


class Upsample2Fn(Function):
    @staticmethod
    def forward(ctx, x):
        x = _f32c(x)
        B, C, H, W = x.shape
        y = torch.empty((B, C, 2 * H, 2 * W), dtype=F32, device=x.device)
        call("itcv_upsample2_fwd", ptr(x), ptr(y), B * C, H, W, stream())
        ctx.shape = (B, C, H, W)
        return y

    @staticmethod
    @once_differentiable
    def backward(ctx, dy):
        B, C, H, W = ctx.shape
        dy = _f32c(dy)
        dx = torch.empty((B, C, H, W), dtype=F32, device=dy.device)
        call("itcv_upsample2_bwd", ptr(dy), ptr(dx), B * C, H, W, stream())
        return dx


class AddFn(Function):
    @staticmethod
    def forward(ctx, a, b):
        a, b = _f32c(a), _f32c(b)
        out = torch.empty_like(a)
        call("itcv_add", ptr(a), ptr(b), ptr(out), a.numel(), stream())
        return out

    @staticmethod
    def backward(ctx, g):
        return g, g


class ReparamFn(Function):

    @staticmethod
    def forward(ctx, mu, logvar, eps):
        mu, logvar, eps = _f32c(mu), _f32c(logvar), _f32c(eps)
        z = torch.empty_like(mu)
        call("itcv_reparam_fwd", ptr(mu), ptr(logvar), ptr(eps), ptr(z), mu.numel(), stream())
        ctx.save_for_backward(logvar, eps)
        return z

    @staticmethod
    @once_differentiable
    def backward(ctx, dz):
        logvar, eps = ctx.saved_tensors
        dz = _f32c(dz)
        dmu, dlv = torch.empty_like(dz), torch.empty_like(dz)
        call("itcv_reparam_bwd", ptr(dz), ptr(logvar), ptr(eps), ptr(dmu), ptr(dlv), dz.numel(), stream())
        return dmu, dlv, None


class KlRowsFn(Function):

    @staticmethod
    def forward(ctx, logvar, mu):
        logvar, mu = _f32c(logvar), _f32c(mu)
        B, D = logvar.shape
        kl = torch.empty((B,), dtype=F32, device=mu.device)
        call("itcv_kl_rows_fwd", ptr(logvar), ptr(mu), ptr(kl), B, D, stream())
        ctx.save_for_backward(logvar, mu)
        return kl

    @staticmethod
    @once_differentiable
    def backward(ctx, g):
        logvar, mu = ctx.saved_tensors
        B, D = logvar.shape
        g = _f32c(g)
        dlv, dmu = torch.empty_like(logvar), torch.empty_like(mu)
        call("itcv_kl_rows_bwd", ptr(g), ptr(logvar), ptr(mu), ptr(dlv), ptr(dmu), B, D, stream())
        return dlv, dmu


_REDUCTION = {"none": 0, "sum": 1, "mean": 2}


class KlLossFn(Function):

    @staticmethod
    def forward(ctx, logvar, mu, reduction, scale):
        logvar, mu = _f32c(logvar), _f32c(mu)
        B, D = logvar.shape
        out = torch.empty((B,) if reduction == 0 else (), dtype=F32, device=mu.device)
        call("itcv_kl_loss_fwd", ptr(logvar), ptr(mu), ptr(out), B, D, reduction, float(scale), stream())
        ctx.save_for_backward(logvar, mu)
        ctx.cfg = (B, D, reduction, float(scale))
        return out

    @staticmethod
    @once_differentiable
    def backward(ctx, g):
        logvar, mu = ctx.saved_tensors
        B, D, reduction, scale = ctx.cfg
        dlv, dmu = torch.empty_like(logvar), torch.empty_like(mu)
        call("itcv_kl_loss_bwd", ptr(_f32c(g)), ptr(logvar), ptr(mu), ptr(dlv), ptr(dmu), B, D, reduction, scale, stream())
        return dlv, dmu, None, None


class TcKlFn(Function):

    @staticmethod
    def forward(ctx, z, mu_all, logvar, dataset_size, row_offset, coef_tc, coef_kl, reduction):
        z, mu_all, logvar = _f32c(z), _f32c(mu_all), _f32c(logvar)
        Bl, D = z.shape
        Bt = mu_all.shape[0]
        dev = z.device
        out = torch.empty((Bl,) if reduction == 0 else (), dtype=F32, device=dev)
        rows = torch.empty((Bl,), dtype=F32, device=dev) if reduction else None
        prodm = torch.empty((Bl,), dtype=F32, device=dev)
        logqz = torch.empty((Bl,), dtype=F32, device=dev)
        lse = torch.empty((Bl, D), dtype=F32, device=dev)
        sjoint = torch.empty((Bl, Bt), dtype=F32, device=dev)
        nws = lib.itcv_tc_fwd_workspace(Bl, Bt, D)
        ws = _ws(nws, dev)
        call("itcv_tc_kl_fwd", ptr(z), ptr(mu_all), ptr(logvar), ptr(out), ptr(rows), ptr(prodm), ptr(logqz), ptr(lse),
             ptr(sjoint), Bl, Bt, int(row_offset), D, int(dataset_size), float(coef_tc), float(coef_kl), reduction, ptr(ws),
             nws, stream())
        ctx.save_for_backward(z, mu_all, logvar, logqz, lse, sjoint)
        ctx.cfg = (int(dataset_size), int(row_offset), float(coef_tc), float(coef_kl), reduction)
        return out

    @staticmethod
    @once_differentiable
    def backward(ctx, g):
        z, mu_all, logvar, logqz, lse, sjoint = ctx.saved_tensors
        n, off, ctc, ckl, reduction = ctx.cfg
        Bl, D = z.shape
        Bt = mu_all.shape[0]
        dz, dlv, dmu = torch.empty_like(z), torch.empty_like(logvar), torch.empty_like(mu_all)
        nws = lib.itcv_tc_bwd_workspace(Bl, Bt)
        ws = _ws(nws, z.device)
        call("itcv_tc_kl_bwd", ptr(_f32c(g)), ptr(z), ptr(mu_all), ptr(logvar), ptr(logqz), ptr(lse), ptr(sjoint), ptr(dz),
             ptr(dmu), ptr(dlv), Bl, Bt, off, D, n, ctc, ckl, reduction, ptr(ws), nws, stream())
        return dz, dmu, dlv, None, None, None, None, None


def _packed_pair(a, b):
    Bt, D = a.shape
    if a.is_contiguous() and b.is_contiguous():
        return D
    if (a.stride() == b.stride() == (2 * D, 1) and b.data_ptr() == a.data_ptr() + D * a.element_size()
            and a.dtype == b.dtype == F32):
        return 2 * D
    return None


class TcFullFn(Function):

    @staticmethod
    def forward(ctx, z, mu_all, logvar_all, dataset_size, row_offset, alpha, beta, gamma, reduction):
        z = _f32c(z)
        if not (mu_all.is_cuda and logvar_all.is_cuda):
            raise abi.HipExtensionError("HIP kernels need device tensors (got a CPU tensor); there is no CPU path")
        ld = _packed_pair(mu_all, logvar_all)
        if ld is None or ld == mu_all.shape[1]:
            mu_all, logvar_all = _f32c(mu_all), _f32c(logvar_all)
            ld = mu_all.shape[1]
        Bl, D = z.shape
        Bt = mu_all.shape[0]
        if tuple(mu_all.shape) != (Bt, D) or tuple(logvar_all.shape) != (Bt, D):
            raise ValueError(f"mu_all / logvar_all must be [Bt, {D}] (got {tuple(mu_all.shape)}, {tuple(logvar_all.shape)})")
        dev = z.device
        out = torch.empty((Bl,) if reduction == 0 else (), dtype=F32, device=dev)
        rows = torch.empty((Bl,), dtype=F32, device=dev) if reduction else None
        comps = torch.empty((3, Bl), dtype=F32, device=dev)
        prodm = torch.empty((Bl,), dtype=F32, device=dev)
        logqz = torch.empty((Bl,), dtype=F32, device=dev)
        lse = torch.empty((Bl, D), dtype=F32, device=dev)
        sjoint = torch.empty((Bl, Bt), dtype=F32, device=dev)
        ivar = torch.empty((Bt, D), dtype=F32, device=dev)
        nws = lib.itcv_tc_full_fwd_workspace(Bl, Bt, D)
        ws = _ws(nws, dev)
        call("itcv_tc_full_fwd", ptr(z), mu_all.data_ptr(), logvar_all.data_ptr(), ld, ptr(out), ptr(rows), ptr(comps),
             ptr(prodm), ptr(logqz), ptr(lse), ptr(sjoint), ptr(ivar), Bl, Bt, int(row_offset), D, int(dataset_size),
             float(alpha), float(beta), float(gamma), reduction, ptr(ws), nws, stream())
        ctx.save_for_backward(z, mu_all, logvar_all, logqz, lse, sjoint, ivar)
        ctx.cfg = (int(dataset_size), int(row_offset), float(alpha), float(beta), float(gamma), reduction, ld)
        ctx.mark_non_differentiable(comps)
        return out, comps

    @staticmethod
    @once_differentiable
    def backward(ctx, g, _g_comps):
        z, mu_all, logvar_all, logqz, lse, sjoint, ivar = ctx.saved_tensors
        n, off, a, b, c, reduction, ld = ctx.cfg
        Bl, D = z.shape
        Bt = mu_all.shape[0]
        dz = torch.empty_like(z)
        if ld == D:
            dmu, dlv = torch.empty((Bt, D), dtype=F32, device=z.device), torch.empty((Bt, D), dtype=F32, device=z.device)
        else:
            dpk = torch.empty((Bt, 2 * D), dtype=F32, device=z.device)
            dmu, dlv = dpk[:, :D], dpk[:, D:]
        nws = lib.itcv_tc_full_bwd_workspace(Bl, Bt)
        ws = _ws(nws, z.device)
        call("itcv_tc_full_bwd", ptr(_f32c(g)), ptr(z), mu_all.data_ptr(), logvar_all.data_ptr(), ld, ptr(logqz), ptr(lse),
             ptr(sjoint), ptr(ivar), ptr(dz), dmu.data_ptr(), dlv.data_ptr(), Bl, Bt, off, D, n, a, b, c, reduction,
             ptr(ws), nws, stream())
        return dz, dmu, dlv, None, None, None, None, None, None


class ReconLossFn(Function):

    @staticmethod
# ... 229 lines not shown
```

### intro-tc-vae_amd/solvers/intro.py

```python
from typing import Optional

import torch
from torch import Tensor

from hipvae import ddp
from hipvae.functional import ExpElboFn
from models import bn_groups
from ops import noise, reparameterize
from solvers.vae import VAESolver


class IntroSolver(VAESolver):
    def __init__(self, dataset, model, batch_size: int, optimizer_e, optimizer_d, recon_loss_type: str,
                 beta_kl: float, beta_rec: float, beta_neg: float, gamma_r: float, device: torch.device,
                 use_amp: bool, grad_scaler, writer=None, test_iter: int = 1000, clip: Optional[float] = None):
        super().__init__(dataset, model, batch_size, optimizer_e, optimizer_d, recon_loss_type, beta_kl, beta_rec,
                         device, use_amp, grad_scaler, writer, test_iter, clip)
        self.beta_neg = beta_neg
        self.gamma_r = gamma_r
        self.batch_passes = True

    def _exp_elbo(self, rec_rows: Tensor, kl_rows: Tensor) -> Tensor:
        while rec_rows.dim() > 1:
            rec_rows = rec_rows.sum(-1)
        if rec_rows.is_cuda and rec_rows.shape == kl_rows.shape and rec_rows.dim() == 1:
            return ExpElboFn.apply(rec_rows, kl_rows, -2 * self.scale)
        return (-2 * self.scale * (rec_rows + kl_rows)).exp().mean()

    def _device_step(self, real: Tensor) -> Tensor:
        if not self.batch_passes:
            return self._device_step_unbatched(real)
        model, scale = self.model, self.scale
        cat = torch.cat

        def two():
            return bn_groups(2)

        noise_batch = noise((real.size(0), model.zdim), self.device)
        self._set_trainable(encoder=True, decoder=False)
        real_mu, real_logvar = model.encode(real)
        z = reparameterize(real_mu, real_logvar)
        with two():
            fake, rec = model.decoder(cat([noise_batch, z])).chunk(2)
        loss_rec = self.compute_rec_loss(real, rec, reduction="mean")
        loss_e_real_kl = self.compute_kl_loss(z, real_mu, real_logvar, write=True)
        with two():
            mu2, logvar2 = model.encode(cat([rec.detach(), fake.detach()]))
        (rec_mu, fake_mu), (rec_logvar, fake_logvar) = mu2.chunk(2), logvar2.chunk(2)
        z_rec = reparameterize(rec_mu, rec_logvar)
        z_fake = reparameterize(fake_mu, fake_logvar)
        with two():
            rec_rec, rec_fake = model.decoder(cat([z_rec, z_fake])).chunk(2)
        kl_rec = self.compute_kl_loss(z_rec, rec_mu, rec_logvar, reduce="none", beta=self.beta_neg)
        kl_fake = self.compute_kl_loss(z_fake, fake_mu, fake_logvar, reduce="none", beta=self.beta_neg)
        expelbo_rec = self._exp_elbo(self.compute_rec_loss(rec, rec_rec, reduction="none"), kl_rec)
        expelbo_fake = self._exp_elbo(self.compute_rec_loss(fake, rec_fake, reduction="none"), kl_fake)
        loss_e = self._lincomb((scale, scale, 0.25, 0.25), loss_rec, loss_e_real_kl, expelbo_rec, expelbo_fake)
        finish_average = self._backward(loss_e, ("encoder",), defer_average=True)

        self._set_trainable(encoder=False, decoder=True)
        with two():
            fake, rec = model.decoder(cat([noise_batch, z.detach()])).chunk(2)
        finish_average()
        norm_e = self._clip()
        self._step("encoder")
        loss_rec = self.compute_rec_loss(real, rec, reduction="mean", write=True)
        with two():
            mu2, logvar2 = model.encode(cat([rec, fake]))
        (rec_mu, fake_mu), (rec_logvar, fake_logvar) = mu2.chunk(2), logvar2.chunk(2)
        z_rec = reparameterize(rec_mu, rec_logvar)
        z_fake = reparameterize(fake_mu, fake_logvar)
        with two():
            rec_rec, rec_fake = model.decoder(cat([z_rec.detach(), z_fake.detach()])).chunk(2)
        g = self.gamma_r * self.beta_rec
        loss_rec_rec = self.compute_rec_loss(rec.detach(), rec_rec, reduction="mean", beta=g)
        loss_fake_rec = self.compute_rec_loss(fake.detach(), rec_fake, reduction="mean", beta=g)
        loss_d_rec_kl = self.compute_kl_loss(z_rec, rec_mu, rec_logvar)
        loss_d_fake_kl = self.compute_kl_loss(z_fake, fake_mu, fake_logvar)
        loss_d = self._lincomb((scale, 0.5 * scale, 0.5 * scale, 0.5 * scale, 0.5 * scale), loss_rec, loss_d_rec_kl,
                               loss_d_fake_kl, loss_rec_rec, loss_fake_rec)
        self._backward(loss_d, ("decoder",))
        norm_d = self._clip()
        self._step("decoder")

        stats = torch.stack([loss_e.detach(), loss_d.detach(), loss_e_real_kl.detach(), loss_rec.detach(),
                             expelbo_fake.detach(), loss_d_fake_kl.detach()])
        ddp.mean_scalars_(stats)
        zero = stats.new_zeros(1)
        self._last_fake = fake.detach() if self.writer else None
        return torch.cat([stats, norm_e if norm_e is not None else zero, norm_d if norm_d is not None else zero])

    def _device_step_unbatched(self, real: Tensor) -> Tensor:
        model, scale = self.model, self.scale
        noise_batch = noise((real.size(0), model.zdim), self.device)
        self._set_trainable(encoder=True, decoder=False)
        fake = model.sample(noise_batch)
        real_mu, real_logvar = model.encode(real)
        z = reparameterize(real_mu, real_logvar)
        rec = model.decoder(z)
        loss_rec = self.compute_rec_loss(real, rec, reduction="mean")
        loss_e_real_kl = self.compute_kl_loss(z, real_mu, real_logvar, write=True)
        rec_mu, rec_logvar, z_rec, rec_rec = model(rec.detach())
        fake_mu, fake_logvar, z_fake, rec_fake = model(fake.detach())
        kl_rec = self.compute_kl_loss(z_rec, rec_mu, rec_logvar, reduce="none", beta=self.beta_neg)
        kl_fake = self.compute_kl_loss(z_fake, fake_mu, fake_logvar, reduce="none", beta=self.beta_neg)
        expelbo_rec = self._exp_elbo(self.compute_rec_loss(rec, rec_rec, reduction="none"), kl_rec)
        expelbo_fake = self._exp_elbo(self.compute_rec_loss(fake, rec_fake, reduction="none"), kl_fake)
        loss_e = self._lincomb((scale, scale, 0.25, 0.25), loss_rec, loss_e_real_kl, expelbo_rec, expelbo_fake)
        finish_average = self._backward(loss_e, ("encoder",), defer_average=True)

        self._set_trainable(encoder=False, decoder=True)
        fake = model.sample(noise_batch)
        rec = model.decoder(z.detach())
        finish_average()
        norm_e = self._clip()
        self._step("encoder")
        loss_rec = self.compute_rec_loss(real, rec, reduction="mean", write=True)
        rec_mu, rec_logvar = model.encode(rec)
        z_rec = reparameterize(rec_mu, rec_logvar)
        fake_mu, fake_logvar = model.encode(fake)
        z_fake = reparameterize(fake_mu, fake_logvar)
        rec_rec = model.decode(z_rec.detach())
        rec_fake = model.decode(z_fake.detach())
        g = self.gamma_r * self.beta_rec
        loss_rec_rec = self.compute_rec_loss(rec.detach(), rec_rec, reduction="mean", beta=g)
        loss_fake_rec = self.compute_rec_loss(fake.detach(), rec_fake, reduction="mean", beta=g)
        loss_d_rec_kl = self.compute_kl_loss(z_rec, rec_mu, rec_logvar)
        loss_d_fake_kl = self.compute_kl_loss(z_fake, fake_mu, fake_logvar)
        loss_d = self._lincomb((scale, 0.5 * scale, 0.5 * scale, 0.5 * scale, 0.5 * scale), loss_rec, loss_d_rec_kl,
                               loss_d_fake_kl, loss_rec_rec, loss_fake_rec)
        self._backward(loss_d, ("decoder",))
        norm_d = self._clip()
        self._step("decoder")

        stats = torch.stack([loss_e.detach(), loss_d.detach(), loss_e_real_kl.detach(), loss_rec.detach(),
                             expelbo_fake.detach(), loss_d_fake_kl.detach()])
        ddp.mean_scalars_(stats)
        zero = stats.new_zeros(1)
        self._last_fake = fake.detach() if self.writer else None
        return torch.cat([stats, norm_e if norm_e is not None else zero, norm_d if norm_d is not None else zero])

    def train_step(self, batch: Tensor, cur_iter: int) -> dict:
        if batch.dim() == 3:
            batch = batch.unsqueeze(0)
        real = batch.to(self.device)
        v_e, v_d, v_kl, v_rec, v_expf, v_dfkl, v_ne, v_nd = self._run(real).tolist()
        if v_e != v_e or v_d != v_d:
            raise RuntimeError
        if self.writer:
            self.write_scalars(cur_iter, losses=dict(r_loss=v_rec, kl_loss=v_kl, expelbo_f=v_expf),
                               diff_kl=v_dfkl - v_kl)
            if self.clip:
                self.writer.add_scalars("total_norm", {"E": v_ne, "D": v_nd}, global_step=cur_iter)
            self.writer.add_scalar("lossE", v_e, global_step=cur_iter)
            self.writer.add_scalar("lossD", v_d, global_step=cur_iter)
            self.write_gradient_norm(cur_iter)
            self.write_images(real, self._last_fake, cur_iter)
            self.write_disentanglemnt_scores(cur_iter)
            self.writer.flush()
        return {"loss_enc": v_e, "loss_dec": v_d, "loss_kl": v_kl, "loss_rec": v_rec,
                "L2": max(v_ne, v_nd) if self.clip else None}
```

### intro-tc-vae_amd/solvers/vae.py

```python
from typing import Optional

import torch
from torch import Tensor

from hipvae import ddp
from hipvae.functional import LinCombFn, conv_math_scope, deferred_wgrad_reduces, direct_grad_accumulation
from hipvae.flat import FlatGroup, clip_grad_norm, fused_update
from models import grad_free_parameters
from ops import kl_divergence, reconstruction_loss
from utils import SingletonWriter

try:
    from dataset import DisentanglementDataset
except Exception:
    class DisentanglementDataset:
        pass


class VAESolver:
    def __init__(self, dataset, model, batch_size: int, optimizer_e, optimizer_d, recon_loss_type: str,
                 beta_kl: float, beta_rec: float, device: torch.device, use_amp: bool, grad_scaler,
                 writer=None, test_iter: int = 1000, clip: Optional[float] = None):
        self.dataset = dataset
        if isinstance(dataset, DisentanglementDataset):
            try:
                from evaluation.generator import LatentGenerator
                self.latent_generator = LatentGenerator(dataset, device)
            except Exception:
                self.latent_generator = None
        self.model = model
        self.batch_size = batch_size
        self.optimizer_e, self.optimizer_d = optimizer_e, optimizer_d
        self.beta_kl, self.beta_rec = beta_kl, beta_rec
        self.device = device
        self.use_amp, self.grad_scaler = use_amp, grad_scaler
        import os as _os
        self.conv_math = _os.environ.get("ITCV_CONV_MATH") or ("f16x3" if use_amp else "fp32")
        self.writer, self.test_iter, self.clip = writer, test_iter, clip
        self.recon_loss_type = recon_loss_type
        self.scale = 1 / (self.model.cdim * self.model.encoder.image_size ** 2)
        self._flat = {}

    def compute_kl_loss(self, z: Optional[Tensor], mu: Tensor, logvar: Tensor, reduce: str = "mean",
                        beta: float = None, write: bool = False) -> Tensor:
        if beta is None:
            beta = self.beta_kl
        if not (write and self.writer):
            return kl_divergence(logvar, mu, reduce=reduce, scale=beta)
        kl = kl_divergence(logvar, mu, reduce=reduce)
        self.write_scalar(SingletonWriter().cur_iter, "kl_loss_unscaled", kl)
        return beta * kl

    def compute_rec_loss(self, x, recon_x, reduction="sum", beta: float = None, write: bool = False) -> Tensor:
        if beta is None:
            beta = self.beta_rec
        if not (write and self.writer):
            return reconstruction_loss(x, recon_x, self.recon_loss_type, reduction, scale=beta)
        rec = reconstruction_loss(x, recon_x, self.recon_loss_type, reduction)
        self.write_scalar(SingletonWriter().cur_iter, "r_loss_unscaled", rec)
        return beta * rec

    @staticmethod
    def _lincomb(weights, *terms):
        if all(isinstance(t, Tensor) and t.numel() == 1 and t.is_cuda for t in terms):
            return LinCombFn.apply(tuple(weights), *terms)
        return sum(w * t for w, t in zip(weights, terms))

    def _params(self, part):
        mod = getattr(self.model, part)
        ent = self.__dict__.setdefault("_plists", {}).get(part)
        if ent is None or ent[0] is not mod:
            ent = self._plists[part] = (mod, list(mod.parameters()))
        return ent[1]

    def _group(self, part) -> FlatGroup:
        params = self._params(part)
        g = self._flat.get(part)
        if g is None or not g.owns(params):
            g = self._flat[part] = FlatGroup(params, inherit=g,
                                             grad_free=grad_free_parameters(getattr(self.model, part)))
        return g

    def _set_trainable(self, encoder: bool, decoder: bool):
        for p in self._params("encoder"):
            p.requires_grad = encoder
        for p in self._params("decoder"):
            p.requires_grad = decoder

    def _backward(self, loss, parts, defer_average=False):
        groups = [self._group(p) for p in parts]
        for g in groups:
            g.zero_grad()
        with direct_grad_accumulation(), deferred_wgrad_reduces():
            loss.backward()
        if defer_average:
            pending = [ddp.average_async(g.flat_g) for g in groups]
            return lambda: [f() for f in pending]
        for g in groups:
            ddp.average_(g.flat_g)
        return None

    def _clip(self):
        if not self.clip:
            return None
        return clip_grad_norm([self._group("encoder"), self._group("decoder")], self.clip)

    def _step(self, part):
        opt = self.optimizer_e if part == "encoder" else self.optimizer_d
        spec = fused_update(opt)
        if spec is None:
            opt.step()
        else:
            g = self._group(part)
            g.bind_optimizer(opt, spec)
            g.fused_step(spec)

    def enable_graph(self, flag: bool = True):
        self._graph_on = bool(flag)
        self._graph = None
        self._graphs, self._graph_warm = {}, {}
        return self

    def _graph_ok(self, specs=None):
        import ops
        if not (getattr(self, "_graph_on", False) and self.writer is None
                and (ddp.get() is None or ddp.graph_capturable())
                and ops._noise["queue"] is None and ops._noise["mode"] == "device"):
            return False
        if specs is None:
            specs = (fused_update(self.optimizer_e), fused_update(self.optimizer_d))
        return specs[0] is not None and specs[1] is not None

    def _run(self, real: Tensor) -> Tensor:
        with conv_math_scope(self.conv_math):
            return self._run_scoped(real)

    def _run_scoped(self, real: Tensor) -> Tensor:
        specs = (fused_update(self.optimizer_e), fused_update(self.optimizer_d)) if getattr(self, "_graph_on", False) \
            else None
        if not self._graph_ok(specs):
            return self._device_step(real)
        key = (tuple(real.shape), real.dtype, self.conv_math) + specs + (getattr(self, "kl_loss", None),)
        from hipvae.functional import bump_weight_epoch
        graphs = self.__dict__.setdefault("_graphs", {})
        ent = graphs.get(key)
        if ent is None:
            warm = self.__dict__.setdefault("_graph_warm", {})
            warm[key] = warm.get(key, 0) + 1
            if warm[key] <= (3 if not graphs else 1):
                return self._device_step(real)
            while len(graphs) >= 4:
                graphs.pop(next(iter(graphs)))
            ent = dict(inp=real.clone())
            bump_weight_epoch()
            torch.cuda.synchronize()
            ent["graph"] = torch.cuda.CUDAGraph()
            ddp.drain_pending_collectives()
            mode = "thread_local"
            with torch.cuda.graph(ent["graph"], capture_error_mode=mode):
                ent["out"] = self._device_step(ent["inp"])
            graphs[key] = ent
        self._graph, self._graph_key, self._graph_in, self._graph_out = ent["graph"], key, ent["inp"], ent["out"]
        ent["inp"].copy_(real)
        ent["graph"].replay()
        bump_weight_epoch()
        return ent["out"]

    def _device_step(self, real: Tensor) -> Tensor:
        self._set_trainable(True, True)
        mu, logvar, z, rec = self.model(real)
        loss_rec = self.compute_rec_loss(real, rec, reduction="mean", write=True)
        loss_kl = self.compute_kl_loss(z, mu, logvar, write=True)
        loss = self._lincomb((self.scale, self.scale), loss_rec, loss_kl)
        self._backward(loss, ("decoder", "encoder"))
        norm = self._clip()
        self._step("encoder")
        self._step("decoder")
        stats = torch.stack([loss.detach(), loss_kl.detach(), loss_rec.detach()])
        ddp.mean_scalars_(stats)
        return torch.cat([stats, norm if norm is not None else stats.new_zeros(1)])

    def train_step(self, batch: Tensor, cur_iter: int) -> dict:
        if batch.dim() == 3:
            batch = batch.unsqueeze(0)
        real = batch.to(self.device)
        v_loss, v_kl, v_rec, v_norm = self._run(real).tolist()
        if v_loss != v_loss:
            raise RuntimeError
        if self.writer:
            self.write_scalars(cur_iter, losses=dict(r_loss=v_rec, kl_loss=v_kl))
            if self.clip:
                self.writer.add_scalar("total_norm", v_norm, global_step=cur_iter)
            self.write_gradient_norm(cur_iter)
            self._write_images_helper(real, cur_iter)
            self.write_disentanglemnt_scores(cur_iter)
            self.writer.flush()
        return {"loss_enc": v_loss, "loss_dec": v_loss, "loss_kl": v_kl, "loss_rec": v_rec,
                "L2": v_norm if self.clip else None}

    def _write_images_helper(self, batch, cur_iter):
        if self.writer is not None and cur_iter % self.test_iter == 0:
            noise = torch.randn(size=(batch.size(0), self.model.zdim), device=self.device)
            with torch.no_grad():
                fake = self.model.sample(noise)
            self.write_images(batch, fake, cur_iter)

    def write_images(self, batch, fake_batch, cur_iter):
        if self.writer is not None and cur_iter % self.test_iter == 0:
            with torch.no_grad():
                _, _, _, rec_det = self.model(batch, deterministic=True)
            k = min(batch.size(0), 16)
            grid = torch.cat([batch[:k], rec_det[:k], fake_batch[:k]], dim=0).data.cpu()
            self.writer.add_images("reconstructions", grid, global_step=cur_iter)

    def write_gradient_norm(self, cur_iter: int):
        grads = [p.grad.detach().norm(2) for p in self.model.encoder.fc.parameters() if p.grad is not None]
        if grads:
            self.writer.add_scalar("fc_grad_norm", torch.stack(grads).norm(2).item(), global_step=cur_iter)

    def write_scalar(self, cur_iter: int, tag: str, value: Tensor):
        if self.writer and value.dim() == 0:
            self.writer.add_scalar(tag, value.data.item(), global_step=cur_iter)

    def write_scalars(self, cur_iter: int, losses: dict, **kwargs):
        if self.writer is not None:
            self.write_losses(cur_iter, losses)
            for name, value in kwargs.items():
                self.writer.add_scalar(name, value, global_step=cur_iter)

    def write_losses(self, cur_iter: int, losses: dict):
        if self.writer is not None:
            self.writer.add_scalars("losses", losses, global_step=cur_iter)

    def write_disentanglemnt_scores(self, cur_iter: int, num_samples: int = 10000):
        if self.writer is None or not isinstance(self.dataset, DisentanglementDataset) or cur_iter % self.test_iter:
            return
        try:
            from evaluation import metrics as M
        except Exception:
            return
        was_training = self.model.training
        self.model.eval()
        n = num_samples if len(self.dataset) >= num_samples else len(self.dataset) // 2
        kw = dict(latent_generator=self.latent_generator, model=self.model, num_samples=n, batch_size=self.batch_size)
        for fn in (M.write_bvae_score, M.write_dci_score, M.write_mig_score, M.write_mod_expl_score):
            fn(self.writer, cur_iter, **kw)
        if was_training:
            self.model.train()

    def write_gradient_flow(self, cur_iter, named_parameters):
        return None
```

Measured before the change: 4048 images/s.

## Share decoder forward pass between encoder and decoder updates with BN stat replay

The second decoder forward pass on the same inputs is dropped. The first pass is recorded with decoder params trainable and its graph is retained for the decoder backward. Batch-norm running-stat updates from the skipped pass are replayed by a new batched kernel that uses saved per-group mean and unbiased variance, so running statistics match the two-pass schedule. The risk is higher memory from the retained graph, plus extra bookkeeping to suppress param grads during the encoder backward and input grads during the decoder backward.

```diff
diff --git a/include/itcv_hip.h b/include/itcv_hip.h
--- a/include/itcv_hip.h
+++ b/include/itcv_hip.h
@@ -107,6 +107,9 @@
 int itcv_bn_finalize(const double* sums, double count, float eps, float momentum, float* running_mean,
                      float* running_var, int64_t* num_batches_tracked, float* mean, float* rstd, int C,
                      void* stream);
+int itcv_bn_finalize_uv(const double* sums, double count, float eps, float momentum, float* running_mean,
+                        float* running_var, int64_t* num_batches_tracked, float* mean, float* rstd, float* unbiased_var,
+                        int C, void* stream);
 int itcv_bn_eval_stats(const float* running_mean, const float* running_var, float eps, float* mean,
                        float* rstd, int C, void* stream);
 int itcv_bn_act_fwd(const float* x, const float* mean, const float* rstd, const float* gamma,
@@ -128,6 +131,16 @@
                       float* running_mean, float* running_var, int64_t* num_batches_tracked, float* mean, float* rstd,
                       void* ws, size_t ws_bytes, size_t plane_stride, const float* tile_stats, int tiles, int tile_pitch,
                       int groups, void* stream);
+int itcv_bn_train_fwd_uv(const float* x, const float* gamma, const float* beta, const float* skip, float* y, void* planes,
+                         int ns, int B, int C, int H, int W, float slope, int pool, float eps, float momentum,
+                         float* running_mean, float* running_var, int64_t* num_batches_tracked, float* mean, float* rstd,
+                         float* unbiased_var, void* ws, size_t ws_bytes, size_t plane_stride, const float* tile_stats,
+                         int tiles, int tile_pitch, int groups, void* stream);
+size_t itcv_bn_replay_desc_bytes(void);
+int itcv_bn_replay_desc(void* host_desc, float* running_mean, float* running_var, int64_t* num_batches_tracked,
+                        const float* mean, const float* unbiased_var, int C, int groups, float momentum, int block0);
+int itcv_bn_replay_many(const void* dev_table, int n, int total_blocks, void* stream);
+int itcv_bn_replay_max_descs(void);
 int itcv_bn_train_bwd(const float* x, const float* dy, const float* mean, const float* rstd, const float* gamma,
                       const float* beta, const float* skip, double* dsums, float* dx, float* dskip, void* dx_planes,
                       int ns, float* dgamma, float* dbeta, int accumulate, int B, int C, int H, int W, float slope,
diff --git a/intro-tc-vae_amd/csrc/norm_act.hip b/intro-tc-vae_amd/csrc/norm_act.hip
--- a/intro-tc-vae_amd/csrc/norm_act.hip
+++ b/intro-tc-vae_amd/csrc/norm_act.hip
@@ -27,19 +27,28 @@
   int64_t* nbt;
   float* mean;
   float* rstd;
+  float* uvar;
 };
 
+__device__ __forceinline__ float bn_blend(float r, float s, float momentum) {
+  float a = (1.f - momentum) * r, b = momentum * s;
+  asm volatile("" : "+v"(a), "+v"(b));
+  return a + b;
+}
+
 __device__ __forceinline__ void bn_finalize(double s1, double s2, double count, float eps, float momentum,
-                                            float* running_mean, float* running_var, int c, float& mean_c, float& rstd_c) {
+                                            float* running_mean, float* running_var, int c, float& mean_c, float& rstd_c,
+                                            float* uvar_c = nullptr) {
   const double m = s1 / count;
   double var = s2 / count - m * m;
   if (var < 0.0) var = 0.0;
   mean_c = (float)m;
   rstd_c = (float)(1.0 / sqrt(var + (double)eps));
-  if (running_mean) running_mean[c] = (1.f - momentum) * running_mean[c] + momentum * (float)m;
+  if (running_mean) running_mean[c] = bn_blend(running_mean[c], (float)m, momentum);
   if (running_var) {
     const double unbiased = count > 1.0 ? var * count / (count - 1.0) : var;
-    running_var[c] = (1.f - momentum) * running_var[c] + momentum * (float)unbiased;
+    running_var[c] = bn_blend(running_var[c], (float)unbiased, momentum);
+    if (uvar_c) *uvar_c = (float)unbiased;
   }
 }
 
@@ -78,7 +87,8 @@
   s2 = block_sum(s2, scratch);
   if (threadIdx.x == 0) {
     if (FUSED) {
-      bn_finalize(s1, s2, f.count, f.eps, f.momentum, f.running_mean, f.running_var, c, f.mean[c], f.rstd[c]);
+      bn_finalize(s1, s2, f.count, f.eps, f.momentum, f.running_mean, f.running_var, c, f.mean[c], f.rstd[c],
+                  f.uvar ? f.uvar + (size_t)gi * grp.cs + c : nullptr);
       if (c == 0 && f.nbt) f.nbt[0] += 1;
     } else {
       part[((size_t)s * 2 + 0) * C + c] = s1;
@@ -96,17 +106,18 @@
 
 __global__ void bn_finalize_kernel(const double* __restrict__ sums, double count, float eps, float momentum,
                                    float* running_mean, float* running_var, int64_t* nbt, float* mean, float* rstd,
-                                   int C) {
+                                   float* uvar, int C) {
   const int c = blockIdx.x * blockDim.x + threadIdx.x;
   if (c == 0 && nbt) nbt[0] += 1;
   if (c >= C) return;
-  bn_finalize(sums[c], sums[C + c], count, eps, momentum, running_mean, running_var, c, mean[c], rstd[c]);
+  bn_finalize(sums[c], sums[C + c], count, eps, momentum, running_mean, running_var, c, mean[c], rstd[c],
+              uvar ? uvar + c : nullptr);
 }
 
 __global__ __launch_bounds__(256) void bn_tile_stats_finalize_kernel(const float* __restrict__ ts, int tiles, int pitch,
                                                                     double count, float eps, float momentum,
                                                                     float* running_mean, float* running_var, int64_t* nbt,
-                                                                    float* mean, float* rstd, int C) {
+                                                                    float* mean, float* rstd, float* uvar, int C) {
   __shared__ double scratch[4];
   const int c = blockIdx.x;
   const float* p1 = ts + (size_t)c * pitch;
@@ -116,14 +127,14 @@
   s1 = block_sum(s1, scratch);
   s2 = block_sum(s2, scratch);
   if (threadIdx.x == 0) {
-    bn_finalize(s1, s2, count, eps, momentum, running_mean, running_var, c, mean[c], rstd[c]);
+    bn_finalize(s1, s2, count, eps, momentum, running_mean, running_var, c, mean[c], rstd[c], uvar ? uvar + c : nullptr);
     if (c == 0 && nbt) nbt[0] += 1;
   }
 }
 
 __global__ void bn_combine_finalize_groups_kernel(const double* __restrict__ part, int splits, int G, double count, float eps,
                                                   float momentum, float* running_mean, float* running_var, int64_t* nbt,
-                                                  float* mean, float* rstd, int C) {
+                                                  float* mean, float* rstd, float* uvar, int C) {
   const int c = blockIdx.x * blockDim.x + threadIdx.x;
   if (c == 0 && nbt) nbt[0] += G;
   if (c >= C) return;
@@ -131,7 +142,8 @@
     const double* pg = part + (size_t)g * splits * 2 * C;
     const double s1 = fold_strided(0.0, pg + c, (size_t)2 * C, splits);
     const double s2 = fold_strided(0.0, pg + C + c, (size_t)2 * C, splits);
-    bn_finalize(s1, s2, count, eps, momentum, running_mean, running_var, c, mean[(size_t)g * C + c], rstd[(size_t)g * C + c]);
+    bn_finalize(s1, s2, count, eps, momentum, running_mean, running_var, c, mean[(size_t)g * C + c], rstd[(size_t)g * C + c],
+                uvar ? uvar + (size_t)g * C + c : nullptr);
   }
 }
 __global__ void bn_combine_param_groups_kernel(const double* __restrict__ part, double* __restrict__ dsums, int C, int splits,
@@ -156,6 +168,38 @@
   if (c >= C) return;
   mean[c] = rm[c];
   rstd[c] = 1.f / sqrtf(rv[c] + eps);
+}
+
+struct BnReplayDesc {
+  float* running_mean;
+  float* running_var;
+  int64_t* nbt;
+  const float* mean;
+  const float* uvar;
+  int C, G;
+  float momentum;
+  int block0;
+};
+static_assert(sizeof(BnReplayDesc) == 56, "BnReplayDesc layout is part of the ABI (itcv_bn_replay_desc_bytes)");
+constexpr int kBnReplayMaxDesc = 64;
+
+__global__ __launch_bounds__(256) void bn_replay_many(const BnReplayDesc* __restrict__ tab, int n) {
+  int di = 0;
+  while (di + 1 < n && (int)blockIdx.x >= tab[di + 1].block0) ++di;
+  const BnReplayDesc d = tab[di];
+  const int c = ((int)blockIdx.x - d.block0) * 256 + (int)threadIdx.x;
+  if (c >= d.C) return;
+  if (c == 0 && d.nbt) d.nbt[0] += d.G;
+  if (d.running_mean) {
+    float r = d.running_mean[c];
+    for (int g = 0; g < d.G; ++g) r = bn_blend(r, d.mean[(size_t)g * d.C + c], d.momentum);
+    d.running_mean[c] = r;
+  }
+  if (d.running_var) {
+    float r = d.running_var[c];
+    for (int g = 0; g < d.G; ++g) r = bn_blend(r, d.uvar[(size_t)g * d.C + c], d.momentum);
+    d.running_var[c] = r;
+  }
 }
 
 __device__ __forceinline__ float lrelu(float v, float slope) { return v > 0.f ? v : v * slope; }
@@ -214,6 +258,7 @@
   int64_t* nbt;
   float* mean_out;
   float* rstd_out;
+  float* uvar_out;
 };
 
 template <int PX, int NS>
@@ -284,7 +329,8 @@
                 t2 = fold_strided(0.0, pg + C + c, (size_t)2 * C, st.splits);
               }
               float um, ur;
-              bn_finalize(t1, t2, st.count, st.eps, st.momentum, st.running_mean, st.running_var, c, um, ur);
+              bn_finalize(t1, t2, st.count, st.eps, st.momentum, st.running_mean, st.running_var, c, um, ur,
+                          st.uvar_out ? st.uvar_out + (size_t)gg * C + c : nullptr);
             }
             if (c == 0 && st.nbt) st.nbt[0] += G;
           }
@@ -933,7 +979,7 @@
   ITCV_CHECK_LAUNCH(who);
   if (p.splits > 1 && p.path != BnPath::SlicedFold) {
     hipLaunchKernelGGL(bn_combine_finalize_groups_kernel, dim3(cdiv(C, 256)), dim3(256), 0, st, part, p.splits, p.G, f.count,
-                       f.eps, f.momentum, f.running_mean, f.running_var, f.nbt, f.mean, f.rstd, C);
+                       f.eps, f.momentum, f.running_mean, f.running_var, f.nbt, f.mean, f.rstd, f.uvar, C);
     ITCV_CHECK_LAUNCH(who);
   }
   return 0;
@@ -1074,18 +1120,25 @@
                         size_t ws_bytes, void* stream) {
   ITCV_REQUIRE(x && mean && rstd && B > 0 && C > 0 && HW > 0, "itcv_bn_train_stats");
   const BnPlan p = bn_plan(false, B, C, HW, 1, 0, 0, 1, false, 0, 0, ws ? ws_bytes : 0, false);
-  const BnFinal f{(double)B * HW, eps, momentum, running_mean, running_var, num_batches_tracked, mean, rstd};
+  const BnFinal f{(double)B * HW, eps, momentum, running_mean, running_var, num_batches_tracked, mean, rstd, nullptr};
   return bn_stats_launch(p, x, B, C, HW, f, ws, ws_bytes, S(stream), "itcv_bn_train_stats");
+}
+
+int itcv_bn_finalize_uv(const double* sums, double count, float eps, float momentum, float* running_mean,
+                        float* running_var, int64_t* num_batches_tracked, float* mean, float* rstd, float* unbiased_var,
+                        int C, void* stream) {
+  ITCV_REQUIRE(sums && mean && rstd && C > 0 && count > 0, "itcv_bn_finalize");
+  hipLaunchKernelGGL(bn_finalize_kernel, dim3(cdiv(C, 256)), dim3(256), 0, S(stream), sums, count, eps, momentum,
+                     running_mean, running_var, num_batches_tracked, mean, rstd, unbiased_var, C);
+  ITCV_CHECK_LAUNCH("itcv_bn_finalize");
+  return 0;
 }
 
 int itcv_bn_finalize(const double* sums, double count, float eps, float momentum, float* running_mean,
                      float* running_var, int64_t* num_batches_tracked, float* mean, float* rstd, int C,
                      void* stream) {
-  ITCV_REQUIRE(sums && mean && rstd && C > 0 && count > 0, "itcv_bn_finalize");
-  hipLaunchKernelGGL(bn_finalize_kernel, dim3(cdiv(C, 256)), dim3(256), 0, S(stream), sums, count, eps, momentum,
-                     running_mean, running_var, num_batches_tracked, mean, rstd, C);
-  ITCV_CHECK_LAUNCH("itcv_bn_finalize");
-  return 0;
+  return itcv_bn_finalize_uv(sums, count, eps, momentum, running_mean, running_var, num_batches_tracked, mean, rstd, nullptr,
+                             C, stream);
 }
 
 int itcv_bn_eval_stats(const float* running_mean, const float* running_var, float eps, float* mean, float* rstd,
@@ -1139,11 +1192,11 @@
   return 0;
 }
 
-int itcv_bn_train_fwd(const float* x, const float* gamma, const float* beta, const float* skip, float* y, void* planes,
-                      int ns, int B, int C, int H, int W, float slope, int pool, float eps, float momentum,
-                      float* running_mean, float* running_var, int64_t* num_batches_tracked, float* mean, float* rstd,
-                      void* ws, size_t ws_bytes, size_t plane_stride, const float* tile_stats, int tiles, int tile_pitch,
-                      int groups, void* stream) {
+int itcv_bn_train_fwd_uv(const float* x, const float* gamma, const float* beta, const float* skip, float* y, void* planes,
+                         int ns, int B, int C, int H, int W, float slope, int pool, float eps, float momentum,
+                         float* running_mean, float* running_var, int64_t* num_batches_tracked, float* mean, float* rstd,
+                         float* unbiased_var, void* ws, size_t ws_bytes, size_t plane_stride, const float* tile_stats,
+                         int tiles, int tile_pitch, int groups, void* stream) {
   ITCV_REQUIRE(x && gamma && beta && mean && rstd && (y || planes) && B > 0 && C > 0 && H > 0 && W > 0, "itcv_bn_train_fwd");
   const double px_out = (double)(groups > 1 ? groups : 1) * B * C * (pool ? H * W / 4 : H * W);
   ProfScope bn_prof(S(stream), 13, ilog2_exact(W) >= 0 ? ilog2_exact(W) : 0, C / 8, pool ? 1 : 0, planes ? ns : 0,
@@ -1157,28 +1210,68 @@
   if (p.path == BnPath::PerGroup) {
     const BnGrp& s = p.grp;
     for (int g = 0; g < groups; ++g)
-      if (int e = itcv_bn_train_fwd(x + g * s.xs, gamma, beta, skip ? skip + g * s.xs : nullptr, y ? y + g * s.os : nullptr,
-                                    planes ? static_cast<u32x4*>(planes) + g * s.ps : nullptr, ns, B, C, H, W, slope, pool,
-                                    eps, momentum, running_mean, running_var, num_batches_tracked, mean + (size_t)g * C,
-                                    rstd + (size_t)g * C, ws, ws_bytes, plane_stride,
-                                    tile_stats ? tile_stats + (size_t)g * tiles : nullptr, tiles, tile_pitch, 1, stream))
+      if (int e = itcv_bn_train_fwd_uv(x + g * s.xs, gamma, beta, skip ? skip + g * s.xs : nullptr, y ? y + g * s.os : nullptr,
+                                       planes ? static_cast<u32x4*>(planes) + g * s.ps : nullptr, ns, B, C, H, W, slope, pool,
+                                       eps, momentum, running_mean, running_var, num_batches_tracked, mean + (size_t)g * C,
+                                       rstd + (size_t)g * C, unbiased_var ? unbiased_var + (size_t)g * C : nullptr, ws,
+                                       ws_bytes, plane_stride, tile_stats ? tile_stats + (size_t)g * tiles : nullptr, tiles,
+                                       tile_pitch, 1, stream))
         return e;
     return 0;
   }
-  const BnFinal f{(double)B * H * W, eps, momentum, running_mean, running_var, num_batches_tracked, mean, rstd};
+  const BnFinal f{(double)B * H * W, eps, momentum, running_mean, running_var, num_batches_tracked, mean, rstd, unbiased_var};
   if (p.path == BnPath::TileStats) {
     ITCV_REQUIRE(tiles > 0 && tile_pitch >= tiles, "itcv_bn_train_fwd(tile statistics)");
     hipLaunchKernelGGL(bn_tile_stats_finalize_kernel, dim3(C), dim3(256), 0, S(stream), tile_stats, tiles, tile_pitch, f.count,
-                       eps, momentum, running_mean, running_var, num_batches_tracked, mean, rstd, C);
+                       eps, momentum, running_mean, running_var, num_batches_tracked, mean, rstd, unbiased_var, C);
     ITCV_CHECK_LAUNCH("itcv_bn_train_fwd(tile statistics)");
   } else if (int e = bn_stats_launch(p, x, B, C, H * W, f, ws, ws_bytes, S(stream), "itcv_bn_train_fwd(statistics)")) {
     return e;
   }
   const BnStatsIn fold = p.path == BnPath::SlicedFold
                              ? BnStatsIn{static_cast<const double*>(ws), p.splits, f.count, eps, momentum, running_mean,
-                                         running_var, num_batches_tracked, mean, rstd}
+                                         running_var, num_batches_tracked, mean, rstd, unbiased_var}
                              : BnStatsIn{};
   return bn_fwd_apply_launch(p, x, mean, rstd, gamma, beta, skip, y, planes, ns, B, C, H, W, slope, pool, fold, S(stream));
+}
+
+int itcv_bn_train_fwd(const float* x, const float* gamma, const float* beta, const float* skip, float* y, void* planes,
+                      int ns, int B, int C, int H, int W, float slope, int pool, float eps, float momentum,
+                      float* running_mean, float* running_var, int64_t* num_batches_tracked, float* mean, float* rstd,
+                      void* ws, size_t ws_bytes, size_t plane_stride, const float* tile_stats, int tiles, int tile_pitch,
+                      int groups, void* stream) {
+  return itcv_bn_train_fwd_uv(x, gamma, beta, skip, y, planes, ns, B, C, H, W, slope, pool, eps, momentum, running_mean,
+                              running_var, num_batches_tracked, mean, rstd, nullptr, ws, ws_bytes, plane_stride, tile_stats,
+                              tiles, tile_pitch, groups, stream);
+}
+
+size_t itcv_bn_replay_desc_bytes(void) { return sizeof(BnReplayDesc); }
+int itcv_bn_replay_max_descs(void) { return kBnReplayMaxDesc; }
+int itcv_bn_replay_desc(void* host_desc, float* running_mean, float* running_var, int64_t* num_batches_tracked,
+                        const float* mean, const float* unbiased_var, int C, int groups, float momentum, int block0) {
+  if (!(host_desc && C > 0 && groups >= 1 && block0 >= 0 && momentum >= 0.f && momentum <= 1.f) ||
+      (running_mean && !mean) || (running_var && !unbiased_var)) {
+    fail("%s: bad argument (descriptor, C > 0, groups >= 1, block0 >= 0, momentum in [0, 1], the saved statistics of every "
+         "running buffer given)", "itcv_bn_replay_desc");
+    return -1;
+  }
+  if (!running_mean && !running_var && !num_batches_tracked) return 0;
+  BnReplayDesc d;
+  memset(&d, 0, sizeof(d));
+  d.running_mean = running_mean, d.running_var = running_var, d.nbt = num_batches_tracked;
+  d.mean = mean, d.uvar = unbiased_var;
+  d.C = C, d.G = groups, d.momentum = momentum, d.block0 = block0;
+  memcpy(host_desc, &d, sizeof(d));
+  return cdiv(C, 256);
+}
+int itcv_bn_replay_many(const void* dev_table, int n, int total_blocks, void* stream) {
+  ITCV_REQUIRE(dev_table && n > 0 && total_blocks > 0, "itcv_bn_replay_many");
+  if (n > kBnReplayMaxDesc)
+    return fail("%s: at most %d descriptors per table (itcv_bn_replay_max_descs)", "itcv_bn_replay_many", kBnReplayMaxDesc);
+  hipLaunchKernelGGL(bn_replay_many, dim3(total_blocks), dim3(256), 0, S(stream),
+                     static_cast<const BnReplayDesc*>(dev_table), n);
+  ITCV_CHECK_LAUNCH("itcv_bn_replay_many");
+  return 0;
 }
 
 int itcv_bn_train_bwd(const float* x, const float* dy, const float* mean, const float* rstd, const float* gamma,
diff --git a/intro-tc-vae_amd/hipvae/abi.py b/intro-tc-vae_amd/hipvae/abi.py
--- a/intro-tc-vae_amd/hipvae/abi.py
+++ b/intro-tc-vae_amd/hipvae/abi.py
@@ -77,6 +77,7 @@
     "itcv_bn_moments": (i32, [p, p, i32, i32, i32, p, sz, p]),
     "itcv_bn_train_stats": (i32, [p, i32, i32, i32, f32, f32, p, p, p, p, p, p, sz, p]),
     "itcv_bn_finalize": (i32, [p, f64, f32, f32, p, p, p, p, p, i32, p]),
+    "itcv_bn_finalize_uv": (i32, [p, f64, f32, f32, p, p, p, p, p, p, i32, p]),
     "itcv_bn_eval_stats": (i32, [p, p, f32, p, p, i32, p]),
     "itcv_bn_act_planes_supported": (i32, [i32] * 4),
     "itcv_bn_act_fwd": (i32, [p, p, p, p, p, p, p, i32, i32, i32, i32, f32, i32, p, i32, sz, p]),
@@ -86,6 +87,12 @@
                                     i32, i32, p, i32, sz, p]),
     "itcv_bn_train_fwd": (i32, [p, p, p, p, p, p, i32, i32, i32, i32, i32, f32, i32, f32, f32, p, p, p, p, p, p, sz, sz, p, i32, i32,
                                 i32, p]),
+    "itcv_bn_train_fwd_uv": (i32, [p, p, p, p, p, p, i32, i32, i32, i32, i32, f32, i32, f32, f32, p, p, p, p, p, p, p, sz, sz, p, i32,
+                                   i32, i32, p]),
+    "itcv_bn_replay_desc_bytes": (sz, []),
+    "itcv_bn_replay_desc": (i32, [p, p, p, p, p, p, i32, i32, f32, i32]),
+    "itcv_bn_replay_many": (i32, [p, i32, i32, p]),
+    "itcv_bn_replay_max_descs": (i32, []),
     "itcv_bn_train_bwd": (i32, [p, p, p, p, p, p, p, p, p, p, p, i32, p, p, i32, i32, i32, i32, i32, f32, i32, i32, p,
                                 sz, sz, i32, p]),
     "itcv_bn_plan_query": (i32, [i32] * 10 + [sz, i32, p, p]),
diff --git a/intro-tc-vae_amd/hipvae/functional.py b/intro-tc-vae_amd/hipvae/functional.py
--- a/intro-tc-vae_amd/hipvae/functional.py
+++ b/intro-tc-vae_amd/hipvae/functional.py
@@ -55,6 +55,79 @@
 def _grad_target(param):
     g = param.grad if _DIRECT[0] else None
     return g if (g is not None and g.is_contiguous() and g.dtype == F32) else None
+
+
+_SHARED_PASS = [None]
+
+
+class SharedPass:
+
+    def __init__(self):
+        self.param_grads = True
+        self.input_grad = True
+        self.records = []
+        self._first = False
+        self._pool = {}
+        self._tables = {}
+
+    @contextlib.contextmanager
+    def record(self):
+        prev, _SHARED_PASS[0] = _SHARED_PASS[0], self
+        self.records, self._first = [], True
+        self.param_grads = self.input_grad = True
+        try:
+            yield self
+        finally:
+            _SHARED_PASS[0] = prev
+
+    def _claim_first(self):
+        first, self._first = self._first, False
+        return first
+
+    def _stats(self, G, C, device):
+        k = (len(self.records), G, C, str(device))
+        buf = self._pool.get(k)
+        if buf is None:
+            buf = self._pool[k] = torch.empty((2, G, C), dtype=F32, device=device)
+        return buf
+
+    def replay(self):
+        replay_bn_running(self.records, self._tables)
+
+
+def _shared_ok(ctx, what):
+    sp = ctx.shared
+    return sp is None or getattr(sp, what)
+
+
+def replay_bn_running(records, tables=None):
+    import ctypes
+    if tables is None:
+        tables = {}
+    recs = [r for r in records if r[0] is not None or r[1] is not None or r[2] is not None]
+    if not recs:
+        return
+    key = tuple((0 if r[0] is None else r[0].data_ptr(), 0 if r[1] is None else r[1].data_ptr(),
+                 0 if r[2] is None else r[2].data_ptr(), r[3].data_ptr(), r[4].data_ptr(), tuple(r[3].shape), r[5])
+                for r in recs)
+    tab = tables.get(key)
+    if tab is None:
+        if len(recs) > lib.itcv_bn_replay_max_descs():
+            raise abi.HipExtensionError("replay_bn_running: more BatchNorm layers than one table holds")
+        nb = lib.itcv_bn_replay_desc_bytes()
+        host = (ctypes.c_uint8 * (nb * len(recs)))()
+        blocks = 0
+        for i, (rm, rv, nbt, mean, uvar, momentum) in enumerate(recs):
+            G, C = mean.shape
+            got = lib.itcv_bn_replay_desc(ctypes.byref(host, i * nb), ptr(rm), ptr(rv), ptr(nbt), ptr(mean), ptr(uvar), C, G,
+                                          float(momentum), blocks)
+            if got <= 0:
+                raise abi.HipExtensionError("itcv_bn_replay_desc: " + abi.last_error())
+            blocks += got
+        tab = tables[key] = (torch.frombuffer(bytearray(host), dtype=torch.uint8).to(recs[0][3].device), len(recs), blocks,
+                             recs)
+    call("itcv_bn_replay_many", ptr(tab[0]), tab[1], tab[2], stream())
+
 
 
 
@@ -575,6 +648,8 @@
         ctx.save_for_backward(None if keep_xp is not None else _require_fp32(x, "Conv2dFn.forward (saved input)"),
                               weight, bias, keep_xp)
         ctx.cfg = (B, Ci, H, W, Co, KS, up2, bias is not None, (Hs, Ws))
+        ctx.shared = _SHARED_PASS[0]
+        ctx.shared_first = ctx.shared is not None and ctx.shared._claim_first()
         return y
 
     @staticmethod
@@ -584,13 +659,16 @@
         B, Ci, H, W, Co, KS, up2, has_bias, (Hs, Ws) = ctx.cfg
         dy = _f32c(dy)
         dx = dw = db = None
-        ns_d = _planes_ns(Co, Ci, KS, False) if ctx.needs_input_grad[0] else 0
-        wg_planes = ctx.needs_input_grad[1] and _wgrad_planes_ok(B, Ci, H, W, Co, KS)
+        need_x = ctx.needs_input_grad[0] and not (ctx.shared_first and not ctx.shared.input_grad)
+        need_w = ctx.needs_input_grad[1] and _shared_ok(ctx, "param_grads")
+        need_b = ctx.needs_input_grad[2] and _shared_ok(ctx, "param_grads")
+        ns_d = _planes_ns(Co, Ci, KS, False) if need_x else 0
+        wg_planes = need_w and _wgrad_planes_ok(B, Ci, H, W, Co, KS)
         dyp = None
         fmt2 = F16X2 if _NS[_CONV_MATH[0]] == F16X2 else 2
         if ns_d or wg_planes:
             dyp = planes_of(dy, ns_d if ns_d else fmt2, gradient=True)
-        if ctx.needs_input_grad[0]:
+        if need_x:
             if ns_d:
                 dx = conv_apply_planes(dyp, weight, weight, 1, None, B, Co, H, W, Ci, KS, False, ns_d)
             else:
@@ -599,7 +677,7 @@
                 lo = torch.empty((B, Ci, H // 2, W // 2), dtype=F32, device=dy.device)
                 call("itcv_upsample2_bwd", ptr(dx), ptr(lo), B * Ci, H // 2, W // 2, stream())
                 dx = lo
-        wg5 = _wgrad5_mode(Ci, H, W, Co, KS, up2) if ctx.needs_input_grad[1] else None
+        wg5 = _wgrad5_mode(Ci, H, W, Co, KS, up2) if need_w else None
         if wg5 == "predict" and xp is None and x is None:
             wg5 = None
         if wg5 is not None:
@@ -613,7 +691,7 @@
                 conv_wgrad5_planes(small, big, B, cs, H, W, wg5 == "stem", out=tgt, accumulate=True, ns=fmt2)
             else:
                 dw = conv_wgrad5_planes(small, big, B, cs, H, W, wg5 == "stem", ns=fmt2)
-        elif ctx.needs_input_grad[1]:
+        elif need_w:
             tgt = _grad_target(weight)
             if wg_planes and (ns_d in (0, fmt2)):
                 if xp is None:
@@ -630,7 +708,7 @@
                     conv_wgrad_raw(x, dy, B, Ci, H, W, Co, KS, up2, out=tgt, accumulate=True)
                 else:
                     dw = conv_wgrad_raw(x, dy, B, Ci, H, W, Co, KS, up2)
-        if has_bias and ctx.needs_input_grad[2]:
+        if has_bias and need_b:
             db = bias_grad_raw(_require_fp32(dy, "Conv2dFn.backward (bias gradient)"), B, Co, H * W, _grad_target(bias))
         return dx, dw, db, None
 
@@ -649,6 +727,8 @@
              nws, stream())
         ctx.save_for_backward(x, weight, bias)
         ctx.cfg = (B, K, N, bias is not None)
+        ctx.shared = _SHARED_PASS[0]
+        ctx.shared_first = ctx.shared is not None and ctx.shared._claim_first()
         return y
 
     @staticmethod
@@ -659,17 +739,18 @@
         dy = _f32c(dy)
         dx = dw = db = None
         nws = lib.itcv_linear_workspace(B, K, N)
-        if ctx.needs_input_grad[0]:
+        need_p = _shared_ok(ctx, "param_grads")
+        if ctx.needs_input_grad[0] and not (ctx.shared_first and not ctx.shared.input_grad):
             dx = torch.empty((B, K), dtype=F32, device=dy.device)
             ws = _ws(nws, dy.device) if nws else None
             call("itcv_linear_dgrad", ptr(dy), ptr(weight), ptr(dx), B, K, N, ptr(ws), nws, stream())
-        if ctx.needs_input_grad[1]:
+        if ctx.needs_input_grad[1] and need_p:
             tgt = _grad_target(weight)
             dw = None if tgt is not None else torch.empty((N, K), dtype=F32, device=dy.device)
             ws = _ws(nws, dy.device) if nws else None
             call("itcv_linear_wgrad", ptr(dy), ptr(x), ptr(tgt if tgt is not None else dw), B, K, N,
                  int(tgt is not None), ptr(ws), nws, stream())
-        if has_bias and ctx.needs_input_grad[2]:
+        if has_bias and ctx.needs_input_grad[2] and need_p:
             db = bias_grad_raw(dy, B, N, 1, _grad_target(bias))
         return dx, dw, db
 
@@ -691,7 +772,12 @@
             raise abi.HipExtensionError(f"BatchNorm groups: batch {B} is not {G} equal passes")
         Bg = B // G
         dev = x.device
-        mean = torch.empty((G, C), dtype=F32, device=dev)
+        shared = _SHARED_PASS[0]
+        uvar = None
+        if shared is not None and training:
+            mean, uvar = shared._stats(G, C, dev)
+        else:
+            mean = torch.empty((G, C), dtype=F32, device=dev)
         rstd = torch.empty((G, C), dtype=F32, device=dev)
         world = _world(group) if training else 1
         oshape = (B, C, H // 2, W // 2) if pool else (B, C, H, W)
@@ -710,10 +796,15 @@
         ts = _tile_stats_of(x, B, G, H * W) if (training and world == 1) else None
         if training and world == 1:
             ws = _ws(nws, dev)
-            call("itcv_bn_train_fwd", ptr(x), ptr(gamma), ptr(beta), ptr(skip), ptr(y) if write_y else None, ptr(yp),
-                 int(out_planes), Bg, C, H, W, float(slope), int(pool), float(eps), float(momentum), ptr(running_mean),
-                 ptr(running_var), ptr(nbt), ptr(mean), ptr(rstd), ptr(ws), nws, pstride,
-                 None if ts is None else ts[0].data_ptr(), ts[1] if ts else 0, ts[2] if ts else 0, G, stream())
+            head = (ptr(x), ptr(gamma), ptr(beta), ptr(skip), ptr(y) if write_y else None, ptr(yp), int(out_planes), Bg, C, H,
+                    W, float(slope), int(pool), float(eps), float(momentum), ptr(running_mean), ptr(running_var), ptr(nbt),
+                    ptr(mean), ptr(rstd))
+            tail = (ptr(ws), nws, pstride, None if ts is None else ts[0].data_ptr(), ts[1] if ts else 0, ts[2] if ts else 0,
+                    G, stream())
+            if uvar is None:
+                call("itcv_bn_train_fwd", *head, *tail)
+            else:
+                call("itcv_bn_train_fwd_uv", *head, ptr(uvar), *tail)
         for g in (range(G) if not (training and world == 1) else ()):
             r = slice(g * Bg, (g + 1) * Bg)
             xg, yg = x[r], (y[r] if write_y else None)
@@ -724,8 +815,9 @@
                 sums = torch.empty((2 * C,), dtype=torch.float64, device=dev)
                 call("itcv_bn_moments", ptr(xg), ptr(sums), Bg, C, H * W, ptr(ws), nws, stream())
                 dist.all_reduce(sums, group=group)
-                call("itcv_bn_finalize", ptr(sums), float(Bg * H * W * world), float(eps), float(momentum),
-                     ptr(running_mean), ptr(running_var), ptr(nbt), ptr(mean[g]), ptr(rstd[g]), C, stream())
+                call("itcv_bn_finalize_uv", ptr(sums), float(Bg * H * W * world), float(eps), float(momentum),
+                     ptr(running_mean), ptr(running_var), ptr(nbt), ptr(mean[g]), ptr(rstd[g]),
+                     None if uvar is None else ptr(uvar[g]), C, stream())
             else:
                 call("itcv_bn_eval_stats", ptr(running_mean), ptr(running_var), float(eps), ptr(mean[g]), ptr(rstd[g]), C,
                      stream())
@@ -735,6 +827,9 @@
             if _POISON[0] and not out_fp32:
                 y.fill_(float("nan"))
             _tag_planes(y, yp, out_planes, bool(out_fp32))
+        if uvar is not None:
+            shared.records.append((running_mean, running_var, nbt, mean, uvar, float(momentum)))
+        ctx.shared = shared
         ctx.save_for_backward(x, gamma, beta, mean, rstd, skip)
         ctx.params = (gamma, beta)
         if not lib.itcv_bn_act_planes_supported(C, H, W, 0):
@@ -755,15 +850,17 @@
         dev = x.device
         Bg = B // G
         nws = lib.itcv_bn_workspace(Bg, C, H * W) * G
-        tg = _grad_target(gamma) if ctx.needs_input_grad[1] else None
-        tb = _grad_target(beta) if ctx.needs_input_grad[2] else None
+        need_g = ctx.needs_input_grad[1] and _shared_ok(ctx, "param_grads")
+        need_b = ctx.needs_input_grad[2] and _shared_ok(ctx, "param_grads")
+        tg = _grad_target(gamma) if need_g else None
+        tb = _grad_target(beta) if need_b else None
         direct = tg is not None and tb is not None
         dgamma = dbeta = None
         if direct:
             pg, pb = tg, tb
         else:
-            dgamma = torch.empty_like(gamma) if ctx.needs_input_grad[1] else None
-            dbeta = torch.empty_like(beta) if ctx.needs_input_grad[2] else None
+            dgamma = torch.empty_like(gamma) if need_g else None
+            dbeta = torch.empty_like(beta) if need_b else None
             pg, pb = dgamma, dbeta
         dx = torch.empty_like(x)
         dskip = torch.empty_like(x) if (skip is not None and ctx.needs_input_grad[3]) else None
diff --git a/intro-tc-vae_amd/solvers/intro.py b/intro-tc-vae_amd/solvers/intro.py
--- a/intro-tc-vae_amd/solvers/intro.py
+++ b/intro-tc-vae_amd/solvers/intro.py
@@ -4,8 +4,8 @@
 from torch import Tensor
 
 from hipvae import ddp
-from hipvae.functional import ExpElboFn
-from models import bn_groups
+from hipvae.functional import ExpElboFn, SharedPass
+from models import _has_hooks, bn_groups
 from ops import noise, reparameterize
 from solvers.vae import VAESolver
 
@@ -19,6 +19,14 @@
         self.beta_neg = beta_neg
         self.gamma_r = gamma_r
         self.batch_passes = True
+        self.share_decoder_pass = True
+        self._shared_pass = SharedPass()
+
+    def _shares_pass(self) -> bool:
+        return bool(self.batch_passes and self.share_decoder_pass) and not _has_hooks(self.model.decoder)
+
+    def _schedule_key(self) -> tuple:
+        return (bool(self.batch_passes), self._shares_pass())
 
     def _exp_elbo(self, rec_rows: Tensor, kl_rows: Tensor) -> Tensor:
         while rec_rows.dim() > 1:
@@ -36,12 +44,19 @@
         def two():
             return bn_groups(2)
 
+        share, shared = self._shares_pass(), self._shared_pass
         noise_batch = noise((real.size(0), model.zdim), self.device)
         self._set_trainable(encoder=True, decoder=False)
         real_mu, real_logvar = model.encode(real)
         z = reparameterize(real_mu, real_logvar)
-        with two():
-            fake, rec = model.decoder(cat([noise_batch, z])).chunk(2)
+        if share:
+            self._set_trainable(encoder=True, decoder=True)
+            with two(), shared.record():
+                fake, rec = model.decoder(cat([noise_batch, z])).chunk(2)
+            self._set_trainable(encoder=True, decoder=False)
+        else:
+            with two():
+                fake, rec = model.decoder(cat([noise_batch, z])).chunk(2)
         loss_rec = self.compute_rec_loss(real, rec, reduction="mean")
         loss_e_real_kl = self.compute_kl_loss(z, real_mu, real_logvar, write=True)
         with two():
@@ -56,11 +71,19 @@
         expelbo_rec = self._exp_elbo(self.compute_rec_loss(rec, rec_rec, reduction="none"), kl_rec)
         expelbo_fake = self._exp_elbo(self.compute_rec_loss(fake, rec_fake, reduction="none"), kl_fake)
         loss_e = self._lincomb((scale, scale, 0.25, 0.25), loss_rec, loss_e_real_kl, expelbo_rec, expelbo_fake)
-        finish_average = self._backward(loss_e, ("encoder",), defer_average=True)
+        shared.param_grads = False
+        finish_average = self._backward(loss_e, ("encoder",), defer_average=True, retain_graph=share)
+        shared.param_grads = True
 
         self._set_trainable(encoder=False, decoder=True)
-        with two():
-            fake, rec = model.decoder(cat([noise_batch, z.detach()])).chunk(2)
+        if share:
+            loss_e, loss_e_real_kl, expelbo_fake = loss_e.detach(), loss_e_real_kl.detach(), expelbo_fake.detach()
+            del (loss_rec, mu2, logvar2, rec_mu, fake_mu, rec_logvar, fake_logvar, z_rec, z_fake, rec_rec, rec_fake, kl_rec,
+                 kl_fake, expelbo_rec, real_mu, real_logvar, z)
+            shared.replay()
+        else:
+            with two():
+                fake, rec = model.decoder(cat([noise_batch, z.detach()])).chunk(2)
         finish_average()
         norm_e = self._clip()
         self._step("encoder")
@@ -79,7 +102,11 @@
         loss_d_fake_kl = self.compute_kl_loss(z_fake, fake_mu, fake_logvar)
         loss_d = self._lincomb((scale, 0.5 * scale, 0.5 * scale, 0.5 * scale, 0.5 * scale), loss_rec, loss_d_rec_kl,
                                loss_d_fake_kl, loss_rec_rec, loss_fake_rec)
-        self._backward(loss_d, ("decoder",))
+        if share:
+            shared.input_grad = False
+            self._backward(loss_d, ("decoder",), inputs=self._params("decoder"))
+        else:
+            self._backward(loss_d, ("decoder",))
         norm_d = self._clip()
         self._step("decoder")
 
diff --git a/intro-tc-vae_amd/solvers/vae.py b/intro-tc-vae_amd/solvers/vae.py
--- a/intro-tc-vae_amd/solvers/vae.py
+++ b/intro-tc-vae_amd/solvers/vae.py
@@ -87,12 +87,12 @@
         for p in self._params("decoder"):
             p.requires_grad = decoder
 
-    def _backward(self, loss, parts, defer_average=False):
+    def _backward(self, loss, parts, defer_average=False, retain_graph=False, inputs=None):
         groups = [self._group(p) for p in parts]
         for g in groups:
             g.zero_grad()
         with direct_grad_accumulation(), deferred_wgrad_reduces():
-            loss.backward()
+            loss.backward(retain_graph=retain_graph, inputs=inputs)
         if defer_average:
             pending = [ddp.average_async(g.flat_g) for g in groups]
             return lambda: [f() for f in pending]
@@ -140,7 +140,8 @@
             else None
         if not self._graph_ok(specs):
             return self._device_step(real)
-        key = (tuple(real.shape), real.dtype, self.conv_math) + specs + (getattr(self, "kl_loss", None),)
+        key = (tuple(real.shape), real.dtype, self.conv_math) + specs + self._schedule_key() \
+            + (getattr(self, "kl_loss", None),)
         from hipvae.functional import bump_weight_epoch
         graphs = self.__dict__.setdefault("_graphs", {})
         ent = graphs.get(key)
@@ -166,6 +167,9 @@
         bump_weight_epoch()
         return ent["out"]
 
+    def _schedule_key(self) -> tuple:
+        return ()
+
     def _device_step(self, real: Tensor) -> Tensor:
         self._set_trainable(True, True)
         mu, logvar, z, rec = self.model(real)
```

Result: faster. 4268 images/s (median of 6 runs) (+5.4%).
